# zhouyifan233/light-transport

Measured on AMD Instinct MI355X. Metric: photon_steps_per_sec, higher is better.
Workload: dtype f64

## Files before the change

light_transport_amd/csrc/lt_api.cpp:

```cpp
#include <hip/hip_runtime_api.h>

#include <dlfcn.h>

#include <algorithm>
#include <cmath>
#include <cctype>
#include <cstdarg>
#include <cstdio>
#include <cstdlib>
#include <cstring>
#include <limits>
#include <mutex>
#include <new>
#include <string>
#include <vector>

#include "lt_internal.hpp"

using namespace ltk;

static const size_t kMeshLdsBudget = 64 * 1024;

namespace {

// ... 593 lines not shown
        const uint64_t full = (body + rounds * (uint64_t)lanes - 1) / (rounds * (uint64_t)lanes);
        for (uint64_t k = 0, done_b = 0; k < rounds * (uint64_t)lanes && done_b < body; k++) {
            const uint64_t take = full < body - done_b ? full : body - done_b;
            plan->batches.emplace_back(l, take);
            done_b += take; left -= take; l = (l + 1) % lanes;
        }
        while (left > 0) {
            const uint64_t take = (double)left > fit ? (uint64_t)fit : left;
            plan->batches.emplace_back(l, take);
            left -= take; l = (l + 1) % lanes;
        }
    }
    return LT_OK;
}

int choose_lanes(lt_ctx* c, uint64_t n)
{
    c->auto_pending = -1;
    if (c->overlap_mode == 1) return 1;
    if (c->overlap_mode >= 2) return n >= 8192 ? c->overlap_mode : 1;
    if (c->blocks_per_cu > 0 || n < kOverlapMinPhotons) return 1;
    for (int k = kAutoLanes - 1; k >= 0; k--) {
        const bool stale = c->auto_photons[k] != 0 && (n > 2 * c->auto_photons[k] || c->auto_photons[k] > 2 * n);
        if (c->auto_ms_per_photon[k] <= 0.0 || stale) { c->auto_pending = k; return k + 1; }
    }
    int best = 0;
    for (int k = 1; k < kAutoLanes; k++) if (c->auto_ms_per_photon[k] < c->auto_ms_per_photon[best]) best = k;
    return best + 1;
}

struct LogRun {
    lt_ctx* c; WalkParams P; Variant v; LaunchCfg cfg; LogGeom G;
};

struct WalkGate {
    std::mutex mu;
    hipEvent_t ring[64] = {};
    unsigned next = 0;
    hipEvent_t last = nullptr;
};
WalkGate& walk_gate(int device)
{
    static WalkGate gates[16];
    return gates[device & 15];
}

hipError_t lane_event(LogLane& ln, hipStream_t s)
{
    if (ln.ev_used == ln.evs.size()) {
        hipEvent_t ev;
        hipError_t e = hipEventCreate(&ev);
        if (e != hipSuccess) return e;
        ln.evs.push_back(ev);
    }
    return hipEventRecord(ln.evs[ln.ev_used++], s);
}

int run_log_plan(LogRun& R, const LogPlan& plan, uint64_t offset, int* n_batches)
{
    lt_ctx* c = R.c;
    const LogGeom& G = R.G;
    const bool hot = G.bits2 != 0 && c->dmap_valid;
    const uint32_t n_hist = G.bits2 ? G.nb1 : G.n_tiles;
    LaunchCfg cfg = R.cfg;
    cfg.lds_bytes = walk_lds_bytes(R.v, R.P.n_media, R.P.n_layers, R.P.n_tris, R.P.n_nodes, n_hist);
    const int resident = walk_max_blocks_per_cu(R.v, cfg.threads, cfg.lds_bytes);
    if (resident <= 0) return c->fail(LT_E_HIP, "lt_launch: log-mode kernel not resident");
    int per_cu = c->blocks_per_cu > 0 ? c->blocks_per_cu : (plan.lanes >= 2 ? (resident + 1) / 2 : resident);
    if (plan.lanes >= 2 && c->knob.overlap_walk_bpc >= 1 && c->knob.overlap_walk_bpc <= 8) per_cu = (int)c->knob.overlap_walk_bpc;
    const unsigned long long cap = (unsigned long long)per_cu * (unsigned long long)c->prop.multiProcessorCount;
    if (plan.lanes >= 2) {
        const size_t gb = c->n_vox() * c->grid_elem();
        HIP_TRY(c, hipEventRecord(c->ev_fork, c->stream));
        for (int l = 1; l < plan.lanes; l++) {
            if (!c->lanes[l].stream) HIP_TRY(c, hipStreamCreateWithFlags(&c->lanes[l].stream, hipStreamNonBlocking));
            HIP_TRY(c, hipStreamWaitEvent(c->lanes[l].stream, c->ev_fork, 0));
            HIP_TRY(c, hipMemsetAsync(c->d_gridx[l - 1].p, 0, gb, c->lanes[l].stream));
        }
    }
    for (const auto& bt : plan.batches) {
        LogLane& ln = c->lanes[bt.first];
        hipStream_t s = ln.stream;
        uint32_t* meta = (uint32_t*)ln.meta.p;
        WalkParams P = R.P;
        P.n_photons = bt.second; P.photon_offset = offset;
        if (bt.first >= 1) P.grid = c->d_gridx[bt.first - 1].p;
        P.head = (unsigned long long*)ln.head.p;
        P.log_idx = (uint32_t*)ln.log_idx.p; P.log_val = ln.log_val.p; P.log_fill = (uint32_t*)ln.log_fill.p;
        P.log_next = meta + LM_NEXT; P.log_overflow = meta + LM_OVERFLOW; P.log_cap_chunks = plan.cap_chunks[bt.first];
        P.log_hist = (uint32_t*)(hot ? ln.hist_unused.p : (G.bits2 ? ln.hist1.p : ln.hist.p)); P.log_n_hist = n_hist; P.log_hist_shift = kTileShift + G.bits2;
        P.log_ntx = G.ntx; P.log_nty = G.nty;
        const unsigned long long want = (bt.second + (unsigned long long)cfg.threads - 1) / (unsigned long long)cfg.threads;
        cfg.blocks = (int)(want < cap ? want : cap);
        if (cfg.blocks < 1) cfg.blocks = 1;

        LogReduceParams L;
        std::memset(&L, 0, sizeof L);
        L.log_idx = P.log_idx; L.log_val = P.log_val; L.log_fill = P.log_fill;
        L.tmp_idx = (uint32_t*)ln.tmp_idx.p; L.tmp_val = ln.tmp_val.p;
        L.hist1 = (uint32_t*)ln.hist1.p; L.hist = (uint32_t*)ln.hist.p;
        L.bin_base = (uint32_t*)ln.bin_base.p; L.bin_cnt = (uint32_t*)ln.bin_cnt.p;
        L.tile_base = (uint32_t*)ln.tile_base.p; L.tile_cnt = (uint32_t*)ln.tile_cnt.p;
        L.cursor1 = (uint32_t*)ln.cursor1.p; L.cursor2 = (uint32_t*)ln.cursor2.p;
        L.items2 = (uint32_t*)ln.items2.p; L.items_c = (uint32_t*)ln.items_c.p; L.items_r = (uint32_t*)ln.items_r.p;
        L.itab = (uint32_t*)ln.itab.p;
        L.meta = meta; L.job = (unsigned long long*)c->d_job.p; L.cap_chunks = P.log_cap_chunks;
        L.n_tiles = G.n_tiles; L.bits2 = G.bits2;
        L.grid = bt.first >= 1 ? c->d_gridx[bt.first - 1].p : c->d_grid.p; L.n_vox = c->n_vox(); L.tally = c->tally;
        L.nx = (uint32_t)c->nx; L.ny = (uint32_t)c->ny; L.nz = (uint32_t)c->nz; L.ntx = G.ntx; L.nty = G.nty;
        L.flush_atomic = 0;
        if (hot) { L.dmap = (const uint16_t*)c->d_dmap.p; L.dmeta = (const uint32_t*)c->d_dmeta.p; }

        HIP_TRY(c, hipMemsetAsync(ln.head.p, 0, sizeof(unsigned long long), s));
        HIP_TRY(c, hipMemsetAsync(meta, 0, LM_WORDS * 4, s));
        HIP_TRY(c, hipMemsetAsync(ln.hist.p, 0, (size_t)G.n_tiles * (G.bits2 ? kLogGroups2 : kLogGroups) * 4, s));
        HIP_TRY(c, hipMemsetAsync(ln.log_fill.p, 0, (size_t)P.log_cap_chunks * 4, s));
        if (G.bits2) HIP_TRY(c, hipMemsetAsync(ln.hist1.p, 0, (size_t)(hot ? log_max_digits() : G.nb1) * kLogGroups * 4, s));
        const bool last_batch = &bt == &plan.batches.back();
        const uint64_t waves_launched = (uint64_t)cfg.blocks * (uint64_t)(cfg.threads / 64);
        const bool big_enough = c->knob.tail_split >= 2 || bt.second >= kTailSplitMinPerWave * waves_launched;
        const bool split = R.v.mesh <= 1 && !R.v.table && !R.v.capture && c->knob.tail_split != 0 && big_enough &&
                           ((plan.lanes == 1 && (c->blocks_per_cu == 0 || c->knob.serial_walks > 0) && (!R.v.f32 || c->knob.tail_split >= 2)) ||
                            (plan.lanes > 1 && last_batch));
        L.alone = (plan.lanes == 1 && c->blocks_per_cu == 0 && !split) ? 1 : 0;
        if (c->knob.part_alone == 0 || c->knob.part_alone == 1) L.alone = (int)c->knob.part_alone;
        L.lds_part = c->knob.part_lds > 0 ? (int)(c->knob.part_lds & 7) : 0;
        Variant vw = R.v;
        if (split) {
            const size_t cap = (size_t)cfg.blocks * (size_t)(cfg.threads / 64) * kDumpPoolLanes;
            P.dump_max = c->knob.tail_split > 1 ? (uint32_t)std::min<long>(c->knob.tail_split, (long)kDumpPoolLanes) : kDumpMaxLanes;
            HIP_TRY(c, ln.pool.ensure(cap * (R.v.f32 ? sizeof(SurvD<float>) : sizeof(SurvD<double>))));
            HIP_TRY(c, ln.pool_n.ensure(4));
            if (!ln.tail_stream) HIP_TRY(c, hipStreamCreateWithFlags(&ln.tail_stream, hipStreamNonBlocking));
            if (!ln.ev_bulk) HIP_TRY(c, hipEventCreateWithFlags(&ln.ev_bulk, hipEventDisableTiming));
            if (!ln.ev_tail) HIP_TRY(c, hipEventCreateWithFlags(&ln.ev_tail, hipEventDisableTiming));
            HIP_TRY(c, hipMemsetAsync(ln.pool_n.p, 0, 4, s));
            P.pool = ln.pool.p; P.pool_n = (uint32_t*)ln.pool_n.p; P.pool_cap = (uint32_t)cap;
            vw.phase = 1;
        }
        const bool train = c->knob.serial_walks > 0;
        if (train) {
            WalkGate& g = walk_gate(c->device);
            std::lock_guard<std::mutex> lk(g.mu);
            if (g.last) HIP_TRY(c, hipStreamWaitEvent(s, g.last, 0));
        }
        HIP_TRY(c, lane_event(ln, s));
        HIP_TRY(c, launch_walk(P, vw, cfg, s));
        HIP_TRY(c, lane_event(ln, s));
        if (split) {
            HIP_TRY(c, hipEventRecord(ln.ev_bulk, s));
            HIP_TRY(c, hipStreamWaitEvent(ln.tail_stream, ln.ev_bulk, 0));
            WalkParams Pt = P;
            Pt.log_idx = nullptr; Pt.log_val = nullptr; Pt.log_n_hist = 0;
            Variant vt = R.v; vt.phase = 2;
            LaunchCfg ct = cfg;
            ct.lds_bytes = walk_lds_bytes(vt, P.n_media, P.n_layers, P.n_tris, P.n_nodes, 0);
            ct.blocks = (int)((P.pool_cap / 64u + (unsigned)(cfg.threads / 64) - 1) / (unsigned)(cfg.threads / 64));
            if (ct.blocks < 1) ct.blocks = 1;
            HIP_TRY(c, launch_walk(Pt, vt, ct, ln.tail_stream));
            HIP_TRY(c, hipEventRecord(ln.ev_tail, ln.tail_stream));
        }
        if (hot) HIP_TRY(c, launch_log_count1(L, s));
        HIP_TRY(c, G.bits2 ? launch_log_scan_bins(L, s) : launch_log_scan_tiles(L, s));
        if (train) {
            WalkGate& g = walk_gate(c->device);
            std::lock_guard<std::mutex> lk(g.mu);
            hipEvent_t& ev = g.ring[g.next++ & 63u];
            if (!ev) HIP_TRY(c, hipEventCreateWithFlags(&ev, hipEventDisableTiming));
            HIP_TRY(c, hipEventRecord(ev, s));
            g.last = ev;
        }
        HIP_TRY(c, lane_event(ln, s));
        HIP_TRY(c, launch_log_part1(L, s));
        LogReduceParams Lr = L;
        if (G.bits2 == 0) { Lr.log_idx = L.tmp_idx; Lr.log_val = L.tmp_val; }
        else HIP_TRY(c, launch_log_part2(L, s));
        HIP_TRY(c, lane_event(ln, s));
        if (split) Lr.flush_atomic = 1;
        HIP_TRY(c, launch_log_reduce(Lr, s));
        HIP_TRY(c, lane_event(ln, s));
        if (split) HIP_TRY(c, hipStreamWaitEvent(s, ln.ev_tail, 0));
        if (bt.first == 0 && G.bits2) c->tile_cnt_ready = true;
        offset += bt.second;
        (*n_batches)++;
    }
    for (int l = 1; l < plan.lanes; l++) {
        HIP_TRY(c, hipEventRecord(c->lanes[l].ev_done, c->lanes[l].stream));
        HIP_TRY(c, hipStreamWaitEvent(c->stream, c->lanes[l].ev_done, 0));
        HIP_TRY(c, launch_grid_add(c->d_grid.p, c->d_gridx[l - 1].p, c->tally, c->n_vox(), c->stream));
    }
    return LT_OK;
}

bool bvh_is_valid(const std::vector<lt_bvh_node>& n, int n_tris, int* max_depth)
{
    std::vector<std::pair<int, int>> todo{{0, 0}};
    std::vector<char> seen(n.size(), 0);
    size_t visited = 0;
    *max_depth = 0;
    while (!todo.empty()) {
        const auto [idx, depth] = todo.back(); todo.pop_back();
        if (idx < 0 || idx >= (int)n.size() || seen[idx]) return false;
        seen[idx] = 1; visited++;
        if (depth > *max_depth) *max_depth = depth;
        const lt_bvh_node& nd = n[idx];
        if (nd.n_prims > 0) { if (nd.offset < 0 || nd.offset + nd.n_prims > n_tris) return false; continue; }
        if (nd.axis < 0 || nd.axis > 2 || nd.offset <= idx + 1) return false;
        todo.emplace_back(nd.offset, depth + 1); todo.emplace_back(idx + 1, depth + 1);
    }
    return visited == n.size();
}

}

extern "C" {

int lt_abi_version(void) { return LT_ABI_VERSION; }

const char* lt_last_error(const lt_ctx* ctx) { return ctx ? ctx->err.c_str() : g_create_error.c_str(); }

int lt_create(lt_ctx** out, int device_id)
{
    if (!out) return LT_E_INVALID;
    *out = nullptr;
    int n_dev = 0;
    hipError_t e = hipGetDeviceCount(&n_dev);
    if (e != hipSuccess || n_dev <= 0) {
        g_create_error = std::string("no HIP device available (") + (e != hipSuccess ? hipGetErrorString(e) : "0 devices") +
                         "); this library has no CPU fallback";
        return LT_E_HIP;
    }
    if (device_id < 0 || device_id >= n_dev) { g_create_error = "device_id out of range"; return LT_E_INVALID; }
    lt_ctx* c = new (std::nothrow) lt_ctx();
    if (!c) { g_create_error = "out of host memory"; return LT_E_NOMEM; }
    c->device = device_id;
    {
        static const char* const names[] = {"query_min", "log_bits2", "log_hot", "overlap_walk_bpc", "diag_no_tally", "log_timing", "march_cells",
                                            "march_scale_milli", "no_march", "no_clearance", "no_near_lists", "clearance_cells", "march_info", "force_march", "tail_split", "part_alone", "serial_walks", "part_lds",
                                            "render_lds_tables"};
        for (const char* k : names) {
            std::string name = "LT_";
            for (const char* q = k; *q; q++) name += (char)std::toupper((unsigned char)*q);
            if (const char* v = std::getenv(name.c_str())) *c->knob_by_name(k) = std::atol(v);
        }
        if (const char* v = std::getenv("LT_OVERLAP_PATTERN")) c->knob.overlap_pattern = v;
    }
    e = hipSetDevice(device_id);
    if (e == hipSuccess) e = hipGetDeviceProperties(&c->prop, device_id);
    if (e == hipSuccess && std::strncmp(c->prop.gcnArchName, "gfx950", 6) != 0) {
        g_create_error = std::string("device arch ") + c->prop.gcnArchName + " is not gfx950: kernels are built for MI355X only";
        delete c;
        return LT_E_UNSUPPORTED;
    }
    if (e == hipSuccess) {
        size_t quarter = c->prop.totalGlobalMem / 4;
        c->log_budget = c->default_log_budget = quarter < ((size_t)64 << 30) ? quarter : ((size_t)64 << 30);
    }
    if (e == hipSuccess) e = hipStreamCreateWithFlags(&c->stream, hipStreamNonBlocking);
    c->lanes[0].stream = c->stream;
    if (e == hipSuccess) e = hipEventCreate(&c->ev0);
    if (e == hipSuccess) e = hipEventCreate(&c->ev1);
    if (e == hipSuccess) e = hipEventCreateWithFlags(&c->ev_fork, hipEventDisableTiming);
    for (int k = 0; k < kMaxLanes && e == hipSuccess; k++) e = hipEventCreateWithFlags(&c->lanes[k].ev_done, hipEventDisableTiming);
    if (e == hipSuccess) e = c->d_job.ensure(2 * sizeof(unsigned long long));
    if (e == hipSuccess) e = c->d_counters.ensure(sizeof(DevCounters));
    if (e == hipSuccess) e = c->d_head.ensure(sizeof(unsigned long long));
    if (e == hipSuccess) e = hipMemsetAsync(c->d_counters.p, 0, sizeof(DevCounters), c->stream);
    if (e != hipSuccess) {
        g_create_error = std::string("lt_create: ") + hipGetErrorString(e);
        delete c;
        return LT_E_HIP;
    }
    *out = c;
    return LT_OK;
}

int lt_destroy(lt_ctx* c)
{
    if (!c) return LT_OK;
    (void)hipSetDevice(c->device);
    if (c->stream) (void)hipStreamSynchronize(c->stream);
    for (int i = 0; i < 2; i++) { c->d_media[i].release(); c->d_zb[i].release(); c->d_if[i].release(); c->d_tris[i].release(); c->d_nodes[i].release(); }
    c->d_lm.release(); c->d_grid.release(); c->d_counters.release(); c->d_head.release(); c->d_table.release();
    c->d_scratch_in.release(); c->d_scratch_out.release(); c->d_scratch_aux.release();
    c->d_mats.release(); c->d_lights.release(); c->d_r0.release(); c->d_r1.release(); c->d_lc.release();
    c->d_img.release(); c->d_xy.release(); c->d_vtx.release(); c->d_vcnt.release(); c->d_clear.release();
    c->d_job.release(); c->d_dmap.release(); c->d_dmeta.release();
    c->d_mcell.release(); c->d_mlist.release(); c->d_mcoarse.release(); c->d_links.release();
    for (int k = 1; k < kMaxLanes; k++) { c->d_gridx[k - 1].release(); if (c->lanes[k].stream) (void)hipStreamSynchronize(c->lanes[k].stream); }
    for (int k = 0; k < kMaxLanes; k++) {
        c->lanes[k].release_all();
        for (hipEvent_t ev : c->lanes[k].evs) (void)hipEventDestroy(ev);
        if (c->lanes[k].ev_done) (void)hipEventDestroy(c->lanes[k].ev_done);
    }
    if (c->ev0) (void)hipEventDestroy(c->ev0);
    if (c->ev1) (void)hipEventDestroy(c->ev1);
    if (c->ev_fork) (void)hipEventDestroy(c->ev_fork);
    for (int k = 0; k < kMaxLanes; k++) {
        if (c->lanes[k].tail_stream) { (void)hipStreamSynchronize(c->lanes[k].tail_stream); (void)hipStreamDestroy(c->lanes[k].tail_stream); }
        if (c->lanes[k].ev_bulk) (void)hipEventDestroy(c->lanes[k].ev_bulk);
        if (c->lanes[k].ev_tail) (void)hipEventDestroy(c->lanes[k].ev_tail);
    }
    for (int k = 1; k < kMaxLanes; k++) if (c->lanes[k].stream) (void)hipStreamDestroy(c->lanes[k].stream);
    if (c->stream) (void)hipStreamDestroy(c->stream);
    delete c;
    return LT_OK;
}
// ... 10 lines not shown
    c->media.assign(media, media + n);
    c->scene_changed();
    c->tables_dirty = true;
    return LT_OK;
}

int lt_set_layers(lt_ctx* c, const double* z_bounds, const int32_t* medium_idx, int n, double n_above, double n_below)
{
    CHECK_CTX(c);
    if (!z_bounds || !medium_idx || n <= 0 || n > kMaxLayers)
        return c->fail(LT_E_INVALID, "lt_set_layers: need 1..%d layers", kMaxLayers);
    if (!std::isfinite(z_bounds[0])) return c->fail(LT_E_INVALID, "lt_set_layers: z_bounds[0] must be finite");
    for (int i = 0; i < n; i++) {
        if (!(z_bounds[i + 1] > z_bounds[i])) return c->fail(LT_E_INVALID, "lt_set_layers: z_bounds must ascend");
        if (medium_idx[i] < 0) return c->fail(LT_E_INVALID, "lt_set_layers: negative medium index");
    }
    if (!(n_above > 0) || !(n_below > 0)) return c->fail(LT_E_INVALID, "lt_set_layers: ambient indices must be > 0");
    c->z_bounds.assign(z_bounds, z_bounds + n + 1);
    c->layer_medium.assign(medium_idx, medium_idx + n);
    c->n_above = n_above; c->n_below = n_below;
    c->have_layers = true; c->have_mesh = false;
    c->scene_changed();
    c->tables_dirty = true;
    return LT_OK;
}

int lt_set_mesh(lt_ctx* c, const double* verts, const int32_t* med_front, const int32_t* med_back, int n_tris,
                const lt_bvh_node* nodes, int n_nodes)
{
    CHECK_CTX(c);
    if (!verts || !med_front || !med_back || n_tris <= 0 || !nodes || n_nodes <= 0)
        return c->fail(LT_E_INVALID, "lt_set_mesh: empty mesh or BVH");
    for (size_t i = 0; i < (size_t)n_tris * 9; i++)
        if (!std::isfinite(verts[i])) return c->fail(LT_E_INVALID, "lt_set_mesh: non-finite vertex");
    std::vector<lt_bvh_node> nn(nodes, nodes + n_nodes);
    int depth = 0;
    if (!bvh_is_valid(nn, n_tris, &depth))
        return c->fail(LT_E_INVALID, "lt_set_mesh: BVH is not a valid pre-order tree over %d triangles", n_tris);
    size_t covered = 0;
    for (const auto& nd : nn) if (nd.n_prims > 0) covered += (size_t)nd.n_prims;
    if (covered != (size_t)n_tris) return c->fail(LT_E_INVALID, "lt_set_mesh: leaves cover %zu of %d triangles", covered, n_tris);
    c->verts.assign(verts, verts + (size_t)n_tris * 9);
    c->med_front.assign(med_front, med_front + n_tris);
    c->med_back.assign(med_back, med_back + n_tris);
    c->nodes.swap(nn);
    c->have_mesh = true; c->have_layers = false;
    c->surf_mats.clear();
    c->scene_changed();
    c->tables_dirty = true;
    return LT_OK;
}

int lt_set_grid(lt_ctx* c, int nx, int ny, int nz, const double origin[3], const double voxel[3], int tally_dtype)
{
    CHECK_CTX(c);
    if (nx <= 0 || ny <= 0 || nz <= 0 || !origin || !voxel) return c->fail(LT_E_INVALID, "lt_set_grid: bad shape");
    if (tally_dtype < LT_TALLY_F32 || tally_dtype > LT_TALLY_U64FX) return c->fail(LT_E_INVALID, "lt_set_grid: bad tally dtype");
    for (int k = 0; k < 3; k++)
        if (!(voxel[k] > 0) || !std::isfinite(origin[k])) return c->fail(LT_E_INVALID, "lt_set_grid: bad origin/voxel");
    if ((double)nx * ny * nz > 2147483647.0) return c->fail(LT_E_UNSUPPORTED, "lt_set_grid: more than 2^31-1 voxels");
    BIND(c);
    c->nx = nx; c->ny = ny; c->nz = nz; c->tally = tally_dtype;
    for (int k = 0; k < 3; k++) { c->origin[k] = origin[k]; c->voxel[k] = voxel[k]; }
    HIP_TRY(c, c->d_grid.ensure(c->n_vox() * c->grid_elem()));
    c->have_grid = true;
    c->scene_changed();
    return lt_zero_tally(c);
}

int lt_set_source(lt_ctx* c, int type, const double pos[3], const double dir[3], const double* extra, int start_medium)
{
    CHECK_CTX(c);
    if (!pos || !dir || (type != LT_SRC_PENCIL && type != LT_SRC_COSINE_QUAD)) return c->fail(LT_E_INVALID, "lt_set_source: bad arguments");
    const double l = std::sqrt(dir[0] * dir[0] + dir[1] * dir[1] + dir[2] * dir[2]);
    if (!(l > 0) || !std::isfinite(l)) return c->fail(LT_E_INVALID, "lt_set_source: zero direction");
    if (type == LT_SRC_COSINE_QUAD && !extra) return c->fail(LT_E_INVALID, "lt_set_source: quad source needs extra[6]");
    c->src_type = type; c->start_medium = start_medium;
    for (int k = 0; k < 3; k++) { c->src_pos[k] = pos[k]; c->src_dir[k] = dir[k] / l; }
    for (int k = 0; k < 6; k++) c->src_extra[k] = extra ? extra[k] : 0.0;
    c->have_source = true;
    c->scene_changed();
    return LT_OK;
}

int lt_set_max_steps(lt_ctx* c, uint32_t max_steps)
{
    CHECK_CTX(c);
    if (max_steps == 0) return c->fail(LT_E_INVALID, "lt_set_max_steps: must be > 0");
    c->max_steps = max_steps;
    return LT_OK;
}

int lt_set_tuning(lt_ctx* c, const char* key, int64_t value)
{
    CHECK_CTX(c);
    long* k = key ? c->knob_by_name(key) : nullptr;
    if (!k) return c->fail(LT_E_INVALID, "lt_set_tuning: unknown key '%s'", key ? key : "(null)");
    *k = value < 0 ? -1 : (long)value;
    if (!std::strcmp(key, "log_hot") || !std::strcmp(key, "log_bits2")) { c->dmap_valid = false; }
    return LT_OK;
}

int lt_set_tally_quantity(lt_ctx* c, int quantity)
{
    CHECK_CTX(c);
    if (quantity != LT_QUANTITY_ABSORBED && quantity != LT_QUANTITY_FLUENCE)
        return c->fail(LT_E_INVALID, "lt_set_tally_quantity: LT_QUANTITY_ABSORBED or LT_QUANTITY_FLUENCE");
    if (quantity != c->quantity) { c->quantity = quantity; c->media_dirty = true; }
    return LT_OK;
}

int lt_set_launch_config(lt_ctx* c, int blocks_per_cu, int threads_per_block)
{
    CHECK_CTX(c);
    if (blocks_per_cu < 0 || threads_per_block < 0 || threads_per_block > 256 || (threads_per_block % 64) != 0)
        return c->fail(LT_E_INVALID, "lt_set_launch_config: threads must be a multiple of 64, <= 256");
    c->blocks_per_cu = blocks_per_cu; c->threads_per_block = threads_per_block;
    return LT_OK;
}

int lt_zero_tally(lt_ctx* c)
{
    CHECK_CTX(c);
    BIND(c);
    if (c->have_grid) HIP_TRY(c, hipMemsetAsync(c->d_grid.p, 0, c->n_vox() * c->grid_elem(), c->stream));
    HIP_TRY(c, hipMemsetAsync(c->d_counters.p, 0, sizeof(DevCounters), c->stream));
    return LT_OK;
}

int lt_launch(lt_ctx* c, uint64_t n_photons, uint64_t photon_offset, uint64_t seed, const double* rng_table,
              uint64_t table_steps, uint32_t flags)
{
    CHECK_CTX(c);
    if (c->media.empty()) return c->fail(LT_E_STATE, "lt_launch: lt_set_media first");
    if (!c->have_layers && !c->have_mesh) return c->fail(LT_E_STATE, "lt_launch: lt_set_layers or lt_set_mesh first");
    if (!c->have_grid) return c->fail(LT_E_STATE, "lt_launch: lt_set_grid first");
    if (!c->have_source) return c->fail(LT_E_STATE, "lt_launch: lt_set_source first");
    const int n_media = (int)c->media.size();
    if (c->have_layers) {
        for (int32_t m : c->layer_medium) if (m >= n_media) return c->fail(LT_E_INVALID, "lt_launch: layer medium index %d >= %d media", m, n_media);
    } else {
        for (size_t i = 0; i < c->med_front.size(); i++)
            if (c->med_front[i] >= n_media || c->med_back[i] >= n_media || c->med_front[i] < -1 || c->med_back[i] < -1)
                return c->fail(LT_E_INVALID, "lt_launch: triangle %zu medium index out of range", i);
        if (c->start_medium < 0 || c->start_medium >= n_media) return c->fail(LT_E_INVALID, "lt_launch: start_medium out of range");
    }
    Variant v;
    v.f32 = (flags & LT_FLAG_F32_WALK) ? 1 : 0;
    v.mesh = c->have_mesh ? 1 : 0;
    v.table = rng_table ? 1 : 0;
    v.tally = c->tally;
    v.capture = c->max_vertices > 0 ? 1 : 0;
    v.phase = 0;
    if (v.capture && (v.f32 || v.table)) return c->fail(LT_E_UNSUPPORTED, "lt_launch: vertex capture runs the f64 walk with the XORWOW generator");
    if (c->on(c->knob.diag_no_tally)) v.tally = 3;
    if (v.table && v.f32) return c->fail(LT_E_UNSUPPORTED, "lt_launch: table RNG runs the f64 walk only");
    if (v.table && v.tally == LT_TALLY_F32) return c->fail(LT_E_UNSUPPORTED, "lt_launch: table RNG needs an f64 or u64fx tally");
    if (v.table && table_steps == 0) return c->fail(LT_E_INVALID, "lt_launch: table_steps == 0");
    BIND(c);
    int rc = upload_tables(c);
    if (rc) return rc;
    if (n_photons == 0) { c->timed = false; return LT_OK; }

    if (v.table) {
        const size_t bytes = (size_t)n_photons * (size_t)table_steps * 4 * sizeof(double);
        HIP_TRY(c, c->d_table.ensure(bytes));
        HIP_TRY(c, hipMemcpyAsync(c->d_table.p, rng_table, bytes, hipMemcpyHostToDevice, c->stream));
        HIP_TRY(c, hipStreamSynchronize(c->stream));
    }

    WalkParams P;
    std::memset(&P, 0, sizeof P);
    P.head = (unsigned long long*)c->d_head.p;
    P.n_photons = n_photons; P.photon_offset = photon_offset; P.seed = seed;
    const int pi = v.f32 ? 1 : 0;
    P.media = c->d_media[pi].p; P.zb = c->d_zb[pi].p; P.ifaces = c->d_if[pi].p; P.layer_medium = (const int32_t*)c->d_lm.p;
    P.tris = c->d_tris[pi].p; P.nodes = c->d_nodes[pi].p; P.links = c->have_mesh && c->have_links ? (const int16_t*)c->d_links.p : nullptr;
    P.n_media = n_media;
    P.n_layers = c->have_layers ? (int)c->layer_medium.size() : 0;
    P.n_tris = c->have_mesh ? (int)c->med_front.size() : 0;
    P.n_nodes = c->have_mesh ? (int)c->nodes.size() : 0;
    P.n_above = c->n_above; P.n_below = c->n_below;
    P.grid = c->d_grid.p; P.nx = c->nx; P.ny = c->ny; P.nz = c->nz; P.tally = c->tally;
    for (int k = 0; k < 3; k++) {
        P.origin[k] = c->origin[k]; P.inv_voxel[k] = 1.0 / c->voxel[k];
        P.src_pos[k] = c->src_pos[k]; P.src_dir[k] = c->src_dir[k];
        P.src_e1[k] = c->src_extra[k]; P.src_e2[k] = c->src_extra[3 + k];
    }
    P.fdim[0] = (double)c->nx; P.fdim[1] = (double)c->ny; P.fdim[2] = (double)c->nz;
    for (int k = 0; k < 3; k++) { P.f32.origin[k] = (float)P.origin[k]; P.f32.inv_voxel[k] = (float)P.inv_voxel[k]; P.f32.fdim[k] = (float)P.fdim[k]; }
    P.src_type = c->src_type; P.start_medium = c->start_medium;
    P.table = (const double*)c->d_table.p; P.table_steps = table_steps;
    P.max_steps = c->max_steps;
    P.counters = (DevCounters*)c->d_counters.p;
    if (c->knob.query_min >= 1 && c->knob.query_min <= 64) P.query_min = (unsigned)c->knob.query_min;
    if (c->have_mesh && c->have_clear) {
        P.clear = (const uint4*)c->d_clear.p; P.cnx = c->cn[0]; P.cny = c->cn[1]; P.cnz = c->cn[2];
        for (int k = 0; k < 3; k++) {
            P.corg[k] = c->corg[k]; P.cinv[k] = 1.0 / c->ccell[k]; P.cdim[k] = (double)c->cn[k];
            P.f32.corg[k] = (float)P.corg[k]; P.f32.cinv[k] = (float)P.cinv[k]; P.f32.cdim[k] = (float)P.cdim[k];
        }
    }
    if (c->have_mesh && c->have_march) P.mg = c->mgrid;
    c->captured_photons = 0;
    if (c->max_vertices > 0) {
        const size_t vb = (size_t)n_photons * c->max_vertices * sizeof(lt_vertex);
        if (vb > ((size_t)64 << 30)) return c->fail(LT_E_NOMEM, "lt_launch: vertex capture needs %zu bytes (> 64 GiB)", vb);
        HIP_TRY(c, c->d_vtx.ensure(vb));
        HIP_TRY(c, c->d_vcnt.ensure((size_t)n_photons * sizeof(uint32_t)));
        HIP_TRY(c, hipMemsetAsync(c->d_vcnt.p, 0, (size_t)n_photons * sizeof(uint32_t), c->stream));
        P.vertices = (lt_vertex*)c->d_vtx.p; P.vertex_counts = (uint32_t*)c->d_vcnt.p; P.max_vertices = c->max_vertices;
        c->captured_photons = n_photons; c->captured_max_vertices = c->max_vertices;
    }

    LaunchCfg cfg;
    cfg.threads = c->threads_per_block > 0 ? c->threads_per_block : 256;
    cfg.lds_bytes = walk_lds_bytes(v, P.n_media, P.n_layers, P.n_tris, P.n_nodes);
    if (v.mesh && (cfg.lds_bytes > kMeshLdsBudget || (c->on(c->knob.force_march) && c->have_march && !v.table))) {
        if (v.table) return c->fail(LT_E_UNSUPPORTED, "lt_launch: table RNG with a mesh beyond the LDS budget");
        v.mesh = c->have_march ? 3 : 2;
        cfg.lds_bytes = walk_lds_bytes(v, P.n_media, P.n_layers, P.n_tris, P.n_nodes);
    }
    int resident = walk_max_blocks_per_cu(v, cfg.threads, cfg.lds_bytes);
    if (resident <= 0) return c->fail(LT_E_HIP, "lt_launch: kernel variant not resident (occupancy query returned %d)", resident);
    int per_cu = c->blocks_per_cu > 0 ? c->blocks_per_cu : resident;
    unsigned long long want = (n_photons + (unsigned long long)cfg.threads - 1) / (unsigned long long)cfg.threads;
    unsigned long long cap = (unsigned long long)per_cu * (unsigned long long)c->prop.multiProcessorCount;
    cfg.blocks = (int)(want < cap ? want : cap);
    if (cfg.blocks < 1) cfg.blocks = 1;

    const int mode = c->tally_mode == 2 ? 1 : c->tally_mode;
    { int rc3 = collect_log_stats(c); if (rc3) return rc3; }
    LogGeom G = log_geom(c);
    bool use_log = mode == 1 && !v.table && c->max_vertices == 0 && G.n_tiles <= kMaxLogTiles && !c->on(c->knob.diag_no_tally);
    if (use_log) {
        LogRun R;
        R.c = c; R.P = P; R.v = v; R.cfg = cfg; R.G = G;
        if (c->dmap_valid && (c->dmap_tiles != G.n_tiles || c->dmap_bits2 != G.bits2)) c->dmap_valid = c->tile_cnt_ready = false;
        c->stages_valid = false;
        for (LogLane& ln : c->lanes) ln.ev_used = 0;
        HIP_TRY(c, hipMemsetAsync(c->d_job.p, 0, 2 * sizeof(unsigned long long), c->stream));
        uint64_t done = 0;
        int n_batches = 0;
        if (c->rec_per_photon <= 0.0 && n_photons > kPilotPhotons) {
            LogPlan pilot;
            rc = plan_log(c, kPilotPhotons, 1, &pilot);
            if (rc == LT_OK) rc = run_log_plan(R, pilot, photon_offset, &n_batches);
            if (rc == LT_E_NOMEM) { use_log = false; rc = LT_OK; }
            else if (rc) return rc;
            else {
                c->log_stats_pending = true; c->pending_photons = kPilotPhotons; c->auto_pending = -1;
                if ((rc = collect_log_stats(c))) return rc;
                done = kPilotPhotons;
            }
        }
        if (use_log && G.bits2 && !c->dmap_valid && c->tile_cnt_ready && G.n_tiles <= kMaxHotTiles && G.nb1 < log_max_digits()) {
            uint32_t max_hot = log_max_digits() - G.nb1;
            if (c->knob.log_hot >= 0 && (uint32_t)c->knob.log_hot < max_hot) max_hot = (uint32_t)c->knob.log_hot;
            if (max_hot > 0) {
                HIP_TRY(c, c->d_dmap.ensure(((size_t)G.n_tiles + 2) * sizeof(uint16_t)));
                HIP_TRY(c, c->d_dmeta.ensure(4 * sizeof(uint32_t)));
                HIP_TRY(c, launch_log_plan((const uint32_t*)c->lanes[0].tile_cnt.p, G.n_tiles, G.bits2, max_hot, (uint16_t*)c->d_dmap.p,
                                           (uint32_t*)c->d_dmeta.p, c->stream));
                c->dmap_valid = true; c->dmap_tiles = G.n_tiles; c->dmap_bits2 = G.bits2;
            }
        }
        if (use_log) {
            int lanes = choose_lanes(c, n_photons - done);
            LogPlan plan;
            rc = plan_log(c, n_photons - done, lanes, &plan);
            while (rc == LT_E_NOMEM && lanes > 1) {
                lanes--; rc = plan_log(c, n_photons - done, lanes, &plan);
                if (c->auto_pending >= 0) c->auto_pending = lanes - 1;
            }
            if (rc == LT_E_NOMEM) { use_log = false; rc = LT_OK; }
            else if (rc) return rc;
            else {
                HIP_TRY(c, hipEventRecord(c->ev0, c->stream));
                if ((rc = run_log_plan(R, plan, photon_offset + done, &n_batches))) return rc;
                HIP_TRY(c, hipEventRecord(c->ev1, c->stream));
                c->stages_valid = true; c->last_batches = (uint64_t)n_batches; c->last_lanes = plan.lanes;
                c->last_hot = G.bits2 != 0 && c->dmap_valid;
                c->log_stats_pending = true; c->pending_photons = n_photons;
                if (c->auto_pending >= 0 && done > 0) c->auto_pending = -1;
                c->timed = true;
                if (c->on(c->knob.log_timing)) {
                    double ms[4]; uint64_t rec = 0, bat = 0;
                    if (lt_last_log_stages(c, ms, &rec, &bat) == LT_OK)
                        std::fprintf(stderr, "[lt log] %llu photons, %d lane(s), %llu batches, %llu records (%.1f / photon), %llu to atomics; "
                                     "stage sums ms: walk %.2f scan %.2f partition %.2f reduce %.2f\n", (unsigned long long)n_photons,
                                     plan.lanes, (unsigned long long)bat, (unsigned long long)rec, (double)rec / (double)n_photons,
                                     (unsigned long long)c->last_overflow, ms[0], ms[1], ms[2], ms[3]);
                }
                return LT_OK;
            }
        }
        P.n_photons = n_photons - done; P.photon_offset = photon_offset + done;
        want = (P.n_photons + (unsigned long long)cfg.threads - 1) / (unsigned long long)cfg.threads;
        cfg.blocks = (int)(want < cap ? want : cap);
        if (cfg.blocks < 1) cfg.blocks = 1;
    }

    c->stages_valid = false;
    HIP_TRY(c, hipMemsetAsync(c->d_head.p, 0, sizeof(unsigned long long), c->stream));
    HIP_TRY(c, hipEventRecord(c->ev0, c->stream));
    HIP_TRY(c, launch_walk(P, v, cfg, c->stream));
    HIP_TRY(c, hipEventRecord(c->ev1, c->stream));
    c->timed = true;
    return LT_OK;
}

int lt_reserve_log(lt_ctx* c, uint64_t n_photons)
{
    CHECK_CTX(c);
    if (!c->have_grid) return c->fail(LT_E_STATE, "lt_reserve_log: lt_set_grid first");
    BIND(c);
    LogPlan plan;
    int lanes = c->overlap_mode == 1 ? 1 : (c->overlap_mode >= 2 ? c->overlap_mode : ((c->blocks_per_cu == 0 && n_photons >= kOverlapMinPhotons) ? kAutoLanes : 1));
    int rc = plan_log(c, n_photons, lanes, &plan);
    if (rc == LT_E_NOMEM) return c->fail(LT_E_NOMEM, "lt_reserve_log: not enough device memory for the deposit log");
    return rc;
}

int lt_set_tally_mode(lt_ctx* c, int mode, uint64_t log_bytes)
{
    CHECK_CTX(c);
    if (mode < 0 || mode > 2) return c->fail(LT_E_INVALID, "lt_set_tally_mode: mode must be LT_MODE_ATOMIC, LT_MODE_LOG or LT_MODE_AUTO");
    c->tally_mode = mode;
    c->log_budget = log_bytes ? (size_t)log_bytes : c->default_log_budget;
    return LT_OK;
}

int lt_last_log_hot_tiles(lt_ctx* c, uint32_t* hot_tiles, uint32_t* threshold)
{
    CHECK_CTX(c);
    if (!c->stages_valid) return c->fail(LT_E_STATE, "lt_last_log_hot_tiles: the last launch did not use the deposit log");
    BIND(c);
    uint32_t m[2] = {0, 0};
    if (c->last_hot) {
        HIP_TRY(c, hipStreamSynchronize(c->stream));
        HIP_TRY(c, hipMemcpy(m, c->d_dmeta.p, sizeof m, hipMemcpyDeviceToHost));
    }
    if (hot_tiles) *hot_tiles = m[0];
    if (threshold) *threshold = m[1];
    return LT_OK;
}

int lt_set_overlap(lt_ctx* c, int lanes)
{
    CHECK_CTX(c);
    if (lanes < 0 || lanes > kMaxLanes) return c->fail(LT_E_INVALID, "lt_set_overlap: 0 (auto), 1, 2 or 3");
    c->overlap_mode = lanes;
    for (double& a : c->auto_ms_per_photon) a = 0.0;
    for (uint64_t& a : c->auto_photons) a = 0;
    c->auto_pending = -1;
    return LT_OK;
}

int lt_sync(lt_ctx* c)
{
    CHECK_CTX(c);
    BIND(c);
    HIP_TRY(c, hipStreamSynchronize(c->stream));
    return collect_log_stats(c);
}

int lt_last_kernel_ms(lt_ctx* c, double* ms)
{
    CHECK_CTX(c);
    if (!ms) return c->fail(LT_E_INVALID, "lt_last_kernel_ms: null output");
    if (!c->timed) return c->fail(LT_E_STATE, "lt_last_kernel_ms: no launch recorded");
    BIND(c);
    HIP_TRY(c, hipEventSynchronize(c->ev1));
    float f = 0;
    HIP_TRY(c, hipEventElapsedTime(&f, c->ev0, c->ev1));
    *ms = (double)f;
    return LT_OK;
}

int lt_last_log_stages(lt_ctx* c, double ms_out[4], uint64_t* records, uint64_t* batches)
{
    CHECK_CTX(c);
    if (!ms_out) return c->fail(LT_E_INVALID, "lt_last_log_stages: null output");
    if (!c->stages_valid) return c->fail(LT_E_STATE, "lt_last_log_stages: the last launch did not use the log tally");
    BIND(c);
    HIP_TRY(c, hipEventSynchronize(c->ev1));
    { int rc3 = collect_log_stats(c); if (rc3) return rc3; }
    for (int k = 0; k < 4; k++) ms_out[k] = 0.0;
    for (int l = 0; l < kMaxLanes; l++) {
        const LogLane& ln = c->lanes[l];
// ... 398 lines not shown
```

light_transport_amd/csrc/lt_internal.hpp:

```cpp
#pragma once
#include <hip/hip_runtime_api.h>
#include <stdint.h>

#include "../../include/lt.h"

namespace ltk {

template <typename R>
struct MedD {
    R mu_t, inv_mu_t, absorb, g;
    R n, one_m_g2, one_p_g2, inv_2g;
    R dep;
    R one_m_g, two_g;
    R pad_;
};

template <typename R>
struct IfD {
    R n_up, n_dn;
    R nr_down, nr_up;
};

template <typename R>
struct TriD {
    R a[3], ab[3], ac[3], n[3];
    int32_t med_front, med_back;
};

template <typename R>
struct NodeD {
    R lo[3], hi[3];
    int32_t offset, n_prims, axis;
    int32_t skip;
};

struct DevCounters {
    unsigned long long photons, steps;
    double w[8];
};
enum { CW_ABSORBED = 0, CW_LOST, CW_ESC_TOP, CW_ESC_BOT, CW_ESC_MESH, CW_SPECULAR, CW_ROULETTE, CW_CAPPED };

constexpr int kMaxMedia = 32;
constexpr uint32_t kLogChunk = 8192;
constexpr uint32_t kTileShift = 14;
constexpr uint32_t kTileSize = 1u << kTileShift;
constexpr uint32_t kTileBX = 5, kTileBY = 5, kTileBZ = 4;
constexpr uint32_t kLogGroups = 16;
constexpr uint32_t kLogGroups2 = 8;
constexpr int kMaxLayers = 64;

constexpr uint32_t kMarchCountMask = 63u;
struct MarchGrid {
    const uint2* cell;
    const uint32_t* list;
    int nx, ny, nz;
    double org[3], inv[3], h[3];
    double fn[3];
    float org32[3], inv32[3], h32[3], fn32[3];
    double nudge64, nudge32;
};

template <typename R>
struct SurvD {
    R p[3], u[3], w, sleft;
    unsigned long long pid;
    int32_t cur;
    uint32_t step;
    uint32_t rng[6];
    uint32_t held[3];
    uint32_t q_pend;
};
constexpr uint32_t kDumpMaxLanes = 32;
constexpr uint32_t kDumpPoolLanes = 48;

struct WalkParams {
    unsigned long long* head;
    unsigned long long n_photons, photon_offset, seed;
    const void* media;
    const void* zb;
    const void* ifaces;
    const int32_t* layer_medium;
    const void* tris;
    const void* nodes;
    const int16_t* links;
    int n_media, n_layers, n_tris, n_nodes;
    double n_above, n_below;
    void* grid;
    int nx, ny, nz, tally;
    double origin[3], inv_voxel[3];
    double fdim[3];
    double cdim[3];
    struct { float origin[3], inv_voxel[3], fdim[3], corg[3], cinv[3], cdim[3]; } f32;
    int src_type, start_medium;
    double src_pos[3], src_dir[3], src_e1[3], src_e2[3];
    const double* table;
    unsigned long long table_steps;
    unsigned max_steps;
    unsigned query_min;
    DevCounters* counters;
    uint32_t* log_idx;
    void* log_val;
    uint32_t* log_fill;
    uint32_t* log_next;
    uint32_t log_cap_chunks;
    uint32_t* log_hist;
    uint32_t log_n_hist, log_hist_shift, log_ntx, log_nty;
    uint32_t* log_overflow;
    const uint4* clear;
    int cnx, cny, cnz;
    double corg[3], cinv[3];
    MarchGrid mg;
    void* pool;
    uint32_t* pool_n;
    uint32_t pool_cap;
    uint32_t dump_max;
    lt_vertex* vertices;
    uint32_t* vertex_counts;
    unsigned max_vertices;
};

struct LaunchCfg {
    int blocks, threads;
    size_t lds_bytes;
};

struct Variant {
    int f32;
    int mesh;
    int table;
    int tally;
    int capture;
    int phase;
};

hipError_t launch_walk(const WalkParams& P, const Variant& v, const LaunchCfg& cfg, hipStream_t s);
size_t walk_lds_bytes(const Variant& v, int n_media, int n_layers, int n_tris, int n_nodes, unsigned n_hist = 0);
int walk_max_blocks_per_cu(const Variant& v, int threads, size_t lds_bytes);

struct RenderParams {
    const void* tris;
    const void* nodes;
    const lt_surface_material* mats;
    const lt_point_light* lights;
    const int16_t* links;
    int n_tris, n_nodes, n_lights;
    int W, H, S, D;
    double cam[3], f_distance;
    const double* xs;
    const double* ys;
    double* rand_0;
    const double* rand_1;
    const int32_t* light_choice;
    double* image;
    int variant;
    int choices;
    int lds_tables;
};
constexpr int kRenderOldMaxDepth = 24;
hipError_t launch_march_clearance(const void* tris_f64, const void* nodes_f64, int n_nodes, const MarchGrid& G, uint2* cells,
                                  double* coarse, hipStream_t s);
hipError_t launch_build_clearance(const void* tris_f64, int n_tris, int near_lists, void* clear_records, int nx, int ny, int nz,
                                  const double org[3], const double cell[3], hipStream_t s);
hipError_t launch_render_surface(const RenderParams& P, hipStream_t s);

enum { LM_NEXT = 0,
       LM_OVERFLOW = 16,
       LM_RECORDS,
       LM_ITEMS2,
       LM_ITEMS_R,
       LM_SLICE,
       LM_ITEMS_C,
       LM_WORK,
       LM_WORDS = 24 };
static_assert(kLogGroups == 16, "LM_NEXT holds one counter per group");
constexpr uint32_t kTileAlign = 8, kBinAlign = 8;

struct LogReduceParams {
    const uint32_t* log_idx; const void* log_val; const uint32_t* log_fill;
    uint32_t* tmp_idx; void* tmp_val;
    uint32_t* hist1;
    uint32_t* hist;
    uint32_t* bin_base; uint32_t* bin_cnt;
    uint32_t* tile_base; uint32_t* tile_cnt;
    uint32_t* cursor1;
    uint32_t* cursor2;
    uint32_t* items2;
    uint32_t* items_c;
    uint32_t* itab;
    uint32_t* items_r;
    uint32_t* meta;
    unsigned long long* job;
    uint32_t cap_chunks;
    uint32_t n_tiles, bits2;
    void* grid; size_t n_vox; int tally;
    uint32_t nx, ny, nz, ntx, nty;
    const uint16_t* dmap; const uint32_t* dmeta;
    int alone;
    int flush_atomic;
    int lds_part;
};
hipError_t launch_log_scan_bins(const LogReduceParams& L, hipStream_t s);
hipError_t launch_log_count1(const LogReduceParams& L, hipStream_t s);
hipError_t launch_log_plan(const uint32_t* tile_cnt, uint32_t n_tiles, uint32_t bits2, uint32_t max_hot, uint16_t* dmap,
                           uint32_t* dmeta, hipStream_t s);
uint32_t log_max_digits();
constexpr uint32_t kMaxHotTiles = 8192;
hipError_t launch_log_scan_tiles(const LogReduceParams& L, hipStream_t s);
hipError_t launch_log_part1(const LogReduceParams& L, hipStream_t s);
hipError_t launch_log_part2(const LogReduceParams& L, hipStream_t s);
hipError_t launch_log_reduce(const LogReduceParams& L, hipStream_t s);
uint32_t log_part_item();

hipError_t launch_intersect_rays(const void* tris, const void* nodes, int n_tris, int n_nodes,
                                 const double* o, const double* d, const double* tmax, size_t n,
                                 int use_bvh, const MarchGrid* G, const int16_t* links, int32_t* prim, double* t, hipStream_t s);
hipError_t launch_triangle_intersect(const double* o, const double* d, const double* tris, size_t n,
                                     double* t, hipStream_t s);
hipError_t launch_intersect_bounds(const double* o, const double* d, const double* tmax,
                                   const double* boxes, size_t n, int32_t* hit, hipStream_t s);
hipError_t launch_eval(int fn, const double* in, size_t n, double* out, hipStream_t s);
hipError_t launch_rng_raw(unsigned long long seed, unsigned long long photon_id, unsigned count,
                          uint32_t* out, hipStream_t s);
hipError_t launch_grid_to_f64(const void* grid, int tally, size_t n, double* out, hipStream_t s);
hipError_t launch_grid_add(void* dst, const void* src, int tally, size_t n, hipStream_t s);

}
```

light_transport_amd/csrc/lt_kernels.hip:

```cpp
#include <hip/hip_runtime.h>

#define ROCRAND_DETAIL_BM_NOT_IN_STATE
#include <rocrand/rocrand_xorwow.h>
#include <rocrand/rocrand_uniform.h>

#include "lt_internal.hpp"

static_assert(sizeof(rocrand_state_xorwow) == 6 * sizeof(uint32_t), "rocrand_state_xorwow is not {d, x[5]}: SurvD::rng and the tail-split hand-over assume it");

namespace ltk {

#define LT_DEV __device__ __forceinline__
#define LT_PV(name, k) (sizeof(R) == 8 ? (R)P.name[k] : (R)P.f32.name[k])
#define LT_GV(name, k) (sizeof(R) == 8 ? (R)G.name[k] : (R)G.name##32[k])

#ifdef LT_K_IN_SGPR
LT_DEV double fma_k(double a, double b, double k) { double r; asm("v_fma_f64 %0, %1, %2, %3" : "=v"(r) : "v"(a), "v"(b), "s"(k)); return r; }
LT_DEV double fma_mk(double a, double k, double c) { return __builtin_fma(a, k, c); }
LT_DEV double mul_k(double a, double k) { return a * k; }
LT_DEV double fma_kk(double x, double k) { double r; asm("v_fma_f64 %0, %1, %2, %2" : "=v"(r) : "v"(x), "s"(k)); return r; }
#else
template <unsigned long long BITS> LT_DEV double fma_kb(double a, double b)
{
    double r;
// ... 31 lines not shown
{
    double r = __builtin_amdgcn_rcp(b);
    r = __builtin_fma(__builtin_fma(-b, r, 1.0), r, r);
    const double q = a * r;
    return __builtin_fma(__builtin_fma(-b, q, a), r, q);
}
LT_DEV double sqrt_core(double x, double y)
{
    double g = x * y, h = 0.5 * y;
    const double r = __builtin_fma(-h, g, 0.5);
    g = __builtin_fma(g, r, g); h = __builtin_fma(h, r, h);
    const double d = __builtin_fma(-g, g, x);
    return __builtin_fma(d, h, g);
}
LT_DEV double sqrt01(double x)
{
    const double xc = __builtin_fmax(x, 0.0);
    return sqrt_core(xc, __builtin_amdgcn_rsq(__builtin_fmax(xc, 1e-300)));
}
LT_DEV double sqrt_pos(double x) { return sqrt_core(x, __builtin_amdgcn_rsq(x)); }
LT_DEV double rsqrt_pos(double x)
{
    double y = __builtin_amdgcn_rsq(x);
    double e = __builtin_fma(-(x * y), y, 1.0);
    y = __builtin_fma(0.5 * y, e, y);
    e = __builtin_fma(-(x * y), y, 1.0);
    return __builtin_fma(0.5 * y, e, y);
}
__device__ const double kWalkMathTab[(97 + 64) * 2] = {
    0x1.5555555555555p-7, -0x1.269621134db92p-2, 0x1.51d07eae2f815p-7, -0x1.1bf99635a6b95p-2, 0x1.4e5e0a72f0539p-7, -0x1.1178e8227e47cp-2,
    0x1.4afd6a052bf5bp-7, -0x1.07138604d5862p-2, 0x1.47ae147ae147bp-7, -0x1.f991c6cb3b379p-3, 0x1.446f86562d9fbp-7, -0x1.e530effe71012p-3,
    0x1.4141414141414p-7, -0x1.d1037f2655e7bp-3, 0x1.3e22cbce4a902p-7, -0x1.bd087383bd8adp-3, 0x1.3b13b13b13b14p-7, -0x1.a93ed3c8ad9e3p-3,
    0x1.3813813813814p-7, -0x1.95a5adcf7017fp-3, 0x1.3521cfb2b78c1p-7, -0x1.823c16551a3c2p-3, 0x1.323e34a2b10bfp-7, -0x1.6f0128b756abcp-3,
    0x1.2f684bda12f68p-7, -0x1.5bf406b543db2p-3, 0x1.2c9fb4d812ca0p-7, -0x1.4913d8333b561p-3, 0x1.29e4129e4129ep-7, -0x1.365fcb0159016p-3,
    0x1.27350b8812735p-7, -0x1.23d712a49c202p-3, 0x1.2492492492492p-7, -0x1.1178e8227e47cp-3, 0x1.21fb78121fb78p-7, -0x1.fe89139dbd566p-4,
    0x1.1f7047dc11f70p-7, -0x1.da727638446a2p-4, 0x1.1cf06ada2811dp-7, -0x1.b6ac88dad5b1cp-4, 0x1.1a7b9611a7b96p-7, -0x1.9335e5d594989p-4,
    0x1.1811811811812p-7, -0x1.700d30aeac0e1p-4, 0x1.15b1e5f75270dp-7, -0x1.4d3115d207eacp-4, 0x1.135c81135c811p-7, -0x1.2aa04a44717a5p-4,
    0x1.1111111111111p-7, -0x1.08598b59e3a07p-4, 0x1.0ecf56be69c90p-7, -0x1.ccb73cdddb2ccp-5, 0x1.0c9714fbcda3bp-7, -0x1.894aa149fb343p-5,
    0x1.0a6810a6810a7p-7, -0x1.466aed42de3eap-5, 0x1.0842108421084p-7, -0x1.0415d89e74444p-5, 0x1.0624dd2f1a9fcp-7, -0x1.8492528c8cabfp-6,
    0x1.0410410410410p-7, -0x1.0205658935847p-6, 0x1.0204081020408p-7, -0x1.010157588de71p-7, 0x1.0000000000000p-7, 0x0.0p+0,
    0x1.fc07f01fc07f0p-8, 0x1.fe02a6b106789p-8, 0x1.f81f81f81f820p-8, 0x1.fc0a8b0fc03e4p-7, 0x1.f44659e4a4271p-8, 0x1.7b91b07d5b11bp-6,
    0x1.f07c1f07c1f08p-8, 0x1.f829b0e783300p-6, 0x1.ecc07b301ecc0p-8, 0x1.39e87b9febd60p-5, 0x1.e9131abf0b767p-8, 0x1.77458f632dcfcp-5,
    0x1.e573ac901e574p-8, 0x1.b42dd711971bfp-5, 0x1.e1e1e1e1e1e1ep-8, 0x1.f0a30c01162a6p-5, 0x1.de5d6e3f8868ap-8, 0x1.16536eea37ae1p-4,
    0x1.dae6076b981dbp-8, 0x1.341d7961bd1d1p-4, 0x1.d77b654b82c34p-8, 0x1.51b073f06183fp-4, 0x1.d41d41d41d41dp-8, 0x1.6f0d28ae56b4cp-4,
    0x1.d0cb58f6ec074p-8, 0x1.8c345d6319b21p-4, 0x1.cd85689039b0bp-8, 0x1.a926d3a4ad563p-4, 0x1.ca4b3055ee191p-8, 0x1.c5e548f5bc743p-4,
    0x1.c71c71c71c71cp-8, 0x1.e27076e2af2e6p-4, 0x1.c3f8f01c3f8f0p-8, 0x1.fec9131dbeabbp-4, 0x1.c0e070381c0e0p-8, 0x1.0d77e7cd08e59p-3,
    0x1.bdd2b899406f7p-8, 0x1.1b72ad52f67a0p-3, 0x1.bacf914c1bad0p-8, 0x1.29552f81ff523p-3, 0x1.b7d6c3dda338bp-8, 0x1.371fc201e8f74p-3,
    0x1.b4e81b4e81b4fp-8, 0x1.44d2b6ccb7d1ep-3, 0x1.b2036406c80d9p-8, 0x1.526e5e3a1b438p-3, 0x1.af286bca1af28p-8, 0x1.5ff3070a793d4p-3,
    0x1.ac5701ac5701bp-8, 0x1.6d60fe719d21dp-3, 0x1.a98ef606a63bep-8, 0x1.7ab890210d909p-3, 0x1.a6d01a6d01a6dp-8, 0x1.87fa06520c911p-3,
    0x1.a41a41a41a41ap-8, 0x1.9525a9cf456b4p-3, 0x1.a16d3f97a4b02p-8, 0x1.a23bc1fe2b563p-3, 0x1.9ec8e951033d9p-8, 0x1.af3c94e80bff3p-3,
    0x1.9c2d14ee4a102p-8, 0x1.bc286742d8cd6p-3, 0x1.999999999999ap-8, 0x1.c8ff7c79a9a22p-3, 0x1.970e4f80cb872p-8, 0x1.d5c216b4fbb91p-3,
    0x1.948b0fcd6e9e0p-8, 0x1.e27076e2af2e6p-3, 0x1.920fb49d0e229p-8, 0x1.ef0adcbdc5936p-3, 0x1.8f9c18f9c18fap-8, 0x1.fb9186d5e3e2bp-3,
    0x1.8d3018d3018d3p-8, 0x1.0402594b4d041p-2, 0x1.8acb90f6bf3aap-8, 0x1.0a324e27390e3p-2, 0x1.886e5f0abb04ap-8, 0x1.1058bf9ae4ad5p-2,
    0x1.8618618618618p-8, 0x1.1675cababa60ep-2, 0x1.83c977ab2beddp-8, 0x1.1c898c16999fbp-2, 0x1.8181818181818p-8, 0x1.22941fbcf7966p-2,
    0x1.7f405fd017f40p-8, 0x1.2895a13de86a3p-2, 0x1.7d05f417d05f4p-8, 0x1.2e8e2bae11d31p-2, 0x1.7ad2208e0ecc3p-8, 0x1.347dd9a987d55p-2,
    0x1.78a4c8178a4c8p-8, 0x1.3a64c556945eap-2, 0x1.767dce434a9b1p-8, 0x1.404308686a7e4p-2, 0x1.745d1745d1746p-8, 0x1.4618bc21c5ec2p-2,
    0x1.724287f46debcp-8, 0x1.4be5f957778a1p-2, 0x1.702e05c0b8170p-8, 0x1.51aad872df82dp-2, 0x1.6e1f76b4337c7p-8, 0x1.5767717455a6cp-2,
    0x1.6c16c16c16c17p-8, 0x1.5d1bdbf5809cap-2, 0x1.6a13cd1537290p-8, 0x1.62c82f2b9c795p-2, 0x1.6816816816817p-8, 0x1.686c81e9b14afp-2,
    0x1.661ec6a5122f9p-8, 0x1.6e08eaa2ba1e4p-2, 0x1.642c8590b2164p-8, 0x1.739d7f6bbd007p-2, 0x1.623fa77016240p-8, 0x1.792a55fdd47a2p-2,
    0x1.6058160581606p-8, 0x1.7eaf83b82afc3p-2, 0x1.5e75bb8d015e7p-8, 0x1.842d1da1e8b17p-2, 0x1.5c9882b931057p-8, 0x1.89a3386c1425bp-2,
    0x1.5ac056b015ac0p-8, 0x1.8f11e873662c7p-2, 0x1.58ed2308158edp-8, 0x1.947941c2116fbp-2, 0x1.571ed3c506b3ap-8, 0x1.99d958117e08bp-2,
    0x1.5555555555555p-8, 0x1.9f323ecbf984cp-2,
    0x0.0p+0, 0x1.0000000000000p+0, 0x1.917a6bc29b42cp-4, 0x1.fd88da3d12526p-1, 0x1.8f8b83c69a60bp-3, 0x1.f6297cff75cb0p-1,
    0x1.294062ed59f06p-2, 0x1.e9f4156c62ddap-1, 0x1.87de2a6aea963p-2, 0x1.d906bcf328d46p-1, 0x1.e2b5d3806f63bp-2, 0x1.c38b2f180bdb1p-1,
    0x1.1c73b39ae68c8p-1, 0x1.a9b66290ea1a3p-1, 0x1.44cf325091dd6p-1, 0x1.8bc806b151741p-1, 0x1.6a09e667f3bcdp-1, 0x1.6a09e667f3bcdp-1,
    0x1.8bc806b151741p-1, 0x1.44cf325091dd6p-1, 0x1.a9b66290ea1a3p-1, 0x1.1c73b39ae68c8p-1, 0x1.c38b2f180bdb1p-1, 0x1.e2b5d3806f63bp-2,
    0x1.d906bcf328d46p-1, 0x1.87de2a6aea963p-2, 0x1.e9f4156c62ddap-1, 0x1.294062ed59f06p-2, 0x1.f6297cff75cb0p-1, 0x1.8f8b83c69a60bp-3,
    0x1.fd88da3d12526p-1, 0x1.917a6bc29b42cp-4, 0x1.0000000000000p+0, 0x0.0p+0, 0x1.fd88da3d12526p-1, -0x1.917a6bc29b42cp-4,
    0x1.f6297cff75cb0p-1, -0x1.8f8b83c69a60bp-3, 0x1.e9f4156c62ddap-1, -0x1.294062ed59f06p-2, 0x1.d906bcf328d46p-1, -0x1.87de2a6aea963p-2,
    0x1.c38b2f180bdb1p-1, -0x1.e2b5d3806f63bp-2, 0x1.a9b66290ea1a3p-1, -0x1.1c73b39ae68c8p-1, 0x1.8bc806b151741p-1, -0x1.44cf325091dd6p-1,
    0x1.6a09e667f3bcdp-1, -0x1.6a09e667f3bcdp-1, 0x1.44cf325091dd6p-1, -0x1.8bc806b151741p-1, 0x1.1c73b39ae68c8p-1, -0x1.a9b66290ea1a3p-1,
    0x1.e2b5d3806f63bp-2, -0x1.c38b2f180bdb1p-1, 0x1.87de2a6aea963p-2, -0x1.d906bcf328d46p-1, 0x1.294062ed59f06p-2, -0x1.e9f4156c62ddap-1,
    0x1.8f8b83c69a60bp-3, -0x1.f6297cff75cb0p-1, 0x1.917a6bc29b42cp-4, -0x1.fd88da3d12526p-1, 0x0.0p+0, -0x1.0000000000000p+0,
    -0x1.917a6bc29b42cp-4, -0x1.fd88da3d12526p-1, -0x1.8f8b83c69a60bp-3, -0x1.f6297cff75cb0p-1, -0x1.294062ed59f06p-2, -0x1.e9f4156c62ddap-1,
    -0x1.87de2a6aea963p-2, -0x1.d906bcf328d46p-1, -0x1.e2b5d3806f63bp-2, -0x1.c38b2f180bdb1p-1, -0x1.1c73b39ae68c8p-1, -0x1.a9b66290ea1a3p-1,
    -0x1.44cf325091dd6p-1, -0x1.8bc806b151741p-1, -0x1.6a09e667f3bcdp-1, -0x1.6a09e667f3bcdp-1, -0x1.8bc806b151741p-1, -0x1.44cf325091dd6p-1,
    -0x1.a9b66290ea1a3p-1, -0x1.1c73b39ae68c8p-1, -0x1.c38b2f180bdb1p-1, -0x1.e2b5d3806f63bp-2, -0x1.d906bcf328d46p-1, -0x1.87de2a6aea963p-2,
    -0x1.e9f4156c62ddap-1, -0x1.294062ed59f06p-2, -0x1.f6297cff75cb0p-1, -0x1.8f8b83c69a60bp-3, -0x1.fd88da3d12526p-1, -0x1.917a6bc29b42cp-4,
    -0x1.0000000000000p+0, 0x0.0p+0, -0x1.fd88da3d12526p-1, 0x1.917a6bc29b42cp-4, -0x1.f6297cff75cb0p-1, 0x1.8f8b83c69a60bp-3,
    -0x1.e9f4156c62ddap-1, 0x1.294062ed59f06p-2, -0x1.d906bcf328d46p-1, 0x1.87de2a6aea963p-2, -0x1.c38b2f180bdb1p-1, 0x1.e2b5d3806f63bp-2,
    -0x1.a9b66290ea1a3p-1, 0x1.1c73b39ae68c8p-1, -0x1.8bc806b151741p-1, 0x1.44cf325091dd6p-1, -0x1.6a09e667f3bcdp-1, 0x1.6a09e667f3bcdp-1,
    -0x1.44cf325091dd6p-1, 0x1.8bc806b151741p-1, -0x1.1c73b39ae68c8p-1, 0x1.a9b66290ea1a3p-1, -0x1.e2b5d3806f63bp-2, 0x1.c38b2f180bdb1p-1,
    -0x1.87de2a6aea963p-2, 0x1.d906bcf328d46p-1, -0x1.294062ed59f06p-2, 0x1.e9f4156c62ddap-1, -0x1.8f8b83c69a60bp-3, 0x1.f6297cff75cb0p-1,
    -0x1.917a6bc29b42cp-4, 0x1.fd88da3d12526p-1
};
constexpr int kLnTabEntries = 97, kScTabEntries = 64;
constexpr size_t kWalkMathTabBytes = sizeof(double) * 2 * (kLnTabEntries + kScTabEntries);
LT_DEV double neg_log_tab(double x, const double* T)
{
    int e = __builtin_amdgcn_frexp_exp(x);
    double m = __builtin_amdgcn_frexp_mant(x);
    if (m < 0.75) { m += m; e -= 1; }
    const double t = m * 128.0;
    const double qf = __builtin_rint(t);
    const double d = t - qf;
    const double2 Tj = *reinterpret_cast<const double2*>(T + 2 * ((int)qf - 96));
    const double r = d * Tj.x;
    double p = 1.0 / 7.0;
    p = fma_k(p, r, -1.0 / 6.0); p = fma_k(p, r, 1.0 / 5.0); p = fma_k(p, r, -0.25); p = fma_k(p, r, 1.0 / 3.0);
    p = __builtin_fma(p, r, -0.5);
    const double lnm = Tj.y + __builtin_fma(r * r, p, r);
    const double de = (double)e;
    return -fma_mk(de, 6.93147180369123816490e-01, fma_mk(de, 1.90821492927058770002e-10, lnm));
}
LT_DEV void sincos_turn_tab(double xi, const double* T, double* sn, double* cs)
{
    const double t = 64.0 * xi;
    const double qf = __builtin_rint(t);
    const double a = mul_k(t - qf, 9.8174770424681038702e-02);
    const double z = a * a;
    double ps = -1.9841269841269841270e-04;
    ps = fma_k(ps, z, 8.3333333333333333333e-03);
    ps = fma_k(ps, z, -1.6666666666666666667e-01);
    const double sd = __builtin_fma(a * z, ps, a);
    double pc = 2.4801587301587301587e-05;
    pc = fma_k(pc, z, -1.3888888888888888889e-03);
    pc = fma_k(pc, z, 4.1666666666666666667e-02);
    pc = __builtin_fma(pc, z, -0.5);
    const double cd = __builtin_fma(pc, z, 1.0);
    const double2 Ti = *reinterpret_cast<const double2*>(T + 2 * (kLnTabEntries + ((int)qf & (kScTabEntries - 1))));
    *sn = __builtin_fma(Ti.x, cd, Ti.y * sd);
    *cs = __builtin_fma(Ti.y, cd, -(Ti.x * sd));
}

LT_DEV void sincos_small_f64(double x, double* sn, double* cs)
{
    const double kf = __builtin_rint(x * 0.63661977236758134308);
    double a = __builtin_fma(-kf, 1.57079632679489655800e+00, x);
    a = __builtin_fma(-kf, 6.12323399573676603587e-17, a);
    const double z = a * a;
    double ps = -7.6471637318198164759e-13;
    ps = fma_k(ps, z, 1.6059043836821614599e-10);
    ps = fma_k(ps, z, -2.5052108385441718775e-08);
    ps = fma_k(ps, z, 2.7557319223985890653e-06);
    ps = fma_k(ps, z, -1.9841269841269841270e-04);
    ps = fma_k(ps, z, 8.3333333333333333333e-03);
    ps = fma_k(ps, z, -1.6666666666666666667e-01);
    const double s = __builtin_fma(a * z, ps, a);
    double pc = 4.7794773323873852974e-14;
    pc = fma_k(pc, z, -1.1470745597729724714e-11);
    pc = fma_k(pc, z, 2.0876756987868098979e-09);
    pc = fma_k(pc, z, -2.7557319223985890653e-07);
    pc = fma_k(pc, z, 2.4801587301587301587e-05);
    pc = fma_k(pc, z, -1.3888888888888888889e-03);
    pc = fma_k(pc, z, 4.1666666666666666667e-02);
    pc = __builtin_fma(pc, z, -0.5);
    const double c = __builtin_fma(pc, z, 1.0);
    const int q = (int)kf & 3;
    const double s1 = (q & 1) ? c : s, c1 = (q & 1) ? s : c;
    *sn = (q & 2) ? -s1 : s1;
    *cs = ((q + 1) & 2) ? -c1 : c1;
}

LT_DEV double neg_log_raw(unsigned k, const double* T)
{
    const unsigned n = k + 1u;
    const int lz = __clz((int)n);
    const unsigned nm = n << (lz & 31);
    const unsigned hi = nm >= 0xC0000000u ? 1u : 0u;
    const unsigned sh = 24u + hi;
    const unsigned j = ((nm >> (sh - 1u)) + 1u) >> 1;
    const int dint = (int)(nm - (j << sh));
    const double d = __builtin_ldexp((double)dint, -(int)sh);
    const double2 Tj = *reinterpret_cast<const double2*>(T + 2 * ((int)j - 96));
    const double r = d * Tj.x;
    double p = 1.0 / 7.0;
    p = fma_k(p, r, -1.0 / 6.0); p = fma_k(p, r, 1.0 / 5.0); p = fma_k(p, r, -0.25); p = fma_k(p, r, 1.0 / 3.0);
    p = __builtin_fma(p, r, -0.5);
    const double lnm = Tj.y + __builtin_fma(r * r, p, r);
    const double de = (double)((int)hi - 1 - lz);
    const double v = -fma_mk(de, 6.93147180369123816490e-01, fma_mk(de, 1.90821492927058770002e-10, lnm));
    return n == 0u ? 0.0 : v;
}
LT_DEV void sincos_turn_raw(unsigned k, const double* T, double* sn, double* cs)
{
    const unsigned n = k + 1u;
    const unsigned iq = ((n >> 25) + 1u) >> 1;
    const int drem = (int)(n - (iq << 26));
    const double a = mul_k((double)drem, 1.4629180792671596e-09);
    const double z = a * a;
    double ps = -1.9841269841269841270e-04;
    ps = fma_k(ps, z, 8.3333333333333333333e-03);
    ps = fma_k(ps, z, -1.6666666666666666667e-01);
    const double sd = __builtin_fma(a * z, ps, a);
    double pc = 2.4801587301587301587e-05;
    pc = fma_k(pc, z, -1.3888888888888888889e-03);
    pc = fma_k(pc, z, 4.1666666666666666667e-02);
    pc = __builtin_fma(pc, z, -0.5);
    const double cd = __builtin_fma(pc, z, 1.0);
    const double2 Ti = *reinterpret_cast<const double2*>(T + 2 * (kLnTabEntries + (int)(iq & (unsigned)(kScTabEntries - 1))));
    *sn = __builtin_fma(Ti.x, cd, Ti.y * sd);
    *cs = __builtin_fma(Ti.y, cd, -(Ti.x * sd));
}
template <typename R> struct Mx;
template <> struct Mx<double> {
    static LT_DEV double log(double x) { return ::log(x); }
    static LT_DEV double sqrt(double x) { return ::sqrt(x); }
    static LT_DEV double abs(double x) { return ::fabs(x); }
    static LT_DEV double clamp_unit(double c) { return __builtin_fmax(__builtin_fmin(c, 1.0), -1.0); }
    static LT_DEV double sin(double x) { return ::sin(x); }
    static LT_DEV double cos(double x) { return ::cos(x); }
    static LT_DEV double neg_log(double xi, const double* T) { return neg_log_tab(xi, T); }
    static LT_DEV double sqrt_unit(double x) { return sqrt01(x); }
    static LT_DEV double max0(double x) { return __builtin_fmax(x, 0.0); }
    static LT_DEV unsigned sign_word(double x) { return (unsigned)__double2hiint(x); }
    static LT_DEV double max_tiny(double x) { return __builtin_fmax(x, 1e-300); }
    static LT_DEV double sqrt_pos(double x) { return ltk::sqrt_pos(x); }
    static LT_DEV double rsqrt_pos(double x) { return ltk::rsqrt_pos(x); }
    static LT_DEV double quot(double a, double b) { return fast_div(a, b); }
    static LT_DEV double rcp48(double d) { double r = __builtin_amdgcn_rcp(d); return __builtin_fma(__builtin_fma(-d, r, 1.0), r, r); }
    static LT_DEV void sincos_turn(double xi, const double* T, double* s, double* c) { sincos_turn_tab(xi, T, s, c); }
    static LT_DEV double inf() { return __builtin_huge_val(); }
    static LT_DEV double uniform(rocrand_state_xorwow* st)
    {
        const unsigned v1 = rocrand(st), v2 = rocrand(st);
        return fma_kk((double)(((unsigned long long)(v2 >> 11) << 32) | v1), 1.1102230246251565404e-16);
    }
    static LT_DEV double uniform32(rocrand_state_xorwow* st) { return fma_kk((double)rocrand(st), 2.3283064365386962891e-10); }
};
template <> struct Mx<float> {
    static LT_DEV float log(float x) { return ::logf(x); }
    static LT_DEV float sqrt(float x) { return ::sqrtf(x); }
    static LT_DEV float abs(float x) { return ::fabsf(x); }
    static LT_DEV float clamp_unit(float c) { return __builtin_fmaxf(__builtin_fminf(c, 1.0f), -1.0f); }
    static LT_DEV float sin(float x) { return ::sinf(x); }
    static LT_DEV float cos(float x) { return ::cosf(x); }
    static LT_DEV float neg_log(float xi, const double*) { return -::logf(xi); }
    static LT_DEV float sqrt_unit(float x) { return ::sqrtf(__builtin_fmaxf(x, 0.0f)); }
    static LT_DEV float max0(float x) { return __builtin_fmaxf(x, 0.0f); }
    static LT_DEV unsigned sign_word(float x) { return __float_as_uint(x); }
    static LT_DEV float max_tiny(float x) { return __builtin_fmaxf(x, 1e-30f); }
    static LT_DEV float sqrt_pos(float x) { return ::sqrtf(x); }
    static LT_DEV float rsqrt_pos(float x) { return 1.0f / ::sqrtf(x); }
    static LT_DEV float quot(float a, float b) { return a / b; }
    static LT_DEV float rcp48(float d) { return 1.0f / d; }
    static LT_DEV void sincos_turn(float xi, const double*, float* s, float* c) { ::sincospif(2.0f * xi, s, c); }
    static LT_DEV float inf() { return __builtin_huge_valf(); }
    static LT_DEV float uniform(rocrand_state_xorwow* st) { return rocrand_uniform(st); }
    static LT_DEV float uniform32(rocrand_state_xorwow* st) { return rocrand_uniform(st); }
};

template <typename R> LT_DEV R dot3(const R* a, const R* b) { return a[0] * b[0] + a[1] * b[1] + a[2] * b[2]; }
template <typename R> LT_DEV void cross3(const R* a, const R* b, R* o)
{
    o[0] = a[1] * b[2] - a[2] * b[1];
    o[1] = a[2] * b[0] - a[0] * b[2];
    o[2] = a[0] * b[1] - a[1] * b[0];
}
template <typename R> LT_DEV void normalize3(R* v)
{
    R l = Mx<R>::sqrt(v[0] * v[0] + v[1] * v[1] + v[2] * v[2]);
    v[0] /= l; v[1] /= l; v[2] /= l;
}

template <typename R>
LT_DEV R tri_hit(const R* o, const R* d, const TriD<R>* T)
{
    const R eps = (R)1e-7;
    const R nan = (R)__builtin_nanf("");
    R n[3] = {T->n[0], T->n[1], T->n[2]};
    R ddn = dot3(d, n);
    if (Mx<R>::abs(ddn) <= eps) return nan;
    R ab[3] = {T->ab[0], T->ab[1], T->ab[2]};
    R ac[3] = {T->ac[0], T->ac[1], T->ac[2]};
    R pvec[3], qvec[3], tvec[3];
    cross3(d, ac, pvec);
    R det = dot3(ab, pvec);
    if (-eps < det && det < eps) return nan;
    R inv_det = (R)1 / det;
    tvec[0] = o[0] - T->a[0]; tvec[1] = o[1] - T->a[1]; tvec[2] = o[2] - T->a[2];
    R u = dot3(tvec, pvec) * inv_det;
    if (u < 0 || u > 1) return nan;
    cross3(tvec, ab, qvec);
    R v = dot3(d, qvec) * inv_det;
    if (v < 0 || u + v > 1) return nan;
    R t = dot3(ac, qvec) * inv_det;
    return (t > eps) ? t : nan;
}

template <typename R> LT_DEV R box_widen()
{
    const R eps = (R)5.9604644775390625e-08;
    return (R)1 + (R)2 * (((R)3 * eps) / ((R)1 - (R)3 * eps));
}

template <typename R>
LT_DEV bool box_hit(const R* lo, const R* hi, const R* o, const R* inv_d, R tmax)
{
    R t0 = 0, t1 = tmax;
    const R widen = box_widen<R>();
#pragma unroll
    for (int i = 0; i < 3; i++) {
        R tn = (lo[i] - o[i]) * inv_d[i];
        R tf = (hi[i] - o[i]) * inv_d[i];
        if (tn > tf) { R s = tn; tn = tf; tf = s; }
        tf *= widen;
        t0 = tn > t0 ? tn : t0;
        t1 = tf < t1 ? tf : t1;
        if (t0 > t1) return false;
    }
    return true;
}

template <typename R>
LT_DEV void consider(const TriD<R>* tris, int i, const R* o, const R* d, int& bi, R& bt)
{
    R t = tri_hit(o, d, &tris[i]);
    if (t == t && t > (R)1e-6) {
        if (t < bt || (t == bt && bi >= 0 && i < bi)) { bt = t; bi = i; }
    }
}

template <typename R>
LT_DEV void nearest_bvh(const TriD<R>* tris, const NodeD<R>* nodes, int n_nodes, const R* o,
                        const R* d, R tmax, int& prim, R& t_out)
{
    int bi = -1; R bt = tmax;
    const R inv_d[3] = {(R)1 / d[0], (R)1 / d[1], (R)1 / d[2]};
    const R slack = box_widen<R>();
    int cur = 0;
    while (cur < n_nodes) {
        const NodeD<R>* nd = &nodes[cur];
        const R lo[3] = {nd->lo[0], nd->lo[1], nd->lo[2]};
        const R hi[3] = {nd->hi[0], nd->hi[1], nd->hi[2]};
        const int np = nd->n_prims, off = nd->offset, skip = nd->skip;
        if (box_hit(lo, hi, o, inv_d, bt * slack)) {
            if (np > 0) {
                for (int k = 0; k < np; k++) consider(tris, off + k, o, d, bi, bt);
                cur = skip;
            } else {
                cur = cur + 1;
            }
        } else {
            cur = skip;
        }
    }
    prim = bi; t_out = bi >= 0 ? bt : Mx<R>::inf();
}

template <typename R>
LT_DEV void nearest_bvh_ordered(const TriD<R>* tris, const NodeD<R>* nodes, int n_nodes, const int16_t* links, const R* o,
                                const R* d, R tmax, int& prim, R& t_out, bool ANY = false)
{
    int bi = -1; R bt = tmax;
    const R inv_d[3] = {(R)1 / d[0], (R)1 / d[1], (R)1 / d[2]};
    const R slack = box_widen<R>();
// ... 224 lines not shown
}

template <typename R>
LT_DEV bool march_round(const MarchGrid& G, MarchWave<R>* W, bool& marching, bool& heavy, bool& dirty, R& tcur, unsigned& qn)
{
    const unsigned lane = threadIdx.x & 63u;
    const R inf = Mx<R>::inf(), tol = (R)1e-4;
    const R hx = LT_GV(h, 0), hy = LT_GV(h, 1), hz = LT_GV(h, 2);
    const R nudge = sizeof(R) == 8 ? (R)G.nudge64 : (R)G.nudge32;
    unsigned n = 0, lst = 0;
    R tex = inf, bt = inf; float clr = 0.0f;
    bool m = marching;
    if (m) {
        bt = march_unbits(W->slot_t[lane]);
        if (!(tcur < bt)) m = false;
    }
    if (m) {
        const R px = W->ray[0][lane], py = W->ray[1][lane], pz = W->ray[2][lane];
        const R ux = W->ray[3][lane], uy = W->ray[4][lane], uz = W->ray[5][lane];
        const R fx = (px + tcur * ux - LT_GV(org, 0)) * LT_GV(inv, 0), fy = (py + tcur * uy - LT_GV(org, 1)) * LT_GV(inv, 1),
                fz = (pz + tcur * uz - LT_GV(org, 2)) * LT_GV(inv, 2);
        if (!(fx >= -tol && fx <= LT_GV(fn, 0) + tol && fy >= -tol && fy <= LT_GV(fn, 1) + tol && fz >= -tol && fz <= LT_GV(fn, 2) + tol) ||
            (ux > 0 ? fx >= LT_GV(fn, 0) : (ux < 0 && fx <= 0)) || (uy > 0 ? fy >= LT_GV(fn, 1) : (uy < 0 && fy <= 0)) ||
            (uz > 0 ? fz >= LT_GV(fn, 2) : (uz < 0 && fz <= 0))) m = false;
        else {
            int cx = (int)__builtin_floor(fx), cy = (int)__builtin_floor(fy), cz = (int)__builtin_floor(fz);
            cx = cx < 0 ? 0 : (cx >= G.nx ? G.nx - 1 : cx);
            cy = cy < 0 ? 0 : (cy >= G.ny ? G.ny - 1 : cy);
            cz = cz < 0 ? 0 : (cz >= G.nz ? G.nz - 1 : cz);
            const uint2 rec = G.cell[((size_t)cz * G.ny + cy) * G.nx + cx];
            n = rec.x & kMarchCountMask; lst = rec.y; clr = __uint_as_float(rec.x & ~kMarchCountMask);
            if (n == kMarchCountMask) { heavy = true; m = false; n = 0; }
            const R ix = W->ray[6][lane], iy = W->ray[7][lane], iz = W->ray[8][lane];
            const R ex = ix < inf && ix > -inf ? (LT_GV(org, 0) + (R)(cx + (ux > 0 ? 1 : 0)) * hx - px) * ix : inf;
            const R ey = iy < inf && iy > -inf ? (LT_GV(org, 1) + (R)(cy + (uy > 0 ? 1 : 0)) * hy - py) * iy : inf;
            const R ez = iz < inf && iz > -inf ? (LT_GV(org, 2) + (R)(cz + (uz > 0 ? 1 : 0)) * hz - pz) * iz : inf;
            tex = ex < ey ? (ex < ez ? ex : ez) : (ey < ez ? ey : ez);
        }
    }
    if (!m) marching = false;
    unsigned excl = 0, total_ = 0;
#pragma unroll
    for (unsigned b = 0; b < 6; b++) {
        const unsigned long long mb = __ballot((n >> b) & 1u);
        excl += __builtin_amdgcn_mbcnt_hi((unsigned)(mb >> 32), __builtin_amdgcn_mbcnt_lo((unsigned)mb, 0u)) << b;
        total_ += (unsigned)__popcll(mb) << b;
    }
    const unsigned incl = excl + n, cap = kMarchQ - qn;
    const bool blocked = incl > cap;
    const unsigned long long bm = __ballot(blocked);
    const unsigned pushed = bm ? (unsigned)__builtin_amdgcn_readlane((int)excl, __ffsll((long long)bm) - 1) : total_;
    if (!blocked) for (unsigned k = 0; k < n; k++) W->q_item[qn + excl + k] = (lane << 26) | (lst + k);
    qn += pushed;
    if (m && !blocked) {
        if (n) dirty = true;
        const R jump_min = (R)1.5 * (hx < hy ? (hx < hz ? hx : hz) : (hy < hz ? hy : hz));
        if (!(tex < bt)) marching = false;
        else {
            R tn = (R)clr > jump_min ? tex + (R)clr : tex + nudge;
            const R floor_ = tcur + nudge;
            tcur = tn > floor_ ? tn : floor_;
            if (!(tcur < bt)) marching = false;
        }
    }
    return bm != 0ull;
}

template <typename R>
LT_DEV void march_drain(const TriD<R>* tris, const MarchGrid& G, MarchWave<R>* W, unsigned& qn)
{
    typedef typename MarchBits<R>::type UB;
    const unsigned lane = threadIdx.x & 63u;
    __builtin_amdgcn_fence(__ATOMIC_RELEASE, "wavefront");
    for (unsigned j0 = 0; j0 < qn; j0 += 64u) {
        const unsigned j = j0 + lane;
        UB tb = ~(UB)0;
        if (j < qn) {
            const unsigned item = W->q_item[j], src = item >> 26;
            const int id = (int)G.list[item & 0x3ffffffu];
            const R o[3] = {W->ray[0][src], W->ray[1][src], W->ray[2][src]};
            const R d[3] = {W->ray[3][src], W->ray[4][src], W->ray[5][src]};
            const R t = tri_hit(o, d, &tris[id]);
            if (t == t && t > (R)1e-6) {
                tb = march_bits(t);
                const UB old = __hip_atomic_fetch_min(&W->slot_t[src], tb, __ATOMIC_RELAXED, __HIP_MEMORY_SCOPE_WORKGROUP);
                if (tb < old) W->slot_i[src] = kMarchNone;
            }
        }
        W->q_t[j] = tb;
    }
    __builtin_amdgcn_fence(__ATOMIC_ACQ_REL, "wavefront");
    for (unsigned j0 = 0; j0 < qn; j0 += 64u) {
        const unsigned j = j0 + lane;
        if (j < qn) {
            const UB tb = W->q_t[j];
            const unsigned item = W->q_item[j], src = item >> 26;
            if (tb != ~(UB)0 && tb == W->slot_t[src])
                (void)__hip_atomic_fetch_min(&W->slot_i[src], G.list[item & 0x3ffffffu], __ATOMIC_RELAXED, __HIP_MEMORY_SCOPE_WORKGROUP);
        }
    }
    __builtin_amdgcn_fence(__ATOMIC_ACQ_REL, "wavefront");
    qn = 0;
}

template <typename R>
LT_DEV void march_result(const TriD<R>* tris, const NodeD<R>* nodes, int n_nodes, const int16_t* links, MarchWave<R>* W, bool use_bvh, R px, R py, R pz,
                         R ux, R uy, R uz, R tmax, int& prim, R& t_out)
{
    const unsigned lane = threadIdx.x & 63u;
    prim = -1; t_out = Mx<R>::inf();
    if (use_bvh) {
        const R o[3] = {px, py, pz}, d[3] = {ux, uy, uz};
        nearest_bvh_walk(tris, nodes, n_nodes, links, o, d, tmax, prim, t_out);
    } else {
        const typename MarchBits<R>::type b = W->slot_t[lane];
        if (b < march_bits(tmax)) { prim = (int)W->slot_i[lane]; t_out = march_unbits(b); }
    }
}

template <typename R>
LT_DEV void march_service(const TriD<R>* tris, const NodeD<R>* nodes, int n_nodes, const MarchGrid& G, MarchWave<R>* W,
                          bool want, R px, R py, R pz, R ux, R uy, R uz, R tmax, R t0, int& prim, R& t_out)
{
    bool marching = false, heavy = false, dirty = false, outside = false;
    R tcur = t0 > 0 ? t0 : (R)0;
    if (want) { outside = !march_enter(G, W, px, py, pz, ux, uy, uz, tmax); marching = !outside; }
    unsigned qn = 0;
    while (__any(marching) || qn > 0) {
        bool full = false;
        if (__any(marching)) full = march_round(G, W, marching, heavy, dirty, tcur, qn);
        if (qn > 0 && (full || qn >= 64u || !__any(marching))) march_drain(tris, G, W, qn);
    }
    if (want) march_result(tris, nodes, n_nodes, (const int16_t*)nullptr, W, outside || heavy, px, py, pz, ux, uy, uz, tmax, prim, t_out);
    else { prim = -1; t_out = Mx<R>::inf(); }
}

template <typename R> LT_DEV R hg_pdf(R cos_t, R g)
{
    R denom = (R)1 + g * g + (R)2 * g * cos_t;
    return (R)0.07957747154594767 * ((R)1 - g * g) / (denom * Mx<R>::sqrt(denom));
}

template <typename R> LT_DEV R hg_sample(R xi, R g, R one_m_g2, R one_p_g2, R inv_2g)
{
    R c;
    if (g == 0) c = (R)2 * xi - (R)1;
    else {
        R t = Mx<R>::quot(one_m_g2, (R)1 - g + (R)2 * g * xi);
        c = (one_p_g2 - t * t) * inv_2g;
    }
    return Mx<R>::clamp_unit(c);
}

template <typename R> LT_DEV R hg_sample_walk(R xi, const MedD<R>* M)
{
    if (M->g == 0) return (R)2 * xi - (R)1;
    const R t = Mx<R>::quot(M->one_m_g2, M->two_g * xi + M->one_m_g);
    return (M->one_p_g2 - t * t) * M->inv_2g;
}

template <typename R> LT_DEV void onb(const R* n, R* v2, R* v3)
{
    if (Mx<R>::abs(n[0]) > Mx<R>::abs(n[1])) {
        R l = Mx<R>::sqrt(n[0] * n[0] + n[2] * n[2]);
        v2[0] = -n[2] / l; v2[1] = 0; v2[2] = n[0] / l;
    } else {
        R l = Mx<R>::sqrt(n[1] * n[1] + n[2] * n[2]);
        v2[0] = 0; v2[1] = n[2] / l; v2[2] = -n[1] / l;
    }
    cross3(n, v2, v3);
}

template <typename R, bool LEAN = false> LT_DEV void disk(R u0, R u1, R* d)
{
    R ox = (R)2 * u0 - (R)1, oy = (R)2 * u1 - (R)1;
    if (ox == 0 && oy == 0) { d[0] = 0; d[1] = 0; return; }
    R r, theta;
    if (Mx<R>::abs(ox) > Mx<R>::abs(oy)) { r = ox; theta = (R)0.7853981633974483 * (oy / ox); }
    else { r = oy; theta = (R)1.5707963267948966 - (R)0.7853981633974483 * (ox / oy); }
    if constexpr (LEAN && sizeof(R) == 8) {
        double sn, cs;
        sincos_small_f64(theta, &sn, &cs);
        d[0] = r * cs; d[1] = r * sn;
    } else {
        d[0] = r * Mx<R>::cos(theta); d[1] = r * Mx<R>::sin(theta);
    }
}

template <typename R> LT_DEV void cosine_hemi_frame(const R* n, const R* v2, const R* v3, const R* wi_in, R u0, R u1, R* out)
{
    R wiz = -wi_in[2];
    R d[2]; disk(u0, u1, d);
    R zz = (R)1 - d[0] * d[0] - d[1] * d[1];
    R z = Mx<R>::sqrt(zz > 0 ? zz : (R)0);
    R oz = z;
    if (wiz < 0) oz = -oz;
    R pdf = (wiz * oz > 0) ? Mx<R>::abs(z) * (R)0.3183098861837907 : (R)0;
#pragma unroll
    for (int k = 0; k < 3; k++) out[k] = d[0] * v2[k] + d[1] * v3[k] + oz * n[k];
    out[3] = pdf;
}
template <typename R, bool LEAN = false> LT_DEV void cosine_hemi(const R* n, const R* wi_in, R u0, R u1, R* out)
{
    R wiz = -wi_in[2];
    R d[2]; disk<R, LEAN>(u0, u1, d);
    R zz = (R)1 - d[0] * d[0] - d[1] * d[1];
    R z = Mx<R>::sqrt(zz > 0 ? zz : (R)0);
    R oz = z;
    R v2[3], v3[3]; onb(n, v2, v3);
    if (wiz < 0) oz = -oz;
    R pdf = (wiz * oz > 0) ? Mx<R>::abs(z) * (R)0.3183098861837907 : (R)0;
#pragma unroll
    for (int k = 0; k < 3; k++) out[k] = d[0] * v2[k] + d[1] * v3[k] + oz * n[k];
    out[3] = pdf;
}

template <typename R> LT_DEV void reflect(const R* v, const R* n, R* o)
{
    R k = (R)2 * dot3(v, n);
    o[0] = v[0] - k * n[0]; o[1] = v[1] - k * n[1]; o[2] = v[2] - k * n[2];
    normalize3(o);
}

template <typename R> LT_DEV void reflect_walk(const R* v, const R* n, R* o)
{
    R k = (R)2 * dot3(v, n);
    o[0] = v[0] - k * n[0]; o[1] = v[1] - k * n[1]; o[2] = v[2] - k * n[2];
    const R inv = Mx<R>::rsqrt_pos(o[0] * o[0] + o[1] * o[1] + o[2] * o[2]);
    o[0] *= inv; o[1] *= inv; o[2] *= inv;
}

template <typename R> LT_DEV R boundary(const R* d, const R* nf, R n1, R n2, R* cos_t_out, R* refr)
{
    R cos_i = -dot3(d, nf);
    if (n1 == n2) {
        *cos_t_out = cos_i; refr[0] = d[0]; refr[1] = d[1]; refr[2] = d[2];
        return 0;
    }
    R Nr = Mx<R>::quot(n1, n2);
    R rad = (R)1 - Nr * Nr * ((R)1 - cos_i * cos_i);
    if (rad <= 0) { *cos_t_out = 0; refr[0] = refr[1] = refr[2] = 0; return 1; }
    R cos_t = Mx<R>::sqrt_pos(rad);
    R a = n1 * cos_i, b = n2 * cos_t, c = n1 * cos_t, e = n2 * cos_i;
    const R sab = a + b, sce = c + e;
    const R rr = Mx<R>::rcp48(sab * sce);
    R rs = (a - b) * sce * rr, rp = (c - e) * sab * rr;
    R k = Nr * cos_i - cos_t;
    refr[0] = d[0] * Nr + nf[0] * k;
    refr[1] = d[1] * Nr + nf[1] * k;
    refr[2] = d[2] * Nr + nf[2] * k;
    const R inv = Mx<R>::rsqrt_pos(refr[0] * refr[0] + refr[1] * refr[1] + refr[2] * refr[2]);
    refr[0] *= inv; refr[1] *= inv; refr[2] *= inv;
    *cos_t_out = cos_t;
    return (R)0.5 * (rs * rs + rp * rp);
}

template <typename R> LT_DEV R boundary_planar(R uz, R n1, R n2, R Nr, R* cos_t_out)
{
    const R cos_i = Mx<R>::abs(uz);
    if (n1 == n2) { *cos_t_out = cos_i; return 0; }
    const R rad = (R)1 - Nr * Nr * ((R)1 - cos_i * cos_i);
    if (rad <= 0) { *cos_t_out = 0; return 1; }
    const R cos_t = Mx<R>::sqrt_pos(rad);
    const R a = n1 * cos_i, b = n2 * cos_t, c = n1 * cos_t, e = n2 * cos_i;
    const R sab = a + b, sce = c + e;
    const R r = Mx<R>::rcp48(sab * sce);
    const R rs = (a - b) * sce * r, rp = (c - e) * sab * r;
    *cos_t_out = cos_t;
    return (R)0.5 * (rs * rs + rp * rp);
}

template <typename R, bool TABLE> LT_DEV void spin(R* u, R ct, typename HeldU<R, TABLE>::type xi_phi, const double* T)
{
    const R st2 = Mx<R>::max0((R)1 - ct * ct);
    R sp, cp; HeldU<R, TABLE>::sincos_turn(xi_phi, T, &sp, &cp);
    R ux = u[0], uy = u[1], uz = u[2];
    if (Mx<R>::abs(uz) > (R)0.99999) {
        const R st = Mx<R>::sqrt_unit(st2);
        u[0] = st * cp; u[1] = st * sp; u[2] = uz >= 0 ? ct : -ct;
    } else {
        const R t2 = (R)1 - uz * uz;
        const R a = st2 * Mx<R>::rsqrt_pos(Mx<R>::max_tiny(st2 * t2));
        const R sc = a * cp, ss = a * sp;
        const R k = uz * sc + ct;
        u[0] = ux * k - uy * ss;
        u[1] = uy * k + ux * ss;
        u[2] = uz * ct - sc * t2;
    }
}

LT_DEV unsigned long long mix64(unsigned long long z)
{
    z = (z ^ (z >> 30)) * 0xBF58476D1CE4E5B9ull;
    z = (z ^ (z >> 27)) * 0x94D049BB133111EBull;
    return z ^ (z >> 31);
}
LT_DEV unsigned long long mix_seed(unsigned long long seed, unsigned long long photon_id)
{
    return mix64(mix64(seed + 0x9E3779B97F4A7C15ull) ^ ((photon_id + 1ull) * 0x9E3779B97F4A7C15ull));
}

constexpr int kRngWarmup = 8;
LT_DEV void photon_stream(unsigned long long seed, unsigned long long photon_id, rocrand_state_xorwow* st)
{
    rocrand_init(mix_seed(seed, photon_id), 0ull, 0ull, st);
#pragma unroll
    for (int k = 0; k < kRngWarmup; k++) (void)rocrand(st);
}

template <int TALLY> struct TallyT { typedef double type; };
template <> struct TallyT<LT_TALLY_F32> { typedef float type; };
template <> struct TallyT<LT_TALLY_U64FX> { typedef unsigned long long type; };
#define LT_TALLY_NONE 3

template <int TALLY, typename R> LT_DEV typename TallyT<TALLY>::type tally_quantum(R dw)
{
    if constexpr (TALLY == LT_TALLY_U64FX) return (unsigned long long)((double)dw * LT_FX_SCALE + 0.5);
    else return (typename TallyT<TALLY>::type)dw;
}

template <int TALLY> LT_DEV void tally_add(void* grid, unsigned idx, typename TallyT<TALLY>::type v)
{
    if constexpr (TALLY == LT_TALLY_NONE) { asm volatile("" ::"v"(idx), "v"(v)); }
    else
        __hip_atomic_fetch_add(reinterpret_cast<typename TallyT<TALLY>::type*>(grid) + idx, v, __ATOMIC_RELAXED,
                               __HIP_MEMORY_SCOPE_AGENT);
}

LT_DEV size_t align16(size_t x) { return (x + 15) & ~(size_t)15; }

template <typename R> struct LdsLayout {
    size_t off_cnt, off_frame, off_media, off_zb, off_if, off_lm, off_tris, off_nodes, off_links, off_hist, off_march, off_math, total;
    __host__ __device__ LdsLayout(int n_media, int n_layers, int n_tris, int n_nodes, unsigned n_hist = 0, size_t march_bytes = 0)
    {
        auto al = [](size_t x) { return (x + 15) & ~(size_t)15; };
        size_t o = 0;
        off_cnt = o;   o = al(o + 8 * sizeof(double));
        off_frame = o; o = al(o + 15 * sizeof(R));
        off_media = o; o = al(o + (size_t)n_media * sizeof(MedD<R>));
        off_zb = o;    o = al(o + (size_t)(n_layers + 1) * sizeof(R));
        off_if = o;    o = al(o + (size_t)(n_layers > 0 ? n_layers + 1 : 0) * sizeof(IfD<R>));
        off_lm = o;    o = al(o + (size_t)(n_layers > 0 ? n_layers : 1) * sizeof(int32_t));
        off_tris = o;  o = al(o + (size_t)n_tris * sizeof(TriD<R>));
        off_nodes = o; o = al(o + (size_t)n_nodes * sizeof(NodeD<R>));
        off_links = o; o = al(o + (size_t)n_nodes * 16 * sizeof(int16_t));
        off_hist = o;  o = al(o + (size_t)n_hist * sizeof(uint32_t));
        off_march = o; o = al(o + march_bytes);
        off_math = o;  o = al(o + (sizeof(R) == 8 ? kWalkMathTabBytes : 0));
        total = o;
    }
};

LT_DEV void lds_copy(void* dst, const void* src, size_t bytes)
{
    uint32_t* d = reinterpret_cast<uint32_t*>(dst);
    const uint32_t* s = reinterpret_cast<const uint32_t*>(src);
    for (size_t i = threadIdx.x; i < bytes / 4; i += blockDim.x) d[i] = s[i];
}

LT_DEV unsigned long long readlane64(unsigned long long v, int lane)
{
    unsigned lo = __builtin_amdgcn_readlane((unsigned)v, lane);
    unsigned hi = __builtin_amdgcn_readlane((unsigned)(v >> 32), lane);
    return ((unsigned long long)hi << 32) | lo;
}

template <typename T> LT_DEV T wave_sum(T v)
{
#pragma unroll
    for (int off = 32; off > 0; off >>= 1) v += __shfl_down(v, off, 64);
    return v;
}

template <typename R>
LT_DEV void record_vertex(const WalkParams& P, unsigned long long rel, unsigned& nv, R px, R py, R pz, R ux, R uy,
                          R uz, R w, int kind, int medium, unsigned step, R gx, R gy, R gz, R pdf_pos, R pdf_dir)
{
    if (nv < P.max_vertices) {
        lt_vertex* v = P.vertices + rel * (unsigned long long)P.max_vertices + nv;
        v->point[0] = (double)px; v->point[1] = (double)py; v->point[2] = (double)pz;
        v->direction[0] = (double)ux; v->direction[1] = (double)uy; v->direction[2] = (double)uz;
        v->g_norm[0] = (double)gx; v->g_norm[1] = (double)gy; v->g_norm[2] = (double)gz;
        v->throughput = (double)w; v->pdf_pos = (double)pdf_pos; v->pdf_dir = (double)pdf_dir;
        v->kind = kind; v->medium = medium; v->step = step; v->pad_ = 0;
        nv++;
        P.vertex_counts[rel] = nv;
    }
}

constexpr unsigned kLogExhausted = 0xfffffffeu;
template <int TALLY>
LT_DEV void emit_deposit(const WalkParams& P, bool has, unsigned idx, typename TallyT<TALLY>::type val,
                         unsigned& lg_cur, unsigned& lg_end, unsigned& lg_chunk, uint32_t* s_hist)
{
    typedef typename TallyT<TALLY>::type TV;
    if (P.log_idx == nullptr) {
        if (has) tally_add<TALLY>(P.grid, idx, val);
        return;
    }
    const unsigned long long m = __ballot(has);
    if (m == 0ull) return;
    const unsigned cnt = (unsigned)__popcll(m);
    if (lg_chunk != kLogExhausted && lg_end - lg_cur < cnt) {
        const int lane = threadIdx.x & 63;
        const unsigned grp = blockIdx.x & (kLogGroups - 1);
        if (lg_chunk < kLogExhausted && lane == 0) P.log_fill[lg_chunk] = lg_cur - lg_chunk * kLogChunk;
        unsigned c = 0;
        if (lane == 0) c = __hip_atomic_fetch_add(P.log_next + grp, 1u, __ATOMIC_RELAXED, __HIP_MEMORY_SCOPE_AGENT);
        c = grp + kLogGroups * __builtin_amdgcn_readfirstlane(c);
        if (c < P.log_cap_chunks) { lg_chunk = c; lg_cur = c * kLogChunk; lg_end = lg_cur + kLogChunk; }
        else { lg_chunk = kLogExhausted; lg_cur = lg_end = 0; }
    }
    if (lg_chunk == kLogExhausted) {
        if ((threadIdx.x & 63) == 0) __hip_atomic_fetch_add(P.log_overflow, cnt, __ATOMIC_RELAXED, __HIP_MEMORY_SCOPE_AGENT);
        if (has) {
            unsigned ntx = P.log_ntx, nty = P.log_nty;
            asm volatile("" : "+s"(ntx), "+s"(nty));
            const unsigned tile = idx >> kTileShift, tx = tile % ntx, ty = (tile / ntx) % nty,
                           tz = tile / (ntx * nty);
            const unsigned vx = (tx << kTileBX) | (idx & 31u), vy = (ty << kTileBY) | ((idx >> 5) & 31u),
                           vz = (tz << kTileBZ) | ((idx >> 10) & 15u);
            tally_add<TALLY>(P.grid, (vz * (unsigned)P.ny + vy) * (unsigned)P.nx + vx, val);
        }
        return;
    }
    if (has) {
        const unsigned rank = __builtin_amdgcn_mbcnt_hi((unsigned)(m >> 32), __builtin_amdgcn_mbcnt_lo((unsigned)m, 0u));
        P.log_idx[lg_cur + rank] = idx;
        reinterpret_cast<TV*>(P.log_val)[lg_cur + rank] = val;
        atomicAdd(&s_hist[idx >> P.log_hist_shift], 1u);
    }
    lg_cur += cnt;
}

constexpr unsigned kPacket = 64;
#ifndef LT_REFILL_MIN
#define LT_REFILL_MIN 4
#endif
constexpr unsigned kRefillMin = LT_REFILL_MIN;
#ifndef LT_QUERY_MIN
#define LT_QUERY_MIN 8
#endif
constexpr unsigned kQueryMin = LT_QUERY_MIN;
constexpr unsigned kQueryMinGlobal = 48;
#ifndef LT_QUERY_MAX_AGE
#define LT_QUERY_MAX_AGE 8
#endif
constexpr unsigned kQueryMaxAge = LT_QUERY_MAX_AGE;
#ifndef LT_MARCH_DRAIN_MIN
#define LT_MARCH_DRAIN_MIN 8
#endif
constexpr unsigned kMarchDrainMin = LT_MARCH_DRAIN_MIN;

#ifndef LT_F64_WAVES
#define LT_F64_WAVES 4
#endif
#ifndef LT_F64_GLOBAL_WAVES
#define LT_F64_GLOBAL_WAVES 3
#endif
#ifndef LT_F64_SLAB_WAVES
#define LT_F64_SLAB_WAVES 4
#endif
#ifndef LT_F32_WAVES
#define LT_F32_WAVES 5
#endif
#ifndef LT_INV_MODE_SLAB
#define LT_INV_MODE_SLAB 1
#endif
#ifndef LT_INV_MODE_MESH
#define LT_INV_MODE_MESH 2
#endif
#ifndef LT_INV_MODE_MARCH
#define LT_INV_MODE_MARCH 2
#endif
#define LT_INV_MODE LT_INV_MODE_SLAB
#define LT_WALK_NAME walk_kernel
#define LT_WALK_BATCH 0
#include "lt_walk_kernel.inc"
#undef LT_WALK_NAME
#undef LT_WALK_BATCH
#undef LT_INV_MODE
#define LT_INV_MODE LT_INV_MODE_MESH
#define LT_WALK_NAME walk_kernel_q
#define LT_WALK_BATCH 1
#include "lt_walk_kernel.inc"
#undef LT_WALK_NAME
#undef LT_WALK_BATCH
#undef LT_INV_MODE
#define LT_INV_MODE LT_INV_MODE_MARCH
#define LT_WALK_NAME walk_kernel_m
#define LT_WALK_BATCH 2
#include "lt_walk_kernel.inc"
#undef LT_WALK_NAME
#undef LT_WALK_BATCH
#undef LT_INV_MODE

typedef void (*WalkFn)(const WalkParams);

template <typename R, int GEOM, bool TABLE, bool CAPTURE>
static WalkFn pick_tally(int tally)
{
    switch (tally) {
    case LT_TALLY_F32:
        if constexpr (TABLE) return nullptr;
        else if constexpr (GEOM == 0) return walk_kernel<R, GEOM, TABLE, LT_TALLY_F32, CAPTURE>;
        else return walk_kernel_q<R, GEOM, TABLE, LT_TALLY_F32, CAPTURE>;
    case LT_TALLY_F64:
        if constexpr (GEOM == 0) return walk_kernel<R, GEOM, TABLE, LT_TALLY_F64, CAPTURE>;
        else return walk_kernel_q<R, GEOM, TABLE, LT_TALLY_F64, CAPTURE>;
    case LT_TALLY_U64FX:
        if constexpr (GEOM == 0) return walk_kernel<R, GEOM, TABLE, LT_TALLY_U64FX, CAPTURE>;
        else return walk_kernel_q<R, GEOM, TABLE, LT_TALLY_U64FX, CAPTURE>;
    case LT_TALLY_NONE:
        if constexpr (!TABLE && GEOM == 0 && !CAPTURE) return walk_kernel<R, GEOM, TABLE, LT_TALLY_NONE, false>; else return nullptr;
    }
    return nullptr;
}

template <typename R, bool CAPTURE>
static WalkFn pick_march(int tally)
{
    switch (tally) {
    case LT_TALLY_F32: return walk_kernel_m<R, 2, false, LT_TALLY_F32, CAPTURE>;
    case LT_TALLY_F64: return walk_kernel_m<R, 2, false, LT_TALLY_F64, CAPTURE>;
    case LT_TALLY_U64FX: return walk_kernel_m<R, 2, false, LT_TALLY_U64FX, CAPTURE>;
    }
    return nullptr;
}

template <typename R, bool TABLE, bool CAPTURE>
static WalkFn pick_geom(const Variant& v)
{
    if (v.mesh == 3) { if constexpr (!TABLE) return pick_march<R, CAPTURE>(v.tally); else return nullptr; }
    if (v.mesh == 0) return pick_tally<R, 0, TABLE, CAPTURE>(v.tally);
    if (v.mesh == 1) return pick_tally<R, 1, TABLE, CAPTURE>(v.tally);
    if constexpr (!TABLE) return pick_tally<R, 2, TABLE, CAPTURE>(v.tally); else return nullptr;
}

template <typename R, int PHASE>
static WalkFn pick_phase(int tally)
{
    switch (tally) {
    case LT_TALLY_F32: return walk_kernel<R, 0, false, LT_TALLY_F32, false, PHASE>;
    case LT_TALLY_F64: return walk_kernel<R, 0, false, LT_TALLY_F64, false, PHASE>;
    case LT_TALLY_U64FX: return walk_kernel<R, 0, false, LT_TALLY_U64FX, false, PHASE>;
    }
    return nullptr;
}

template <typename R, int PHASE>
static WalkFn pick_phase_q(int tally)
{
    switch (tally) {
    case LT_TALLY_F32: return walk_kernel_q<R, 1, false, LT_TALLY_F32, false, PHASE>;
    case LT_TALLY_F64: return walk_kernel_q<R, 1, false, LT_TALLY_F64, false, PHASE>;
    case LT_TALLY_U64FX: return walk_kernel_q<R, 1, false, LT_TALLY_U64FX, false, PHASE>;
    }
    return nullptr;
}

static WalkFn pick(const Variant& v)
{
    if (v.phase) {
        if (v.mesh > 1 || v.table || v.capture) return nullptr;
        if (v.mesh == 1) {
            if (v.phase == 1) return v.f32 ? pick_phase_q<float, 1>(v.tally) : pick_phase_q<double, 1>(v.tally);
            return v.f32 ? pick_phase_q<float, 2>(v.tally) : pick_phase_q<double, 2>(v.tally);
        }
        if (v.phase == 1) return v.f32 ? pick_phase<float, 1>(v.tally) : pick_phase<double, 1>(v.tally);
        return v.f32 ? pick_phase<float, 2>(v.tally) : pick_phase<double, 2>(v.tally);
    }
    if (v.capture) return (v.f32 || v.table) ? nullptr : pick_geom<double, false, true>(v);
    if (v.f32) return v.table ? nullptr : pick_geom<float, false, false>(v);
    return v.table ? pick_geom<double, true, false>(v) : pick_geom<double, false, false>(v);
}

size_t walk_lds_bytes(const Variant& v, int n_media, int n_layers, int n_tris, int n_nodes, unsigned n_hist)
{
    if (v.mesh) n_layers = 0;
    if (v.mesh != 1) { n_tris = 0; n_nodes = 0; }
    return v.f32 ? LdsLayout<float>(n_media, n_layers, n_tris, n_nodes, n_hist, v.mesh == 3 ? 4 * sizeof(MarchWave<float>) : 0).total
                 : LdsLayout<double>(n_media, n_layers, n_tris, n_nodes, n_hist, v.mesh == 3 ? 4 * sizeof(MarchWave<double>) : 0).total;
}

int walk_max_blocks_per_cu(const Variant& v, int threads, size_t lds_bytes)
{
    WalkFn fn = pick(v);
    if (!fn) return 0;
    int nb = 0;
    if (hipOccupancyMaxActiveBlocksPerMultiprocessor(&nb, reinterpret_cast<const void*>(fn), threads, lds_bytes) != hipSuccess)
        return 0;
    return nb;
}

hipError_t launch_walk(const WalkParams& Pin, const Variant& v, const LaunchCfg& cfg, hipStream_t s)
{
    WalkFn fn = pick(v);
    if (!fn) return hipErrorInvalidValue;
    WalkParams P = Pin;
    if (v.mesh) P.n_layers = 0; else { P.n_tris = 0; P.n_nodes = 0; }
    if (cfg.lds_bytes > 64 * 1024) {
        hipError_t e = hipFuncSetAttribute(reinterpret_cast<const void*>(fn),
                                           hipFuncAttributeMaxDynamicSharedMemorySize, (int)cfg.lds_bytes);
        if (e != hipSuccess) return e;
    }
    hipLaunchKernelGGL(fn, dim3(cfg.blocks), dim3(cfg.threads), cfg.lds_bytes, s, P);
    return hipGetLastError();
}

__global__ void k_intersect_rays(const TriD<double>* tris, const NodeD<double>* nodes, int n_tris, int n_nodes,
                                 const double* o, const double* d, const double* tmax, size_t n, int use_bvh,
                                 const MarchGrid G, const int16_t* links, int32_t* prim, double* t)
{
    size_t i = (size_t)blockIdx.x * blockDim.x + threadIdx.x;
    if (use_bvh == 2) {
        __shared__ MarchWave<double> mw[4];
        const bool want = i < n;
        const size_t k = want ? i : 0;
        int pi; double tt;
        march_service<double>(tris, nodes, n_nodes, G, &mw[threadIdx.x >> 6], want, o[3 * k], o[3 * k + 1], o[3 * k + 2], d[3 * k], d[3 * k + 1],
                              d[3 * k + 2], tmax ? tmax[k] : __builtin_huge_val(), 0.0, pi, tt);
        if (want) { prim[i] = pi; t[i] = tt; }
        return;
    }
    if (i >= n) return;
    double oo[3] = {o[3 * i], o[3 * i + 1], o[3 * i + 2]}, dd[3] = {d[3 * i], d[3 * i + 1], d[3 * i + 2]};
    double tm = tmax ? tmax[i] : __builtin_huge_val();
    int pi; double tt;
    if (use_bvh == 4) nearest_bvh_ordered(tris, nodes, n_nodes, links + ray_octant(dd) * 2 * n_nodes, oo, dd, tm, pi, tt);
    else if (use_bvh == 3) nearest_march(tris, nodes, n_nodes, G, oo, dd, tm, 0.0, pi, tt);
    else if (use_bvh) nearest_bvh(tris, nodes, n_nodes, oo, dd, tm, pi, tt);
    else nearest_brute(tris, n_tris, oo, dd, tm, pi, tt);
    prim[i] = pi; t[i] = tt;
}

__global__ void k_triangle_intersect(const double* o, const double* d, const double* tris, size_t n, double* t)
{
    size_t i = (size_t)blockIdx.x * blockDim.x + threadIdx.x;
    if (i >= n) return;
    const double* a = tris + 9 * i; const double* b = a + 3; const double* c = a + 6;
    TriD<double> T;
    {
#pragma clang fp contract(off)
        for (int k = 0; k < 3; k++) { T.a[k] = a[k]; T.ab[k] = b[k] - a[k]; T.ac[k] = c[k] - a[k]; }
        double nn[3];
        nn[0] = T.ab[1] * T.ac[2] - T.ab[2] * T.ac[1];
        nn[1] = T.ab[2] * T.ac[0] - T.ab[0] * T.ac[2];
        nn[2] = T.ab[0] * T.ac[1] - T.ab[1] * T.ac[0];
        double l = ::sqrt(nn[0] * nn[0] + nn[1] * nn[1] + nn[2] * nn[2]);
        for (int k = 0; k < 3; k++) T.n[k] = nn[k] / l;
    }
    T.med_front = T.med_back = -1;
    double oo[3] = {o[3 * i], o[3 * i + 1], o[3 * i + 2]}, dd[3] = {d[3 * i], d[3 * i + 1], d[3 * i + 2]};
    t[i] = tri_hit(oo, dd, &T);
}

__global__ void k_intersect_bounds(const double* o, const double* d, const double* tmax, const double* boxes,
                                   size_t n, int32_t* hit)
{
    size_t i = (size_t)blockIdx.x * blockDim.x + threadIdx.x;
    if (i >= n) return;
    double oo[3] = {o[3 * i], o[3 * i + 1], o[3 * i + 2]};
    double inv[3] = {1.0 / d[3 * i], 1.0 / d[3 * i + 1], 1.0 / d[3 * i + 2]};
    double lo[3] = {boxes[6 * i], boxes[6 * i + 1], boxes[6 * i + 2]};
    double hi[3] = {boxes[6 * i + 3], boxes[6 * i + 4], boxes[6 * i + 5]};
    hit[i] = box_hit(lo, hi, oo, inv, tmax ? tmax[i] : __builtin_huge_val()) ? 1 : 0;
}

__global__ void k_eval(int fn, const double* in, size_t n, double* out)
{
    size_t i = (size_t)blockIdx.x * blockDim.x + threadIdx.x;
    if (i >= n) return;
    switch (fn) {
    case LT_FN_HG_PDF: out[i] = hg_pdf(in[2 * i], in[2 * i + 1]); break;
    case LT_FN_HG_SAMPLE: {
        double g = in[2 * i + 1];
        out[i] = hg_sample(in[2 * i], g, 1.0 - g * g, 1.0 + g * g, 1.0 / (2.0 * g));
    } break;
    case LT_FN_ONB: {
        double nn[3] = {in[3 * i], in[3 * i + 1], in[3 * i + 2]}, v2[3], v3[3];
        onb(nn, v2, v3);
        for (int k = 0; k < 3; k++) { out[6 * i + k] = v2[k]; out[6 * i + 3 + k] = v3[k]; }
    } break;
    case LT_FN_DISK: { double dd[2]; disk(in[2 * i], in[2 * i + 1], dd); out[2 * i] = dd[0]; out[2 * i + 1] = dd[1]; } break;
    case LT_FN_COSINE_HEMI: {
        double nn[3] = {in[8 * i], in[8 * i + 1], in[8 * i + 2]}, wi[3] = {in[8 * i + 3], in[8 * i + 4], in[8 * i + 5]}, o4[4];
        cosine_hemi(nn, wi, in[8 * i + 6], in[8 * i + 7], o4);
        for (int k = 0; k < 4; k++) out[4 * i + k] = o4[k];
    } break;
    case LT_FN_REFLECT: {
        double v[3] = {in[6 * i], in[6 * i + 1], in[6 * i + 2]}, nn[3] = {in[6 * i + 3], in[6 * i + 4], in[6 * i + 5]}, r[3];
        reflect(v, nn, r);
        for (int k = 0; k < 3; k++) out[3 * i + k] = r[k];
    } break;
    case LT_FN_BOUNDARY: {
        double dd[3] = {in[8 * i], in[8 * i + 1], in[8 * i + 2]}, nf[3] = {in[8 * i + 3], in[8 * i + 4], in[8 * i + 5]}, ct, refr[3];
        out[5 * i] = boundary(dd, nf, in[8 * i + 6], in[8 * i + 7], &ct, refr);
        out[5 * i + 1] = ct; out[5 * i + 2] = refr[0]; out[5 * i + 3] = refr[1]; out[5 * i + 4] = refr[2];
    } break;
    case LT_FN_SPIN: {
        double u[3] = {in[5 * i], in[5 * i + 1], in[5 * i + 2]};
        spin<double, true>(u, in[5 * i + 3], in[5 * i + 4], kWalkMathTab);
        for (int k = 0; k < 3; k++) out[3 * i + k] = u[k];
    } break;
    case LT_FN_WALK_MATH: {
        const double x = in[i];
        out[5 * i] = neg_log_tab(x, kWalkMathTab);
        sincos_turn_tab(x, kWalkMathTab, &out[5 * i + 1], &out[5 * i + 2]);
        out[5 * i + 3] = sqrt01(x);
        out[5 * i + 4] = fast_div(1.0, 1.0 + x);
    } break;
    case LT_FN_WALK_MATH_RAW: {
        const unsigned k = (unsigned)in[i];
        out[3 * i] = neg_log_raw(k, kWalkMathTab);
        sincos_turn_raw(k, kWalkMathTab, &out[3 * i + 1], &out[3 * i + 2]);
    } break;
    }
}

__global__ void k_rng_raw(unsigned long long seed, unsigned long long photon_id, unsigned count, uint32_t* out)
{
    if (blockIdx.x != 0 || threadIdx.x != 0) return;
    rocrand_state_xorwow st;
    photon_stream(seed, photon_id, &st);
    for (unsigned i = 0; i < count; i++) out[i] = rocrand(&st);
}

__global__ void k_grid_to_f64(const void* grid, int tally, size_t n, double* out)
{
    for (size_t i = (size_t)blockIdx.x * blockDim.x + threadIdx.x; i < n; i += (size_t)gridDim.x * blockDim.x) {
        if (tally == LT_TALLY_F32) out[i] = (double)reinterpret_cast<const float*>(grid)[i];
        else if (tally == LT_TALLY_F64) out[i] = reinterpret_cast<const double*>(grid)[i];
        else out[i] = (double)reinterpret_cast<const unsigned long long*>(grid)[i] * (1.0 / LT_FX_SCALE);
    }
}

template <typename T>
__global__ void __launch_bounds__(256) k_grid_add(T* __restrict__ dst, const T* __restrict__ src, size_t n)
{
    constexpr size_t kV = 16 / sizeof(T);
    struct alignas(16) V { T v[kV]; };
    const size_t nv = n / kV;
    for (size_t i = (size_t)blockIdx.x * blockDim.x + threadIdx.x; i < nv; i += (size_t)gridDim.x * blockDim.x) {
        V a = reinterpret_cast<V*>(dst)[i];
        const V b = reinterpret_cast<const V*>(src)[i];
#pragma unroll
        for (size_t k = 0; k < kV; k++) a.v[k] += b.v[k];
        reinterpret_cast<V*>(dst)[i] = a;
    }
    for (size_t i = nv * kV + (size_t)blockIdx.x * blockDim.x + threadIdx.x; i < n; i += (size_t)gridDim.x * blockDim.x) dst[i] += src[i];
}
// ... 568 lines not shown
```

light_transport_amd/csrc/lt_walk_kernel.inc:

```
#ifndef LT_MED
#define LT_MED(i) reinterpret_cast<const MedD<R>*>(reinterpret_cast<const unsigned char*>(s_med) + __umul24((unsigned)(i), (unsigned)sizeof(MedD<R>)))
#endif
#if LT_WALK_BATCH != 2
template <typename R, int GEOM, bool TABLE, int TALLY, bool CAPTURE, int PHASE = 0>
#else
template <typename R, int GEOM, bool TABLE, int TALLY, bool CAPTURE>
#endif
#if LT_WALK_BATCH == 0 && defined(LT_SLAB_VGPR_CAP)
__attribute__((amdgpu_num_vgpr(LT_SLAB_VGPR_CAP)))
#endif
__global__ void __launch_bounds__(256, (sizeof(R) == 8 ? (GEOM == 0 ? LT_F64_SLAB_WAVES : (GEOM == 2 ? LT_F64_GLOBAL_WAVES : LT_F64_WAVES)) : (GEOM == 0 ? LT_F32_WAVES : 4))) LT_WALK_NAME(const WalkParams P)
{
    constexpr bool MESH = GEOM != 0;
#if LT_WALK_BATCH == 2
    constexpr int PHASE = 0;
#endif
#if LT_WALK_PRIO
    __builtin_amdgcn_s_setprio(LT_WALK_PRIO);
#endif
    extern __shared__ __attribute__((aligned(16))) unsigned char lds_raw[];
    const LdsLayout<R> L(P.n_media, P.n_layers, GEOM == 1 ? P.n_tris : 0, GEOM == 1 ? P.n_nodes : 0,
                         P.log_idx ? P.log_n_hist : 0u, LT_WALK_BATCH == 2 ? 4 * sizeof(MarchWave<R>) : 0);
    uint32_t* s_hist = reinterpret_cast<uint32_t*>(lds_raw + L.off_hist);
    if (P.log_idx) for (unsigned t = threadIdx.x; t < P.log_n_hist; t += blockDim.x) s_hist[t] = 0;
    double* s_cnt = reinterpret_cast<double*>(lds_raw + L.off_cnt);
    const MedD<R>* s_med = reinterpret_cast<const MedD<R>*>(lds_raw + L.off_media);
    const R* s_zb = reinterpret_cast<const R*>(lds_raw + L.off_zb);
    const int32_t* s_lm = reinterpret_cast<const int32_t*>(lds_raw + L.off_lm);
    const IfD<R>* s_if = reinterpret_cast<const IfD<R>*>(lds_raw + L.off_if);
    const TriD<R>* s_tris = GEOM == 2 ? reinterpret_cast<const TriD<R>*>(P.tris)
                                      : reinterpret_cast<const TriD<R>*>(lds_raw + L.off_tris);
    const NodeD<R>* s_nodes = GEOM == 2 ? reinterpret_cast<const NodeD<R>*>(P.nodes)
                                        : reinterpret_cast<const NodeD<R>*>(lds_raw + L.off_nodes);

    const int16_t* s_links = !MESH || !P.links ? nullptr
                             : (GEOM == 1 ? reinterpret_cast<const int16_t*>(lds_raw + L.off_links) : P.links);
    if (threadIdx.x < 8) s_cnt[threadIdx.x] = 0.0;
    R* s_frame = reinterpret_cast<R*>(lds_raw + L.off_frame);
    if (threadIdx.x == 64 % blockDim.x && P.src_type == LT_SRC_COSINE_QUAD) {
        const R nrm[3] = {(R)P.src_dir[0], (R)P.src_dir[1], (R)P.src_dir[2]};
        R v2[3], v3[3];
        onb(nrm, v2, v3);
#pragma unroll
        for (int k = 0; k < 3; k++) { s_frame[k] = v2[k]; s_frame[3 + k] = v3[k]; }
    }
#if LT_INV_MODE == 2
    const R* s_inv = s_frame + 6;
    if (threadIdx.x == 128 % blockDim.x) {
#pragma unroll
        for (int k = 0; k < 3; k++) { s_frame[6 + k] = LT_PV(origin, k); s_frame[9 + k] = LT_PV(inv_voxel, k); s_frame[12 + k] = LT_PV(fdim, k); }
    }
#endif
    const double* s_math = reinterpret_cast<const double*>(lds_raw + L.off_math);
    if constexpr (sizeof(R) == 8) lds_copy(lds_raw + L.off_math, kWalkMathTab, kWalkMathTabBytes);
    lds_copy(lds_raw + L.off_media, P.media, (size_t)P.n_media * sizeof(MedD<R>));
    if constexpr (!MESH) {
        lds_copy(lds_raw + L.off_zb, P.zb, (size_t)(P.n_layers + 1) * sizeof(R));
        lds_copy(lds_raw + L.off_lm, P.layer_medium, (size_t)P.n_layers * sizeof(int32_t));
        lds_copy(lds_raw + L.off_if, P.ifaces, (size_t)(P.n_layers + 1) * sizeof(IfD<R>));
    } else if constexpr (GEOM == 1) {
        lds_copy(lds_raw + L.off_tris, P.tris, (size_t)P.n_tris * sizeof(TriD<R>));
        lds_copy(lds_raw + L.off_nodes, P.nodes, (size_t)P.n_nodes * sizeof(NodeD<R>));
        if (P.links) lds_copy(lds_raw + L.off_links, P.links, (size_t)P.n_nodes * 16 * sizeof(int16_t));
    }
    __syncthreads();

    const R eps = (R)1e-6;
    const R inf = Mx<R>::inf();
    const int lane = threadIdx.x & 63;

    bool alive = false;
    R px = 0, py = 0, pz = 0, ux = 0, uy = 0, uz = 1, w = 0, sleft = 0;
    int cur = 0;
    unsigned step = 0, max_steps = P.max_steps, nv = 0;
    unsigned long long pid = 0, grp = 0;
    rocrand_state_xorwow rng;
    double acc_abs = 0.0, acc_lost = 0.0;
    unsigned long long acc_steps = 0;
    typedef typename TallyT<TALLY>::type TV;
    constexpr unsigned kNoVoxel = 0xffffffffu;
    unsigned pend_idx = kNoVoxel;
    TV pend_val = 0;
    unsigned lg_cur = 0, lg_end = 0, lg_chunk = kNoVoxel;
    unsigned long long pk_next = 0, pk_end = 0;
    bool q_done = false;
    bool dumped = false;
#if LT_WALK_BATCH
    bool q_pend = false;
#if LT_WALK_BATCH == 1
    typename HeldU<R, TABLE>::type q_u1 = 0, q_u2 = 0, q_u3 = 0;
#endif
#if LT_WALK_BATCH == 2
    R q_tc = 0;
    bool q_march = false, q_dirty = false, q_bvh = false;
    unsigned mq_n = 0;
    MarchWave<R>* const mw = reinterpret_cast<MarchWave<R>*>(lds_raw + L.off_march) + (threadIdx.x >> 6);
#endif
#if defined(LT_DIAG_MESH)
    unsigned long long dg_iter = 0, dg_alive = 0, dg_prep = 0, dg_wait = 0, dg_trav_it = 0, dg_trav = 0, dg_go = 0, dg_bnd_it = 0, dg_bnd = 0,
                       dg_int_it = 0, dg_int = 0, dg_refill_it = 0, dg_refill = 0, dg_bvh_it = 0, dg_bvh = 0, dg_l4_it = 0, dg_l4 = 0;
    unsigned long long dg_clk_srv = 0, dg_clk_bnd = 0, dg_clk_all = clock64();
    unsigned long long dgm_clk[4] = {0, 0, 0, 0};
#endif
#endif

#if LT_WALK_BATCH == 1
    const unsigned query_min = P.query_min ? P.query_min : (GEOM == 2 ? kQueryMinGlobal : kQueryMin);
    unsigned q_age = 0;
#elif LT_WALK_BATCH == 2
    const unsigned drain_min = P.query_min ? P.query_min : kMarchDrainMin;
#endif
#if LT_INV_MODE == 2
#define gx0 s_inv[0]
#define gy0 s_inv[1]
#define gz0 s_inv[2]
#define ivx s_inv[3]
#define ivy s_inv[4]
#define ivz s_inv[5]
#define fnx s_inv[6]
#define fny s_inv[7]
#define fnz s_inv[8]
#else
    R gx0 = LT_PV(origin, 0), gy0 = LT_PV(origin, 1), gz0 = LT_PV(origin, 2);
    R ivx = LT_PV(inv_voxel, 0), ivy = LT_PV(inv_voxel, 1), ivz = LT_PV(inv_voxel, 2);
    [[maybe_unused]] const R fnx = LT_PV(fdim, 0), fny = LT_PV(fdim, 1), fnz = LT_PV(fdim, 2);
#if LT_INV_MODE == 1
    asm volatile("" : "+v"(gx0), "+v"(gy0), "+v"(gz0), "+v"(ivx), "+v"(ivy), "+v"(ivz));
#endif
#endif

    if constexpr (PHASE == 2) {
        q_done = true;
        const unsigned have = *P.pool_n < P.pool_cap ? *P.pool_n : P.pool_cap;
        const unsigned e = (blockIdx.x * (blockDim.x >> 6) + (threadIdx.x >> 6)) * 64u + (unsigned)lane;
        if (e < have) {
            const SurvD<R>& S = reinterpret_cast<const SurvD<R>*>(P.pool)[e];
            px = S.p[0]; py = S.p[1]; pz = S.p[2]; ux = S.u[0]; uy = S.u[1]; uz = S.u[2]; w = S.w; sleft = S.sleft;
            cur = S.cur; step = S.step;
            __builtin_memcpy(&rng, S.rng, sizeof S.rng);
            alive = true;
#if LT_WALK_BATCH == 1
            if constexpr (!TABLE) {
                q_pend = S.q_pend != 0u;
                q_u1 = __builtin_bit_cast(typename HeldU<R, TABLE>::type, S.held[0]);
                q_u2 = __builtin_bit_cast(typename HeldU<R, TABLE>::type, S.held[1]);
                q_u3 = __builtin_bit_cast(typename HeldU<R, TABLE>::type, S.held[2]);
            }
#endif
        }
    }
    for (;;) {
        unsigned long long need = __ballot(!alive);
        if (need != 0ull && !(q_done && pk_next >= pk_end) &&
            ((unsigned)__popcll(need) >= kRefillMin || need == __ballot(true))) {
            const unsigned cnt = (unsigned)__popcll(need);
#if LT_WALK_BATCH && defined(LT_DIAG_MESH)
            dg_refill_it++; dg_refill += cnt;
#endif
            const unsigned rank = __builtin_amdgcn_mbcnt_hi((unsigned)(need >> 32),
                                      __builtin_amdgcn_mbcnt_lo((unsigned)need, 0u));
            const unsigned long long avail = pk_end - pk_next;
            unsigned long long nlo = 0, nhi = 0;
            if (cnt > avail && !q_done) {
                const int leader = __ffsll((long long)need) - 1;
                unsigned long long base = 0;
                if (lane == leader)
                    base = __hip_atomic_fetch_add(P.head, (unsigned long long)kPacket, __ATOMIC_RELAXED,
                                                  __HIP_MEMORY_SCOPE_AGENT);
                base = readlane64(base, leader);
                nlo = base < P.n_photons ? base : P.n_photons;
                nhi = base + kPacket < P.n_photons ? base + kPacket : P.n_photons;
                if (nhi >= P.n_photons) q_done = true;
            }
            bool got = false;
            unsigned long long id = 0;
            if (!alive) {
                if (rank < avail) { id = pk_next + rank; got = true; }
                else if (rank - avail < nhi - nlo) { id = nlo + (rank - avail); got = true; }
            }
            if (cnt <= avail) pk_next += cnt;
            else {
                unsigned long long used = cnt - avail;
                if (used > nhi - nlo) used = nhi - nlo;
                pk_next = nlo + used; pk_end = nhi;
            }

            if (got) {
                pid = P.photon_offset + id;
                alive = true; w = 1; sleft = 0; step = 0; grp = 0;
                R e_pdf_dir = 1;
                max_steps = P.max_steps;
                if constexpr (!TABLE) photon_stream(P.seed, pid, &rng);
                if (P.src_type == LT_SRC_COSINE_QUAD) {
                    R u4[4];
                    if constexpr (TABLE) {
                        const double* t = P.table + (id * P.table_steps + grp) * 4;
#pragma unroll
                        for (int k = 0; k < 4; k++) u4[k] = (R)(1.0 - t[k]);
                    } else {
#pragma unroll
                        for (int k = 0; k < 4; k++) u4[k] = Mx<R>::uniform32(&rng);
                    }
                    grp++;
                    R nrm[3] = {(R)P.src_dir[0], (R)P.src_dir[1], (R)P.src_dir[2]};
                    R wi[3] = {-nrm[0], -nrm[1], -nrm[2]};
                    R o4[4];
                    {
                        const R v2[3] = {s_frame[0], s_frame[1], s_frame[2]}, v3[3] = {s_frame[3], s_frame[4], s_frame[5]};
                        cosine_hemi_frame(nrm, v2, v3, wi, u4[2], u4[3], o4);
                    }
                    e_pdf_dir = Mx<R>::abs(o4[0] * nrm[0] + o4[1] * nrm[1] + o4[2] * nrm[2]) * (R)0.3183098861837907;
                    ux = o4[0]; uy = o4[1]; uz = o4[2];
                    px = (R)P.src_pos[0] + u4[0] * (R)P.src_e1[0] + u4[1] * (R)P.src_e2[0] + eps * o4[0];
                    py = (R)P.src_pos[1] + u4[0] * (R)P.src_e1[1] + u4[1] * (R)P.src_e2[1] + eps * o4[1];
                    pz = (R)P.src_pos[2] + u4[0] * (R)P.src_e1[2] + u4[1] * (R)P.src_e2[2] + eps * o4[2];
                } else {
                    px = (R)P.src_pos[0]; py = (R)P.src_pos[1]; pz = (R)P.src_pos[2];
                    ux = (R)P.src_dir[0]; uy = (R)P.src_dir[1]; uz = (R)P.src_dir[2];
                }
                if constexpr (!MESH) {
                    cur = -1;
                    for (int l = 0; l < P.n_layers; l++)
                        if (pz >= s_zb[l] && pz < s_zb[l + 1]) { cur = l; break; }
                    if (cur < 0) {
                        atomicAdd(&s_cnt[CW_ESC_TOP], (double)w); alive = false;
                    } else if (P.src_type == LT_SRC_PENCIL && pz == s_zb[0] && uz > 0) {
                        R n2 = s_med[s_lm[0]].n, n1 = (R)P.n_above;
                        if (n1 != n2) {
                            R d[3] = {ux, uy, uz}, nf[3] = {0, 0, -1}, ct, refr[3];
                            R Rs = boundary(d, nf, n1, n2, &ct, refr);
                            atomicAdd(&s_cnt[CW_SPECULAR], (double)(w * Rs));
                            w -= w * Rs;
                            if (!(w > 0)) alive = false;
                            ux = refr[0]; uy = refr[1]; uz = refr[2];
                        }
                    }
                } else {
                    cur = P.start_medium;
                }
                nv = 0;
                if constexpr (CAPTURE) if (P.vertices) {
                    P.vertex_counts[id] = 0;
                    if (alive) {
                        R pdf_pos = 1;
                        if (P.src_type == LT_SRC_COSINE_QUAD) {
                            const R e1[3] = {(R)P.src_e1[0], (R)P.src_e1[1], (R)P.src_e1[2]}, e2[3] = {(R)P.src_e2[0], (R)P.src_e2[1], (R)P.src_e2[2]};
                            R cr[3]; cross3(e1, e2, cr);
                            pdf_pos = (R)1 / Mx<R>::sqrt(dot3(cr, cr));
                        }
                        record_vertex<R>(P, id, nv, px, py, pz, ux, uy, uz, w, LT_VERTEX_LIGHT, cur, 0u, (R)P.src_dir[0], (R)P.src_dir[1],
                                         (R)P.src_dir[2], pdf_pos, e_pdf_dir);
                    }
                }
                if constexpr (TABLE) {
                    unsigned long long cap = P.table_steps > grp ? P.table_steps - grp : 0ull;
                    if (cap < (unsigned long long)max_steps) max_steps = (unsigned)cap;
                }
            }
        }
        if constexpr (PHASE == 1) {
            if (q_done && pk_next >= pk_end && !dumped) {
                const unsigned long long am = __ballot(alive);
                const unsigned na = (unsigned)__popcll(am);
                if (na != 0u && na <= P.dump_max) {
                    emit_deposit<TALLY>(P, pend_idx != kNoVoxel, pend_idx, pend_val, lg_cur, lg_end, lg_chunk, s_hist);
                    pend_idx = kNoVoxel;
                    const int leader = __ffsll((long long)am) - 1;
                    unsigned base = 0;
                    if (lane == leader) base = __hip_atomic_fetch_add(P.pool_n, na, __ATOMIC_RELAXED, __HIP_MEMORY_SCOPE_AGENT);
                    base = (unsigned)__builtin_amdgcn_readlane((int)base, leader);
                    if (alive) {
                        const unsigned slot = base + __builtin_amdgcn_mbcnt_hi((unsigned)(am >> 32), __builtin_amdgcn_mbcnt_lo((unsigned)am, 0u));
                        if (slot < P.pool_cap) {
                            SurvD<R>& S = reinterpret_cast<SurvD<R>*>(P.pool)[slot];
                            S.p[0] = px; S.p[1] = py; S.p[2] = pz; S.u[0] = ux; S.u[1] = uy; S.u[2] = uz; S.w = w; S.sleft = sleft;
                            S.pid = 0ull; S.cur = cur; S.step = step;
                            __builtin_memcpy(S.rng, &rng, sizeof S.rng);
#if LT_WALK_BATCH == 1
                            if constexpr (!TABLE) {
                                S.q_pend = q_pend ? 1u : 0u;
                                S.held[0] = __builtin_bit_cast(uint32_t, q_u1); S.held[1] = __builtin_bit_cast(uint32_t, q_u2);
                                S.held[2] = __builtin_bit_cast(uint32_t, q_u3);
                                q_pend = false;
                            }
#else
                            S.q_pend = 0u;
#endif
                            alive = false;
                        }
                    }
                    dumped = true;
                }
            }
        }
        if (!__any(alive)) break;

#if LT_WALK_BATCH == 2
        unsigned f_idx = kNoVoxel;
        TV f_val = 0;
        bool go = false;
        R u1 = 0, s = 0, tb = inf;
        typename HeldU<R, TABLE>::type x2 = 0, x3 = 0;
        int hit_tri = -1;
#if defined(LT_DIAG_MESH)
        const long long dgm_t0 = clock64();
        dg_iter++; dg_alive += __popcll(__ballot(alive)); dg_prep += __popcll(__ballot(alive && !q_pend));
#endif
        if (alive && !q_pend) {
            if (step >= max_steps) {
                atomicAdd(&s_cnt[CW_CAPPED], (double)w); alive = false;
            } else {
                step++;
                acc_steps++;
                const float clr = march_clearance<R>(P.mg, px, py, pz);
                const typename HeldU<R, TABLE>::type x0 = HeldU<R, TABLE>::draw(&rng);
                u1 = Mx<R>::uniform32(&rng);
                x2 = HeldU<R, TABLE>::draw(&rng);
                x3 = HeldU<R, TABLE>::draw(&rng);
                grp++;
                const MedD<R>* Mq = LT_MED(cur);
                if (sleft == 0) sleft = HeldU<R, TABLE>::neg_log(x0, s_math);
                s = (Mq->mu_t > 0) ? sleft * Mq->inv_mu_t : inf;
                if (!(s < (R)clr)) {
                    q_pend = true;
                    mw->held[0][lane] = s; mw->held[1][lane] = u1; mw->held[2][lane] = HeldU<R, TABLE>::as_real(x2); mw->held[3][lane] = HeldU<R, TABLE>::as_real(x3);
                    q_tc = clr > 0.0f ? (R)clr : (R)0;
                    q_march = march_enter<R>(P.mg, mw, px, py, pz, ux, uy, uz, s);
                    q_bvh = !q_march; q_dirty = false;
                } else go = true;
            }
        }
        {
            bool full = false;
#if defined(LT_DIAG_MESH)
            const long long dgm_t1 = clock64();
            dgm_clk[0] += dgm_t1 - dgm_t0;
            { const unsigned long long m_ = __ballot(q_march); if (m_) { dg_trav_it++; dg_trav += __popcll(m_); } }
#endif
            if (__any(q_march)) {
                bool heavy = false;
                full = march_round<R>(P.mg, mw, q_march, heavy, q_dirty, q_tc, mq_n);
                q_bvh = q_bvh || heavy;
            }
#if defined(LT_DIAG_MESH)
            const long long dgm_t2 = clock64();
            dgm_clk[1] += dgm_t2 - dgm_t1;
#endif
            const unsigned long long wm = __ballot(q_pend && !q_march && q_dirty);
            if (mq_n > 0 && (full || mq_n >= 64u || (unsigned)__popcll(wm) >= drain_min || !__any(go || q_march))) {
#if defined(LT_DIAG_MESH)
                dg_bvh_it++; dg_bvh += mq_n;
#endif
                march_drain<R>(s_tris, P.mg, mw, mq_n);
                q_dirty = false;
            }
#if defined(LT_DIAG_MESH)
            const long long dgm_t3 = clock64();
            dgm_clk[2] += dgm_t3 - dgm_t2;
#endif
            if (q_pend && !q_march && !q_dirty) {
                s = mw->held[0][lane]; u1 = mw->held[1][lane]; x2 = HeldU<R, TABLE>::from_real(mw->held[2][lane]); x3 = HeldU<R, TABLE>::from_real(mw->held[3][lane]);
                R th;
                march_result<R>(s_tris, s_nodes, P.n_nodes, s_links, mw, q_bvh, px, py, pz, ux, uy, uz, s, hit_tri, th);
                if (hit_tri >= 0) tb = th;
                q_pend = false; q_bvh = false; go = true;
            }
#if defined(LT_DIAG_MESH)
            dgm_clk[3] += clock64() - dgm_t3;
#endif
        }
#if defined(LT_DIAG_MESH)
        const long long dg_t1 = clock64();
        {
            const unsigned long long gm = __ballot(go), bm = __ballot(go && hit_tri >= 0);
            dg_go += __popcll(gm);
            if (bm) { dg_bnd_it++; dg_bnd += __popcll(bm); }
            if (gm & ~bm) { dg_int_it++; dg_int += __popcll(gm & ~bm); }
        }
#endif
        if (go) {
            {
                const MedD<R>* Mp = LT_MED(cur);
                const R mu_t = Mp->mu_t;
#elif LT_WALK_BATCH
        unsigned f_idx = kNoVoxel;
        TV f_val = 0;
        bool go = false;
        R u1 = 0, s = 0, tb = inf;
        typename HeldU<R, TABLE>::type x2 = 0, x3 = 0;
        int hit_tri = -1;
#if defined(LT_DIAG_MESH)
        dg_iter++; dg_alive += __popcll(__ballot(alive)); dg_prep += __popcll(__ballot(alive && !(MESH && q_pend)));
#endif
        if (alive && !(MESH && q_pend)) {
            if (step >= max_steps) {
                atomicAdd(&s_cnt[CW_CAPPED], (double)w); alive = false;
            } else {
                step++;
                acc_steps++;
                float clr = -1.0f;
                unsigned rec_y = 0u, rec_z = 0xffffffffu;
                if constexpr (GEOM == 2) {
                    if (P.mg.cell) clr = march_clearance<R>(P.mg, px, py, pz);
                } else if constexpr (MESH) {
                    if (P.clear) {
                        const R cx = (px - LT_PV(corg, 0)) * LT_PV(cinv, 0), cy = (py - LT_PV(corg, 1)) * LT_PV(cinv, 1),
                                cz = (pz - LT_PV(corg, 2)) * LT_PV(cinv, 2);
                        if (cx >= 0 && cx < LT_PV(cdim, 0) && cy >= 0 && cy < LT_PV(cdim, 1) && cz >= 0 && cz < LT_PV(cdim, 2)) {
                            const uint4 rec = P.clear[((size_t)(int)cz * P.cny + (int)cy) * P.cnx + (int)cx];
                            clr = __uint_as_float(rec.x); rec_y = rec.y; rec_z = rec.z;
                        }
                    }
                }
                typename HeldU<R, TABLE>::type x0, h1, h2, h3;
                if constexpr (TABLE) {
                    const double* t = P.table + ((pid - P.photon_offset) * P.table_steps + grp) * 4;
                    x0 = (R)(1.0 - t[0]); h1 = (R)(1.0 - t[1]); h2 = (R)(1.0 - t[2]); h3 = (R)(1.0 - t[3]);
                } else if constexpr (sizeof(R) == 8) {
                    x0 = rocrand(&rng); h1 = rocrand(&rng); h2 = rocrand(&rng); h3 = rocrand(&rng);
                } else {
                    x0 = Mx<R>::uniform32(&rng); h1 = Mx<R>::uniform32(&rng); h2 = Mx<R>::uniform32(&rng); h3 = HeldU<R, TABLE>::draw(&rng);
                }
                u1 = HeldU<R, TABLE>::get(h1); x2 = h2; x3 = h3;
                grp++;
                const MedD<R>* Mq = LT_MED(MESH ? cur : s_lm[cur]);
                if (sleft == 0) sleft = HeldU<R, TABLE>::neg_log(x0, s_math);
                s = (Mq->mu_t > 0) ? sleft * Mq->inv_mu_t : inf;

                if constexpr (!MESH) {
                    if (uz != 0) {
                        const R dz = (uz > 0 ? s_zb[cur + 1] : s_zb[cur]) - pz;
                        const R guard = sizeof(R) == 8 ? (R)(1.0 + 1e-12) : (R)(1.0 + 1e-5);
                        const bool near = !(Mx<R>::abs(dz) > s * Mx<R>::abs(uz) * guard);
                        if (__any(near)) {
                            R den = uz;
                            asm volatile("" : "+v"(den));
                            if (near) tb = dz / den;
                        }
                    }
                    go = true;
                } else {
                    if (!(s < (R)clr)) {
                        bool need = true;
                        if constexpr (GEOM == 1) {
                            const float c2 = (float)__builtin_bit_cast(_Float16, (unsigned short)(rec_y & 0xffffu));
                            if (s < (R)c2) {
                                const unsigned i0 = rec_z & 0xffffu, i1 = rec_z >> 16;
                                need = (i0 != 0xffffu && plane_within_reach(&s_tris[i0], px, py, pz, ux, uy, uz, s)) ||
                                       (i1 != 0xffffu && plane_within_reach(&s_tris[i1], px, py, pz, ux, uy, uz, s));
                            }
                        }
                        if (need) { q_pend = true; q_u1 = h1; q_u2 = h2; q_u3 = h3; }
                        else go = true;
                    } else go = true;
                }
            }
        }
        if constexpr (MESH) {
            const unsigned long long wq = __ballot(q_pend);
#if defined(LT_DIAG_MESH)
            if (wq != 0ull && ((unsigned)__popcll(wq) >= query_min || q_age + 1 > kQueryMaxAge || !__any(go))) { dg_trav_it++; dg_trav += __popcll(wq); }
            else dg_wait += __popcll(wq);
#endif
            if (wq != 0ull) q_age++;
            if (wq != 0ull && ((unsigned)__popcll(wq) >= query_min || q_age > kQueryMaxAge || !__any(go))) {
                q_age = 0;
#if defined(LT_DIAG_MESH)
                const long long dg_t0 = clock64();
#endif
                if (q_pend) {
                    {
                        const MedD<R>* Mq = LT_MED(MESH ? cur : s_lm[cur]);
                        s = (Mq->mu_t > 0) ? sleft * Mq->inv_mu_t : inf;
                    }
                    u1 = HeldU<R, TABLE>::get(q_u1); x2 = q_u2; x3 = q_u3;
                    R o[3] = {px, py, pz}, d[3] = {ux, uy, uz}, th;
                    if constexpr (GEOM == 2) {
                        nearest_bvh_walk(s_tris, s_nodes, P.n_nodes, s_links, o, d, s, hit_tri, th);
                    } else {
                    uint4 rec = make_uint4(0u, 0u, 0xffffffffu, 0xffffffffu);
                    if (P.clear) {
                        const R cx = (px - LT_PV(corg, 0)) * LT_PV(cinv, 0), cy = (py - LT_PV(corg, 1)) * LT_PV(cinv, 1),
                                cz = (pz - LT_PV(corg, 2)) * LT_PV(cinv, 2);
                        if (cx >= 0 && cx < LT_PV(cdim, 0) && cy >= 0 && cy < LT_PV(cdim, 1) && cz >= 0 && cz < LT_PV(cdim, 2))
                            rec = P.clear[((size_t)(int)cz * P.cny + (int)cy) * P.cnx + (int)cx];
                    }
#if defined(LT_DIAG_MESH)
                    {
                        const float c2_ = (float)__builtin_bit_cast(_Float16, (unsigned short)(rec.y & 0xffffu));
                        const float c4_ = (float)__builtin_bit_cast(_Float16, (unsigned short)(rec.y >> 16));
                        const unsigned long long fb = __ballot(!(s < (R)c4_)), f4 = __ballot(!(s < (R)c2_) && s < (R)c4_);
                        if (fb) { dg_bvh_it++; dg_bvh += __popcll(fb); }
                        if (f4) { dg_l4_it++; dg_l4 += __popcll(f4); }
                    }
#endif
                    nearest_listed(s_tris, s_nodes, P.n_nodes, s_links, rec, o, d, s, hit_tri, th);
                    }
                    if (hit_tri >= 0) tb = th;
                    q_pend = false; go = true;
                }
#if defined(LT_DIAG_MESH)
                dg_clk_srv += clock64() - dg_t0;
#endif
            }
        }
#if defined(LT_DIAG_MESH)
        {
            const unsigned long long gm = __ballot(go), bm = __ballot(go && hit_tri >= 0);
            dg_go += __popcll(gm);
            if (bm) { dg_bnd_it++; dg_bnd += __popcll(bm); }
            if (gm & ~bm) { dg_int_it++; dg_int += __popcll(gm & ~bm); }
        }
#endif
#if defined(LT_DIAG_MESH)
        const long long dg_t1 = clock64();
#endif
        if (go) {
            {
                const MedD<R>* Mp = LT_MED(MESH ? cur : s_lm[cur]);
                const R mu_t = Mp->mu_t;
#else
        unsigned f_idx = kNoVoxel;
        TV f_val = 0;
        if (alive) {
            if (step >= max_steps) {
                atomicAdd(&s_cnt[CW_CAPPED], (double)w); alive = false;
            } else {
                step++;
                acc_steps++;
                float clr = -1.0f;
                if constexpr (GEOM == 2) {
                    if (P.mg.cell) clr = march_clearance<R>(P.mg, px, py, pz);
                } else if constexpr (MESH) {
                    if (P.clear) {
                        const R cx = (px - LT_PV(corg, 0)) * LT_PV(cinv, 0), cy = (py - LT_PV(corg, 1)) * LT_PV(cinv, 1),
                                cz = (pz - LT_PV(corg, 2)) * LT_PV(cinv, 2);
                        if (cx >= 0 && cx < LT_PV(cdim, 0) && cy >= 0 && cy < LT_PV(cdim, 1) && cz >= 0 && cz < LT_PV(cdim, 2))
                            clr = __uint_as_float(P.clear[((size_t)(int)cz * P.cny + (int)cy) * P.cnx + (int)cx].x);
                    }
                }
                R u1;
                typename HeldU<R, TABLE>::type x0, x2, x3;
                if constexpr (TABLE) {
                    const double* t = P.table + ((pid - P.photon_offset) * P.table_steps + grp) * 4;
                    x0 = (R)(1.0 - t[0]); u1 = (R)(1.0 - t[1]); x2 = (R)(1.0 - t[2]); x3 = (R)(1.0 - t[3]);
                } else {
                    x0 = HeldU<R, TABLE>::draw(&rng);
                    u1 = Mx<R>::uniform32(&rng);
                    x2 = HeldU<R, TABLE>::draw(&rng);
                    x3 = HeldU<R, TABLE>::draw(&rng);
                }
                grp++;
                const MedD<R>* Mp = LT_MED(MESH ? cur : s_lm[cur]);
                const R mu_t = Mp->mu_t;
                if (sleft == 0) sleft = HeldU<R, TABLE>::neg_log(x0, s_math);
                const R s = (mu_t > 0) ? sleft * Mp->inv_mu_t : inf;

                R tb = inf; int hit_tri = -1;
                if constexpr (!MESH) {
                    if (uz != 0) {
                        const R dz = (uz > 0 ? s_zb[cur + 1] : s_zb[cur]) - pz;
                        const R guard = sizeof(R) == 8 ? (R)(1.0 + 1e-12) : (R)(1.0 + 1e-5);
                        const bool near = !(Mx<R>::abs(dz) > s * Mx<R>::abs(uz) * guard);
                        if (__any(near)) {
                            R den = uz;
                            asm volatile("" : "+v"(den));
                            if (near) tb = dz / den;
                        }
                    }
                } else {
                    const bool query = !(s < (R)clr);
                    if (query) {
                        R o[3] = {px, py, pz}, d[3] = {ux, uy, uz}, th;
                        nearest_bvh_walk(s_tris, s_nodes, P.n_nodes, s_links, o, d, s, hit_tri, th);
                        if (hit_tri >= 0) tb = th;
                    }
                }
#endif
                const bool at_boundary = MESH ? (hit_tri >= 0) : (tb <= s);
                if (!at_boundary && !(s < inf)) {
                    atomicAdd(&s_cnt[MESH ? CW_ESC_MESH : CW_CAPPED], (double)w); alive = false;
                } else if (at_boundary) {
                    px += ux * tb; py += uy * tb; pz += uz * tb;
                    sleft -= tb * mu_t;
                    if (!(sleft > 0)) sleft = 0;
                    if constexpr (!MESH) {
                        const bool down = uz > 0;
                        const int k = down ? cur + 1 : cur, next = down ? cur + 1 : cur - 1;
                        pz = s_zb[k];
                        const IfD<R> F = s_if[k];
                        const R Nr = down ? F.nr_down : F.nr_up;
                        R ct;
                        const R Rf = boundary_planar(uz, down ? F.n_up : F.n_dn, down ? F.n_dn : F.n_up, Nr, &ct);
                        const bool refl = HeldU<R, TABLE>::get(x3) <= Rf;
                        const bool gone = !refl && (next < 0 || next >= P.n_layers);
                        if constexpr (CAPTURE) if (P.vertices)
                            record_vertex<R>(P, pid - P.photon_offset, nv, px, py, pz, ux, uy, uz, w,
                                             refl ? LT_VERTEX_REFLECTIVE : LT_VERTEX_TRANSMISSIVE, cur, step, (R)0, (R)0, down ? (R)-1 : (R)1, (R)0,
                                             gone ? (R)0 : (refl ? Rf : (R)1 - Rf));
                        if (refl) uz = -uz;
                        else if (gone) { atomicAdd(&s_cnt[next < 0 ? CW_ESC_TOP : CW_ESC_BOT], (double)w); alive = false; }
                        else { ux *= Nr; uy *= Nr; uz = down ? ct : -ct; cur = next; }
                    } else {
                    R nf[3], n1 = Mp->n, n2; int next;
                    {
                        const TriD<R>* T = &s_tris[hit_tri];
                        R tn[3] = {T->n[0], T->n[1], T->n[2]};
                        R d[3] = {ux, uy, uz};
                        R dn = dot3(d, tn);
                        R sg = dn > 0 ? (R)-1 : (R)1;
                        nf[0] = sg * tn[0]; nf[1] = sg * tn[1]; nf[2] = sg * tn[2];
                        next = dn > 0 ? T->med_front : T->med_back;
                        n2 = next >= 0 ? s_med[next].n : n1;
                    }
                    R d[3] = {ux, uy, uz}, ct, refr[3];
                    R Rf = boundary(d, nf, n1, n2, &ct, refr);
                    if constexpr (CAPTURE) if (P.vertices) {
                        const bool refl = HeldU<R, TABLE>::get(x3) <= Rf;
                        const bool leaves = !refl && next < 0;
                        record_vertex<R>(P, pid - P.photon_offset, nv, px, py, pz, ux, uy, uz, w,
                                         refl ? LT_VERTEX_REFLECTIVE : LT_VERTEX_TRANSMISSIVE, cur, step, nf[0], nf[1], nf[2], (R)0,
                                         leaves ? (R)0 : (refl ? Rf : (R)1 - Rf));
                    }
                    if (HeldU<R, TABLE>::get(x3) <= Rf) {
                        R ro[3]; reflect_walk(d, nf, ro);
                        ux = ro[0]; uy = ro[1]; uz = ro[2];
                        px += eps * nf[0]; py += eps * nf[1]; pz += eps * nf[2];
                    } else if (next < 0) {
                        atomicAdd(&s_cnt[CW_ESC_MESH], (double)w); alive = false;
                    } else {
                        ux = refr[0]; uy = refr[1]; uz = refr[2];
                        px -= eps * nf[0]; py -= eps * nf[1]; pz -= eps * nf[2];
                        cur = next;
                    }
                    }
                } else {
                    px += ux * s; py += uy * s; pz += uz * s;
                    sleft = 0;
                    const R dw = w * Mp->absorb;
                    if constexpr (CAPTURE) if (P.vertices) {
                        const R ct_c = hg_sample_walk(u1, Mp);
                        record_vertex<R>(P, pid - P.photon_offset, nv, px, py, pz, ux, uy, uz, w, LT_VERTEX_VOLUME, cur, step, (R)0, (R)0, (R)0,
                                         (R)0, (w - dw > 0) ? hg_pdf(-ct_c, Mp->g) : (R)0);
                    }
                    const R fx = (px - gx0) * ivx, fy = (py - gy0) * ivy, fz = (pz - gz0) * ivz;
                    const unsigned vx = (unsigned)(int)fx, vy = (unsigned)(int)fy, vz = (unsigned)(int)fz;
                    bool inside;
                    if constexpr (!MESH) inside = (int)(Mx<R>::sign_word(fx) | Mx<R>::sign_word(fy) | Mx<R>::sign_word(fz)) >= 0 &&
                                                  vx < (unsigned)P.nx && vy < (unsigned)P.ny && vz < (unsigned)P.nz;
                    else inside = fx >= 0 && fx < fnx && fy >= 0 && fy < fny && fz >= 0 && fz < fnz;
                    const unsigned idx = P.log_idx
                        ? (((__umul24(__umul24(vz >> kTileBZ, P.log_nty) + (vy >> kTileBY), P.log_ntx) + (vx >> kTileBX)) << kTileShift)
                           | ((vz & 15u) << 10) | ((vy & 31u) << 5) | (vx & 31u))
                        : (vz * (unsigned)P.ny + vy) * (unsigned)P.nx + vx;
                    const TV q = tally_quantum<TALLY, R>(w * Mp->dep);
                    const bool same = inside && idx == pend_idx;
                    const bool flush = inside && !same;
                    f_idx = flush ? pend_idx : kNoVoxel; f_val = pend_val;
                    pend_val = same ? pend_val + q : (flush ? q : pend_val);
                    pend_idx = flush ? idx : pend_idx;
                    acc_abs += inside ? (double)dw : 0.0;
                    acc_lost += inside ? 0.0 : (double)dw;
                    w -= dw;
                    if (!(w > 0)) alive = false;
                    else {
                        R u[3] = {ux, uy, uz};
                        spin<R, TABLE>(u, hg_sample_walk(u1, Mp), x2, s_math);
                        ux = u[0]; uy = u[1]; uz = u[2];
                        if (w < (R)1e-4) {
                            if (HeldU<R, TABLE>::get(x3) <= (R)0.1) { atomicAdd(&s_cnt[CW_ROULETTE], -9.0 * (double)w); w *= (R)10; }
                            else { atomicAdd(&s_cnt[CW_ROULETTE], (double)w); alive = false; }
                        }
                    }
                }
            }
        }
#if LT_WALK_BATCH && defined(LT_DIAG_MESH)
        dg_clk_bnd += clock64() - dg_t1;
#endif
        emit_deposit<TALLY>(P, f_idx != kNoVoxel, f_idx, f_val, lg_cur, lg_end, lg_chunk, s_hist);
    }
    emit_deposit<TALLY>(P, pend_idx != kNoVoxel, pend_idx, pend_val, lg_cur, lg_end, lg_chunk, s_hist);
    if (P.log_idx && lg_chunk < kLogExhausted && (threadIdx.x & 63) == 0) P.log_fill[lg_chunk] = lg_cur - lg_chunk * kLogChunk;

#if LT_WALK_BATCH && defined(LT_DIAG_MESH)
#if LT_WALK_BATCH == 2
    if (blockIdx.x == 7 && threadIdx.x == 0) {
        const double tot = (double)(clock64() - dg_clk_all);
        printf("[march diag] iterations %llu, cycles per iteration %.0f | alive %.1f, preparing %.1f | share of the wave's time: prepare %.3f, march round %.3f "
               "(in %.3f of iterations, %.1f lanes), drain %.3f (in %.3f of iterations, %.1f items), resolve %.3f, complete %.3f | complete %.1f lanes: "
               "boundary in %.3f of iterations (%.1f lanes), interaction in %.3f (%.1f lanes) | refills %.3f of iterations (%.1f lanes)\n",
               dg_iter, tot / dg_iter, (double)dg_alive / dg_iter, (double)dg_prep / dg_iter, dgm_clk[0] / tot, dgm_clk[1] / tot, (double)dg_trav_it / dg_iter,
               dg_trav_it ? (double)dg_trav / dg_trav_it : 0.0, dgm_clk[2] / tot, (double)dg_bvh_it / dg_iter, dg_bvh_it ? (double)dg_bvh / dg_bvh_it : 0.0,
               dgm_clk[3] / tot, dg_clk_bnd / tot, (double)dg_go / dg_iter, (double)dg_bnd_it / dg_iter, dg_bnd_it ? (double)dg_bnd / dg_bnd_it : 0.0,
               (double)dg_int_it / dg_iter, dg_int_it ? (double)dg_int / dg_int_it : 0.0, (double)dg_refill_it / dg_iter, dg_refill_it ? (double)dg_refill / dg_refill_it : 0.0);
    }
#else
    if (blockIdx.x == 7 && threadIdx.x == 0) {
        const double tot = (double)(clock64() - dg_clk_all);
        printf("[mesh diag] cycles per service %.0f; share of the wave's time: services %.3f, complete-stage %.3f; cycles per iteration %.0f\n",
               dg_trav_it ? (double)dg_clk_srv / dg_trav_it : 0.0, dg_clk_srv / tot, dg_clk_bnd / tot, tot / dg_iter);
    }
#endif
    if (blockIdx.x == 7 && threadIdx.x == 0)
        printf("[mesh diag] iterations %llu | alive %.1f/64 | prepare %.1f | waiting for a query %.1f | traversals: %.3f of iterations, %.1f lanes each | "
               "complete %.1f lanes: boundary in %.3f of iterations (%.1f lanes), interaction in %.3f (%.1f lanes) | refills: %.3f of iterations, %.1f lanes | "
               "services with BVH lanes %.3f of iterations (%.1f lanes), with 4-triangle lanes %.3f (%.1f lanes)\n",
               dg_iter, (double)dg_alive / dg_iter, (double)dg_prep / dg_iter, (double)dg_wait / dg_iter, (double)dg_trav_it / dg_iter,
               dg_trav_it ? (double)dg_trav / dg_trav_it : 0.0, (double)dg_go / dg_iter, (double)dg_bnd_it / dg_iter,
               dg_bnd_it ? (double)dg_bnd / dg_bnd_it : 0.0, (double)dg_int_it / dg_iter, dg_int_it ? (double)dg_int / dg_int_it : 0.0,
               (double)dg_refill_it / dg_iter, dg_refill_it ? (double)dg_refill / dg_refill_it : 0.0,
               (double)dg_bvh_it / dg_iter, dg_bvh_it ? (double)dg_bvh / dg_bvh_it : 0.0, (double)dg_l4_it / dg_iter, dg_l4_it ? (double)dg_l4 / dg_l4_it : 0.0);
#endif
    const double wa = wave_sum(acc_abs), wl = wave_sum(acc_lost);
    const unsigned long long ws = wave_sum(acc_steps);
    if (lane == 0) {
        atomicAdd(&s_cnt[CW_ABSORBED], wa);
        atomicAdd(&s_cnt[CW_LOST], wl);
        __hip_atomic_fetch_add(&P.counters->steps, ws, __ATOMIC_RELAXED, __HIP_MEMORY_SCOPE_AGENT);
    }
    __syncthreads();
    if (P.log_idx)
        for (unsigned t = threadIdx.x; t < P.log_n_hist; t += blockDim.x)
            if (s_hist[t]) __hip_atomic_fetch_add(&P.log_hist[t * kLogGroups + (blockIdx.x & (kLogGroups - 1))], s_hist[t],
                                                  __ATOMIC_RELAXED, __HIP_MEMORY_SCOPE_AGENT);
    if (PHASE != 2 && blockIdx.x == 0 && threadIdx.x == 8)
        __hip_atomic_fetch_add(&P.counters->photons, P.n_photons, __ATOMIC_RELAXED, __HIP_MEMORY_SCOPE_AGENT);
    if (threadIdx.x < 8)
        __hip_atomic_fetch_add(&P.counters->w[threadIdx.x], s_cnt[threadIdx.x], __ATOMIC_RELAXED,
                               __HIP_MEMORY_SCOPE_AGENT);
}
#if LT_INV_MODE == 2
#undef gx0
#undef gy0
#undef gz0
#undef ivx
#undef ivy
#undef ivz
#undef fnx
#undef fny
#undef fnz
#endif
```

Before: 88.33 billion.

## Specialize slab walk kernel on log mode and pair-align medium reads

Adds a compile-time LOG template parameter to the slab walk kernel so deposit routing and histogram handling are resolved statically instead of testing P.log_idx at runtime. It also moves the math table and histogram to fixed LDS offsets at the front, reorders MedD into 16-byte-aligned pairs so they can be fetched with paired loads, and caches the current medium offset and next boundary z. Table cells for log and sincos lookups can be fetched early, separately from the arithmetic. Step accounting moves to photon termination. The cost is more kernel instantiations, stricter launch validation, and a changed MedD layout that the host packing must match.

After: 91.70 billion, median of 6. 1.04x the previous value.

```diff
diff --git a/light_transport_amd/csrc/lt_api.cpp b/light_transport_amd/csrc/lt_api.cpp
--- a/light_transport_amd/csrc/lt_api.cpp
+++ b/light_transport_amd/csrc/lt_api.cpp
@@ -769,7 +769,7 @@
             HIP_TRY(c, hipStreamWaitEvent(ln.tail_stream, ln.ev_bulk, 0));
             WalkParams Pt = P;
             Pt.log_idx = nullptr; Pt.log_val = nullptr; Pt.log_n_hist = 0;
-            Variant vt = R.v; vt.phase = 2;
+            Variant vt = R.v; vt.phase = 2; vt.log = 0;
             LaunchCfg ct = cfg;
             ct.lds_bytes = walk_lds_bytes(vt, P.n_media, P.n_layers, P.n_tris, P.n_nodes, 0);
             ct.blocks = (int)((P.pool_cap / 64u + (unsigned)(cfg.threads / 64) - 1) / (unsigned)(cfg.threads / 64));
@@ -1086,6 +1086,7 @@
     v.tally = c->tally;
     v.capture = c->max_vertices > 0 ? 1 : 0;
     v.phase = 0;
+    v.log = 0;
     if (v.capture && (v.f32 || v.table)) return c->fail(LT_E_UNSUPPORTED, "lt_launch: vertex capture runs the f64 walk with the XORWOW generator");
     if (c->on(c->knob.diag_no_tally)) v.tally = 3;
     if (v.table && v.f32) return c->fail(LT_E_UNSUPPORTED, "lt_launch: table RNG runs the f64 walk only");
@@ -1170,6 +1171,7 @@
     if (use_log) {
         LogRun R;
         R.c = c; R.P = P; R.v = v; R.cfg = cfg; R.G = G;
+        R.v.log = 1;
         if (c->dmap_valid && (c->dmap_tiles != G.n_tiles || c->dmap_bits2 != G.bits2)) c->dmap_valid = c->tile_cnt_ready = false;
         c->stages_valid = false;
         for (LogLane& ln : c->lanes) ln.ev_used = 0;
diff --git a/light_transport_amd/csrc/lt_internal.hpp b/light_transport_amd/csrc/lt_internal.hpp
--- a/light_transport_amd/csrc/lt_internal.hpp
+++ b/light_transport_amd/csrc/lt_internal.hpp
@@ -7,13 +7,16 @@
 namespace ltk {
 
 template <typename R>
-struct MedD {
-    R mu_t, inv_mu_t, absorb, g;
-    R n, one_m_g2, one_p_g2, inv_2g;
-    R dep;
+struct alignas(2 * sizeof(R)) MedD {
+    R mu_t, inv_mu_t;
+    R absorb, dep;
+    R g, inv_2g;
     R one_m_g, two_g;
+    R one_m_g2, one_p_g2;
+    R n;
     R pad_;
 };
+static_assert(sizeof(MedD<double>) == 96 && sizeof(MedD<float>) == 48, "MedD: six aligned pairs");
 
 template <typename R>
 struct IfD {
@@ -131,6 +134,7 @@
     int tally;
     int capture;
     int phase;
+    int log;
 };
 
 hipError_t launch_walk(const WalkParams& P, const Variant& v, const LaunchCfg& cfg, hipStream_t s);
diff --git a/light_transport_amd/csrc/lt_kernels.hip b/light_transport_amd/csrc/lt_kernels.hip
--- a/light_transport_amd/csrc/lt_kernels.hip
+++ b/light_transport_amd/csrc/lt_kernels.hip
@@ -207,7 +207,14 @@
     *cs = ((q + 1) & 2) ? -c1 : c1;
 }
 
-LT_DEV double neg_log_raw(unsigned k, const double* T)
+LT_DEV const double2* neg_log_raw_cell(unsigned k, const double* T)
+{
+    const unsigned nm = (k + 1u) << (__clz((int)(k + 1u)) & 31);
+    const unsigned sh = 24u + (nm >= 0xC0000000u ? 1u : 0u);
+    const unsigned j = ((nm >> (sh - 1u)) + 1u) >> 1;
+    return reinterpret_cast<const double2*>(T + 2 * ((int)(j < 96u ? 96u : j) - 96));
+}
+LT_DEV double neg_log_raw_at(unsigned k, const double2 Tj)
 {
     const unsigned n = k + 1u;
     const int lz = __clz((int)n);
@@ -217,7 +224,6 @@
     const unsigned j = ((nm >> (sh - 1u)) + 1u) >> 1;
     const int dint = (int)(nm - (j << sh));
     const double d = __builtin_ldexp((double)dint, -(int)sh);
-    const double2 Tj = *reinterpret_cast<const double2*>(T + 2 * ((int)j - 96));
     const double r = d * Tj.x;
     double p = 1.0 / 7.0;
     p = fma_k(p, r, -1.0 / 6.0); p = fma_k(p, r, 1.0 / 5.0); p = fma_k(p, r, -0.25); p = fma_k(p, r, 1.0 / 3.0);
@@ -227,7 +233,13 @@
     const double v = -fma_mk(de, 6.93147180369123816490e-01, fma_mk(de, 1.90821492927058770002e-10, lnm));
     return n == 0u ? 0.0 : v;
 }
-LT_DEV void sincos_turn_raw(unsigned k, const double* T, double* sn, double* cs)
+LT_DEV double neg_log_raw(unsigned k, const double* T) { return neg_log_raw_at(k, *neg_log_raw_cell(k, T)); }
+LT_DEV const double2* sincos_turn_raw_cell(unsigned k, const double* T)
+{
+    const unsigned iq = (((k + 1u) >> 25) + 1u) >> 1;
+    return reinterpret_cast<const double2*>(T + 2 * (kLnTabEntries + (int)(iq & (unsigned)(kScTabEntries - 1))));
+}
+LT_DEV void sincos_turn_raw_at(unsigned k, const double2 Ti, double* sn, double* cs)
 {
     const unsigned n = k + 1u;
     const unsigned iq = ((n >> 25) + 1u) >> 1;
@@ -243,10 +255,10 @@
     pc = fma_k(pc, z, 4.1666666666666666667e-02);
     pc = __builtin_fma(pc, z, -0.5);
     const double cd = __builtin_fma(pc, z, 1.0);
-    const double2 Ti = *reinterpret_cast<const double2*>(T + 2 * (kLnTabEntries + (int)(iq & (unsigned)(kScTabEntries - 1))));
     *sn = __builtin_fma(Ti.x, cd, Ti.y * sd);
     *cs = __builtin_fma(Ti.y, cd, -(Ti.x * sd));
 }
+LT_DEV void sincos_turn_raw(unsigned k, const double* T, double* sn, double* cs) { sincos_turn_raw_at(k, *sincos_turn_raw_cell(k, T), sn, cs); }
 template <typename R> struct Mx;
 template <> struct Mx<double> {
     static LT_DEV double log(double x) { return ::log(x); }
@@ -777,11 +789,14 @@
     return Mx<R>::clamp_unit(c);
 }
 
+template <typename R> struct alignas(2 * sizeof(R)) Pair { R a, b; };
+template <typename R> LT_DEV Pair<R> ld_pair(const R* p) { return *reinterpret_cast<const Pair<R>*>(p); }
 template <typename R> LT_DEV R hg_sample_walk(R xi, const MedD<R>* M)
 {
-    if (M->g == 0) return (R)2 * xi - (R)1;
-    const R t = Mx<R>::quot(M->one_m_g2, M->two_g * xi + M->one_m_g);
-    return (M->one_p_g2 - t * t) * M->inv_2g;
+    const Pair<R> gi = ld_pair(&M->g), den = ld_pair(&M->one_m_g), num = ld_pair(&M->one_m_g2);
+    if (gi.a == 0) return (R)2 * xi - (R)1;
+    const R t = Mx<R>::quot(num.a, den.b * xi + den.a);
+    return (num.b - t * t) * gi.b;
 }
 
 template <typename R> LT_DEV void onb(const R* n, R* v2, R* v3)
@@ -895,10 +910,15 @@
     return (R)0.5 * (rs * rs + rp * rp);
 }
 
+template <typename R> LT_DEV void spin_with(R* u, R ct, R sp, R cp);
 template <typename R, bool TABLE> LT_DEV void spin(R* u, R ct, typename HeldU<R, TABLE>::type xi_phi, const double* T)
 {
+    R sp, cp; HeldU<R, TABLE>::sincos_turn(xi_phi, T, &sp, &cp);
+    spin_with(u, ct, sp, cp);
+}
+template <typename R> LT_DEV void spin_with(R* u, R ct, R sp, R cp)
+{
     const R st2 = Mx<R>::max0((R)1 - ct * ct);
-    R sp, cp; HeldU<R, TABLE>::sincos_turn(xi_phi, T, &sp, &cp);
     R ux = u[0], uy = u[1], uz = u[2];
     if (Mx<R>::abs(uz) > (R)0.99999) {
         const R st = Mx<R>::sqrt_unit(st2);
@@ -954,14 +974,22 @@
 
 LT_DEV size_t align16(size_t x) { return (x + 15) & ~(size_t)15; }
 
-template <typename R> struct LdsLayout {
+template <typename R, bool FRONT = false> struct LdsLayout {
+    static constexpr size_t al(size_t x) { return (x + 15) & ~(size_t)15; }
+    static constexpr size_t kCntBytes = al(8 * sizeof(double));
+    static constexpr size_t kFrameBytes = al(15 * sizeof(R));
+    static constexpr size_t kMathBytes = al(sizeof(R) == 8 ? kWalkMathTabBytes : 0);
+    static constexpr size_t kOffCnt = 0, kOffFrame = kCntBytes, kOffMath = kOffFrame + kFrameBytes, kOffHist = kOffMath + kMathBytes;
     size_t off_cnt, off_frame, off_media, off_zb, off_if, off_lm, off_tris, off_nodes, off_links, off_hist, off_march, off_math, total;
     __host__ __device__ LdsLayout(int n_media, int n_layers, int n_tris, int n_nodes, unsigned n_hist = 0, size_t march_bytes = 0)
     {
-        auto al = [](size_t x) { return (x + 15) & ~(size_t)15; };
         size_t o = 0;
-        off_cnt = o;   o = al(o + 8 * sizeof(double));
-        off_frame = o; o = al(o + 15 * sizeof(R));
+        off_cnt = o;   o += kCntBytes;
+        off_frame = o; o += kFrameBytes;
+        if constexpr (FRONT) {
+            off_math = o; o += kMathBytes;
+            off_hist = o; o = al(o + (size_t)n_hist * sizeof(uint32_t));
+        }
         off_media = o; o = al(o + (size_t)n_media * sizeof(MedD<R>));
         off_zb = o;    o = al(o + (size_t)(n_layers + 1) * sizeof(R));
         off_if = o;    o = al(o + (size_t)(n_layers > 0 ? n_layers + 1 : 0) * sizeof(IfD<R>));
@@ -969,9 +997,9 @@
         off_tris = o;  o = al(o + (size_t)n_tris * sizeof(TriD<R>));
         off_nodes = o; o = al(o + (size_t)n_nodes * sizeof(NodeD<R>));
         off_links = o; o = al(o + (size_t)n_nodes * 16 * sizeof(int16_t));
-        off_hist = o;  o = al(o + (size_t)n_hist * sizeof(uint32_t));
+        if constexpr (!FRONT) { off_hist = o; o = al(o + (size_t)n_hist * sizeof(uint32_t)); }
         off_march = o; o = al(o + march_bytes);
-        off_math = o;  o = al(o + (sizeof(R) == 8 ? kWalkMathTabBytes : 0));
+        if constexpr (!FRONT) { off_math = o; o += kMathBytes; }
         total = o;
     }
 };
@@ -1014,12 +1042,12 @@
 }
 
 constexpr unsigned kLogExhausted = 0xfffffffeu;
-template <int TALLY>
+template <int TALLY, int ROUTE = -1>
 LT_DEV void emit_deposit(const WalkParams& P, bool has, unsigned idx, typename TallyT<TALLY>::type val,
                          unsigned& lg_cur, unsigned& lg_end, unsigned& lg_chunk, uint32_t* s_hist)
 {
     typedef typename TallyT<TALLY>::type TV;
-    if (P.log_idx == nullptr) {
+    if (ROUTE < 0 ? P.log_idx == nullptr : ROUTE == 0) {
         if (has) tally_add<TALLY>(P.grid, idx, val);
         return;
     }
@@ -1097,6 +1125,9 @@
 #endif
 #ifndef LT_INV_MODE_MARCH
 #define LT_INV_MODE_MARCH 2
+#endif
+#ifndef LT_SLAB_READS
+#define LT_SLAB_READS 2
 #endif
 #define LT_INV_MODE LT_INV_MODE_SLAB
 #define LT_WALK_NAME walk_kernel
@@ -1162,13 +1193,13 @@
     if constexpr (!TABLE) return pick_tally<R, 2, TABLE, CAPTURE>(v.tally); else return nullptr;
 }
 
-template <typename R, int PHASE>
+template <typename R, int PHASE, bool LOG>
 static WalkFn pick_phase(int tally)
 {
     switch (tally) {
-    case LT_TALLY_F32: return walk_kernel<R, 0, false, LT_TALLY_F32, false, PHASE>;
-    case LT_TALLY_F64: return walk_kernel<R, 0, false, LT_TALLY_F64, false, PHASE>;
-    case LT_TALLY_U64FX: return walk_kernel<R, 0, false, LT_TALLY_U64FX, false, PHASE>;
+    case LT_TALLY_F32: return walk_kernel<R, 0, false, LT_TALLY_F32, false, PHASE, LOG>;
+    case LT_TALLY_F64: return walk_kernel<R, 0, false, LT_TALLY_F64, false, PHASE, LOG>;
+    case LT_TALLY_U64FX: return walk_kernel<R, 0, false, LT_TALLY_U64FX, false, PHASE, LOG>;
     }
     return nullptr;
 }
@@ -1192,8 +1223,12 @@
             if (v.phase == 1) return v.f32 ? pick_phase_q<float, 1>(v.tally) : pick_phase_q<double, 1>(v.tally);
             return v.f32 ? pick_phase_q<float, 2>(v.tally) : pick_phase_q<double, 2>(v.tally);
         }
-        if (v.phase == 1) return v.f32 ? pick_phase<float, 1>(v.tally) : pick_phase<double, 1>(v.tally);
-        return v.f32 ? pick_phase<float, 2>(v.tally) : pick_phase<double, 2>(v.tally);
+        if (v.phase == 1) return !v.log ? nullptr : (v.f32 ? pick_phase<float, 1, true>(v.tally) : pick_phase<double, 1, true>(v.tally));
+        return v.log ? nullptr : (v.f32 ? pick_phase<float, 2, false>(v.tally) : pick_phase<double, 2, false>(v.tally));
+    }
+    if (v.mesh == 0 && v.log) {
+        if (v.table || v.capture) return nullptr;
+        return v.f32 ? pick_phase<float, 0, true>(v.tally) : pick_phase<double, 0, true>(v.tally);
     }
     if (v.capture) return (v.f32 || v.table) ? nullptr : pick_geom<double, false, true>(v);
     if (v.f32) return v.table ? nullptr : pick_geom<float, false, false>(v);
@@ -1204,6 +1239,8 @@
 {
     if (v.mesh) n_layers = 0;
     if (v.mesh != 1) { n_tris = 0; n_nodes = 0; }
+    if (v.mesh == 0)
+        return v.f32 ? LdsLayout<float, true>(n_media, n_layers, 0, 0, n_hist).total : LdsLayout<double, true>(n_media, n_layers, 0, 0, n_hist).total;
     return v.f32 ? LdsLayout<float>(n_media, n_layers, n_tris, n_nodes, n_hist, v.mesh == 3 ? 4 * sizeof(MarchWave<float>) : 0).total
                  : LdsLayout<double>(n_media, n_layers, n_tris, n_nodes, n_hist, v.mesh == 3 ? 4 * sizeof(MarchWave<double>) : 0).total;
 }
@@ -1222,6 +1259,7 @@
 {
     WalkFn fn = pick(v);
     if (!fn) return hipErrorInvalidValue;
+    if (v.mesh == 0 && (v.log != 0) != (Pin.log_idx != nullptr)) return hipErrorInvalidValue;
     WalkParams P = Pin;
     if (v.mesh) P.n_layers = 0; else { P.n_tris = 0; P.n_nodes = 0; }
     if (cfg.lds_bytes > 64 * 1024) {
diff --git a/light_transport_amd/csrc/lt_walk_kernel.inc b/light_transport_amd/csrc/lt_walk_kernel.inc
--- a/light_transport_amd/csrc/lt_walk_kernel.inc
+++ b/light_transport_amd/csrc/lt_walk_kernel.inc
@@ -1,7 +1,14 @@
 #ifndef LT_MED
 #define LT_MED(i) reinterpret_cast<const MedD<R>*>(reinterpret_cast<const unsigned char*>(s_med) + __umul24((unsigned)(i), (unsigned)sizeof(MedD<R>)))
 #endif
-#if LT_WALK_BATCH != 2
+#if LT_WALK_BATCH == 0
+#define LT_END_PHOTON() do { alive = false; acc_steps += step; } while (0)
+#else
+#define LT_END_PHOTON() do { alive = false; } while (0)
+#endif
+#if LT_WALK_BATCH == 0
+template <typename R, int GEOM, bool TABLE, int TALLY, bool CAPTURE, int PHASE = 0, bool LOG = false>
+#elif LT_WALK_BATCH != 2
 template <typename R, int GEOM, bool TABLE, int TALLY, bool CAPTURE, int PHASE = 0>
 #else
 template <typename R, int GEOM, bool TABLE, int TALLY, bool CAPTURE>
@@ -19,24 +26,36 @@
     __builtin_amdgcn_s_setprio(LT_WALK_PRIO);
 #endif
     extern __shared__ __attribute__((aligned(16))) unsigned char lds_raw[];
+#if LT_WALK_BATCH == 0
+    static_assert(GEOM == 0 && !(LOG && PHASE == 2) && !(LOG && (TABLE || CAPTURE)), "walk_kernel: slabs; the tail deposits with atomics");
+    constexpr int ROUTE = LOG ? 1 : 0;
+    constexpr bool log_mode = LOG;
+    typedef LdsLayout<R, true> Lds;
+    const Lds L(P.n_media, P.n_layers, 0, 0, LOG ? P.log_n_hist : 0u, 0);
+    constexpr size_t o_cnt = Lds::kOffCnt, o_frame = Lds::kOffFrame, o_math = Lds::kOffMath, o_hist = Lds::kOffHist;
+#else
+    constexpr int ROUTE = -1;
+    const bool log_mode = P.log_idx != nullptr;
     const LdsLayout<R> L(P.n_media, P.n_layers, GEOM == 1 ? P.n_tris : 0, GEOM == 1 ? P.n_nodes : 0,
                          P.log_idx ? P.log_n_hist : 0u, LT_WALK_BATCH == 2 ? 4 * sizeof(MarchWave<R>) : 0);
-    uint32_t* s_hist = reinterpret_cast<uint32_t*>(lds_raw + L.off_hist);
-    if (P.log_idx) for (unsigned t = threadIdx.x; t < P.log_n_hist; t += blockDim.x) s_hist[t] = 0;
-    double* s_cnt = reinterpret_cast<double*>(lds_raw + L.off_cnt);
+    const size_t o_cnt = L.off_cnt, o_frame = L.off_frame, o_math = L.off_math, o_hist = L.off_hist;
+#endif
+    uint32_t* s_hist = reinterpret_cast<uint32_t*>(lds_raw + o_hist);
+    if (log_mode) for (unsigned t = threadIdx.x; t < P.log_n_hist; t += blockDim.x) s_hist[t] = 0;
+    double* s_cnt = reinterpret_cast<double*>(lds_raw + o_cnt);
     const MedD<R>* s_med = reinterpret_cast<const MedD<R>*>(lds_raw + L.off_media);
     const R* s_zb = reinterpret_cast<const R*>(lds_raw + L.off_zb);
     const int32_t* s_lm = reinterpret_cast<const int32_t*>(lds_raw + L.off_lm);
     const IfD<R>* s_if = reinterpret_cast<const IfD<R>*>(lds_raw + L.off_if);
     const TriD<R>* s_tris = GEOM == 2 ? reinterpret_cast<const TriD<R>*>(P.tris)
                                       : reinterpret_cast<const TriD<R>*>(lds_raw + L.off_tris);
-    const NodeD<R>* s_nodes = GEOM == 2 ? reinterpret_cast<const NodeD<R>*>(P.nodes)
+    [[maybe_unused]] const NodeD<R>* s_nodes = GEOM == 2 ? reinterpret_cast<const NodeD<R>*>(P.nodes)
                                         : reinterpret_cast<const NodeD<R>*>(lds_raw + L.off_nodes);
 
-    const int16_t* s_links = !MESH || !P.links ? nullptr
+    [[maybe_unused]] const int16_t* s_links = !MESH || !P.links ? nullptr
                              : (GEOM == 1 ? reinterpret_cast<const int16_t*>(lds_raw + L.off_links) : P.links);
     if (threadIdx.x < 8) s_cnt[threadIdx.x] = 0.0;
-    R* s_frame = reinterpret_cast<R*>(lds_raw + L.off_frame);
+    R* s_frame = reinterpret_cast<R*>(lds_raw + o_frame);
     if (threadIdx.x == 64 % blockDim.x && P.src_type == LT_SRC_COSINE_QUAD) {
         const R nrm[3] = {(R)P.src_dir[0], (R)P.src_dir[1], (R)P.src_dir[2]};
         R v2[3], v3[3];
@@ -51,8 +70,8 @@
         for (int k = 0; k < 3; k++) { s_frame[6 + k] = LT_PV(origin, k); s_frame[9 + k] = LT_PV(inv_voxel, k); s_frame[12 + k] = LT_PV(fdim, k); }
     }
 #endif
-    const double* s_math = reinterpret_cast<const double*>(lds_raw + L.off_math);
-    if constexpr (sizeof(R) == 8) lds_copy(lds_raw + L.off_math, kWalkMathTab, kWalkMathTabBytes);
+    const double* s_math = reinterpret_cast<const double*>(lds_raw + o_math);
+    if constexpr (sizeof(R) == 8) lds_copy(lds_raw + o_math, kWalkMathTab, kWalkMathTabBytes);
     lds_copy(lds_raw + L.off_media, P.media, (size_t)P.n_media * sizeof(MedD<R>));
     if constexpr (!MESH) {
         lds_copy(lds_raw + L.off_zb, P.zb, (size_t)(P.n_layers + 1) * sizeof(R));
@@ -72,6 +91,10 @@
     bool alive = false;
     R px = 0, py = 0, pz = 0, ux = 0, uy = 0, uz = 1, w = 0, sleft = 0;
     int cur = 0;
+#if LT_WALK_BATCH == 0 && LT_SLAB_READS >= 1
+    unsigned moff = (unsigned)L.off_media;
+#define LT_MOFF(layer) ((unsigned)L.off_media + __umul24((unsigned)s_lm[layer], (unsigned)sizeof(MedD<R>)))
+#endif
     unsigned step = 0, max_steps = P.max_steps, nv = 0;
     unsigned long long pid = 0, grp = 0;
     rocrand_state_xorwow rng;
@@ -137,6 +160,12 @@
             const SurvD<R>& S = reinterpret_cast<const SurvD<R>*>(P.pool)[e];
             px = S.p[0]; py = S.p[1]; pz = S.p[2]; ux = S.u[0]; uy = S.u[1]; uz = S.u[2]; w = S.w; sleft = S.sleft;
             cur = S.cur; step = S.step;
+#if LT_WALK_BATCH == 0 && LT_SLAB_READS >= 1
+            moff = LT_MOFF(cur);
+#endif
+#if LT_WALK_BATCH == 0
+            acc_steps -= step;
+#endif
             __builtin_memcpy(&rng, S.rng, sizeof S.rng);
             alive = true;
 #if LT_WALK_BATCH == 1
@@ -189,7 +218,7 @@
                 pid = P.photon_offset + id;
                 alive = true; w = 1; sleft = 0; step = 0; grp = 0;
                 R e_pdf_dir = 1;
-                max_steps = P.max_steps;
+                if constexpr (TABLE || LT_WALK_BATCH != 0) max_steps = P.max_steps;
                 if constexpr (!TABLE) photon_stream(P.seed, pid, &rng);
                 if (P.src_type == LT_SRC_COSINE_QUAD) {
                     R u4[4];
@@ -222,6 +251,9 @@
                     cur = -1;
                     for (int l = 0; l < P.n_layers; l++)
                         if (pz >= s_zb[l] && pz < s_zb[l + 1]) { cur = l; break; }
+#if LT_WALK_BATCH == 0 && LT_SLAB_READS >= 1
+                    if (cur >= 0) moff = LT_MOFF(cur);
+#endif
                     if (cur < 0) {
                         atomicAdd(&s_cnt[CW_ESC_TOP], (double)w); alive = false;
                     } else if (P.src_type == LT_SRC_PENCIL && pz == s_zb[0] && uz > 0) {
@@ -263,7 +295,7 @@
                 const unsigned long long am = __ballot(alive);
                 const unsigned na = (unsigned)__popcll(am);
                 if (na != 0u && na <= P.dump_max) {
-                    emit_deposit<TALLY>(P, pend_idx != kNoVoxel, pend_idx, pend_val, lg_cur, lg_end, lg_chunk, s_hist);
+                    emit_deposit<TALLY, ROUTE>(P, pend_idx != kNoVoxel, pend_idx, pend_val, lg_cur, lg_end, lg_chunk, s_hist);
                     pend_idx = kNoVoxel;
                     const int leader = __ffsll((long long)am) - 1;
                     unsigned base = 0;
@@ -286,7 +318,7 @@
 #else
                             S.q_pend = 0u;
 #endif
-                            alive = false;
+                            LT_END_PHOTON();
                         }
                     }
                     dumped = true;
@@ -524,21 +556,9 @@
         TV f_val = 0;
         if (alive) {
             if (step >= max_steps) {
-                atomicAdd(&s_cnt[CW_CAPPED], (double)w); alive = false;
+                atomicAdd(&s_cnt[CW_CAPPED], (double)w); LT_END_PHOTON();
             } else {
                 step++;
-                acc_steps++;
-                float clr = -1.0f;
-                if constexpr (GEOM == 2) {
-                    if (P.mg.cell) clr = march_clearance<R>(P.mg, px, py, pz);
-                } else if constexpr (MESH) {
-                    if (P.clear) {
-                        const R cx = (px - LT_PV(corg, 0)) * LT_PV(cinv, 0), cy = (py - LT_PV(corg, 1)) * LT_PV(cinv, 1),
-                                cz = (pz - LT_PV(corg, 2)) * LT_PV(cinv, 2);
-                        if (cx >= 0 && cx < LT_PV(cdim, 0) && cy >= 0 && cy < LT_PV(cdim, 1) && cz >= 0 && cz < LT_PV(cdim, 2))
-                            clr = __uint_as_float(P.clear[((size_t)(int)cz * P.cny + (int)cy) * P.cnx + (int)cx].x);
-                    }
-                }
                 R u1;
                 typename HeldU<R, TABLE>::type x0, x2, x3;
                 if constexpr (TABLE) {
@@ -551,35 +571,47 @@
                     x3 = HeldU<R, TABLE>::draw(&rng);
                 }
                 grp++;
-                const MedD<R>* Mp = LT_MED(MESH ? cur : s_lm[cur]);
-                const R mu_t = Mp->mu_t;
+#if LT_SLAB_READS >= 1
+                const MedD<R>* Mp = reinterpret_cast<const MedD<R>*>(lds_raw + moff);
+#else
+                const MedD<R>* Mp = LT_MED(s_lm[cur]);
+#endif
+                const Pair<R> fp = ld_pair(&Mp->mu_t);
+                const R mu_t = fp.a;
+#if LT_SLAB_READS >= 2
+                constexpr bool kEarlyTab = sizeof(R) == 8 && !TABLE;
+                const R z_ahead = s_zb[uz > 0 ? cur + 1 : cur];
+                double2 ln_cell = {0.0, 0.0}, sc_cell = {0.0, 0.0};
+                if constexpr (kEarlyTab) { ln_cell = *neg_log_raw_cell(x0, s_math); sc_cell = *sincos_turn_raw_cell(x2, s_math); }
+                if (sleft == 0) {
+                    if constexpr (kEarlyTab) sleft = neg_log_raw_at(x0, ln_cell);
+                    else sleft = HeldU<R, TABLE>::neg_log(x0, s_math);
+                }
+#else
                 if (sleft == 0) sleft = HeldU<R, TABLE>::neg_log(x0, s_math);
-                const R s = (mu_t > 0) ? sleft * Mp->inv_mu_t : inf;
-
-                R tb = inf; int hit_tri = -1;
-                if constexpr (!MESH) {
-                    if (uz != 0) {
-                        const R dz = (uz > 0 ? s_zb[cur + 1] : s_zb[cur]) - pz;
-                        const R guard = sizeof(R) == 8 ? (R)(1.0 + 1e-12) : (R)(1.0 + 1e-5);
-                        const bool near = !(Mx<R>::abs(dz) > s * Mx<R>::abs(uz) * guard);
-                        if (__any(near)) {
-                            R den = uz;
-                            asm volatile("" : "+v"(den));
-                            if (near) tb = dz / den;
-                        }
-                    }
-                } else {
-                    const bool query = !(s < (R)clr);
-                    if (query) {
-                        R o[3] = {px, py, pz}, d[3] = {ux, uy, uz}, th;
-                        nearest_bvh_walk(s_tris, s_nodes, P.n_nodes, s_links, o, d, s, hit_tri, th);
-                        if (hit_tri >= 0) tb = th;
+#endif
+                const R s_mu = sleft * fp.b;
+                const R s = (mu_t > 0) ? s_mu : inf;
+
+                R tb = inf; constexpr int hit_tri = -1;
+                if (uz != 0) {
+#if LT_SLAB_READS >= 2
+                    const R dz = z_ahead - pz;
+#else
+                    const R dz = (uz > 0 ? s_zb[cur + 1] : s_zb[cur]) - pz;
+#endif
+                    const R guard = sizeof(R) == 8 ? (R)(1.0 + 1e-12) : (R)(1.0 + 1e-5);
+                    const bool near = !(Mx<R>::abs(dz) > s * Mx<R>::abs(uz) * guard);
+                    if (__any(near)) {
+                        R den = uz;
+                        asm volatile("" : "+v"(den));
+                        if (near) tb = dz / den;
                     }
                 }
 #endif
                 const bool at_boundary = MESH ? (hit_tri >= 0) : (tb <= s);
                 if (!at_boundary && !(s < inf)) {
-                    atomicAdd(&s_cnt[MESH ? CW_ESC_MESH : CW_CAPPED], (double)w); alive = false;
+                    atomicAdd(&s_cnt[MESH ? CW_ESC_MESH : CW_CAPPED], (double)w); LT_END_PHOTON();
                 } else if (at_boundary) {
                     px += ux * tb; py += uy * tb; pz += uz * tb;
                     sleft -= tb * mu_t;
@@ -587,7 +619,11 @@
                     if constexpr (!MESH) {
                         const bool down = uz > 0;
                         const int k = down ? cur + 1 : cur, next = down ? cur + 1 : cur - 1;
+#if LT_WALK_BATCH == 0 && LT_SLAB_READS >= 2
+                        pz = z_ahead;
+#else
                         pz = s_zb[k];
+#endif
                         const IfD<R> F = s_if[k];
                         const R Nr = down ? F.nr_down : F.nr_up;
                         R ct;
@@ -599,8 +635,13 @@
                                              refl ? LT_VERTEX_REFLECTIVE : LT_VERTEX_TRANSMISSIVE, cur, step, (R)0, (R)0, down ? (R)-1 : (R)1, (R)0,
                                              gone ? (R)0 : (refl ? Rf : (R)1 - Rf));
                         if (refl) uz = -uz;
-                        else if (gone) { atomicAdd(&s_cnt[next < 0 ? CW_ESC_TOP : CW_ESC_BOT], (double)w); alive = false; }
-                        else { ux *= Nr; uy *= Nr; uz = down ? ct : -ct; cur = next; }
+                        else if (gone) { atomicAdd(&s_cnt[next < 0 ? CW_ESC_TOP : CW_ESC_BOT], (double)w); LT_END_PHOTON(); }
+                        else {
+                            ux *= Nr; uy *= Nr; uz = down ? ct : -ct; cur = next;
+#if LT_WALK_BATCH == 0 && LT_SLAB_READS >= 1
+                            moff = LT_MOFF(next);
+#endif
+                        }
                     } else {
                     R nf[3], n1 = Mp->n, n2; int next;
                     {
@@ -627,7 +668,7 @@
                         ux = ro[0]; uy = ro[1]; uz = ro[2];
                         px += eps * nf[0]; py += eps * nf[1]; pz += eps * nf[2];
                     } else if (next < 0) {
-                        atomicAdd(&s_cnt[CW_ESC_MESH], (double)w); alive = false;
+                        atomicAdd(&s_cnt[CW_ESC_MESH], (double)w); LT_END_PHOTON();
                     } else {
                         ux = refr[0]; uy = refr[1]; uz = refr[2];
                         px -= eps * nf[0]; py -= eps * nf[1]; pz -= eps * nf[2];
@@ -637,7 +678,8 @@
                 } else {
                     px += ux * s; py += uy * s; pz += uz * s;
                     sleft = 0;
-                    const R dw = w * Mp->absorb;
+                    const Pair<R> ad = ld_pair(&Mp->absorb);
+                    const R dw = w * ad.a;
                     if constexpr (CAPTURE) if (P.vertices) {
                         const R ct_c = hg_sample_walk(u1, Mp);
                         record_vertex<R>(P, pid - P.photon_offset, nv, px, py, pz, ux, uy, uz, w, LT_VERTEX_VOLUME, cur, step, (R)0, (R)0, (R)0,
@@ -649,11 +691,11 @@
                     if constexpr (!MESH) inside = (int)(Mx<R>::sign_word(fx) | Mx<R>::sign_word(fy) | Mx<R>::sign_word(fz)) >= 0 &&
                                                   vx < (unsigned)P.nx && vy < (unsigned)P.ny && vz < (unsigned)P.nz;
                     else inside = fx >= 0 && fx < fnx && fy >= 0 && fy < fny && fz >= 0 && fz < fnz;
-                    const unsigned idx = P.log_idx
+                    const unsigned idx = log_mode
                         ? (((__umul24(__umul24(vz >> kTileBZ, P.log_nty) + (vy >> kTileBY), P.log_ntx) + (vx >> kTileBX)) << kTileShift)
                            | ((vz & 15u) << 10) | ((vy & 31u) << 5) | (vx & 31u))
                         : (vz * (unsigned)P.ny + vy) * (unsigned)P.nx + vx;
-                    const TV q = tally_quantum<TALLY, R>(w * Mp->dep);
+                    const TV q = tally_quantum<TALLY, R>(w * ad.b);
                     const bool same = inside && idx == pend_idx;
                     const bool flush = inside && !same;
                     f_idx = flush ? pend_idx : kNoVoxel; f_val = pend_val;
@@ -662,14 +704,20 @@
                     acc_abs += inside ? (double)dw : 0.0;
                     acc_lost += inside ? 0.0 : (double)dw;
                     w -= dw;
-                    if (!(w > 0)) alive = false;
+                    if (!(w > 0)) LT_END_PHOTON();
                     else {
                         R u[3] = {ux, uy, uz};
+#if LT_WALK_BATCH == 0 && LT_SLAB_READS >= 2
+                        if constexpr (kEarlyTab) {
+                            R sp, cp; sincos_turn_raw_at(x2, sc_cell, &sp, &cp);
+                            spin_with<R>(u, hg_sample_walk(u1, Mp), sp, cp);
+                        } else
+#endif
                         spin<R, TABLE>(u, hg_sample_walk(u1, Mp), x2, s_math);
                         ux = u[0]; uy = u[1]; uz = u[2];
                         if (w < (R)1e-4) {
                             if (HeldU<R, TABLE>::get(x3) <= (R)0.1) { atomicAdd(&s_cnt[CW_ROULETTE], -9.0 * (double)w); w *= (R)10; }
-                            else { atomicAdd(&s_cnt[CW_ROULETTE], (double)w); alive = false; }
+                            else { atomicAdd(&s_cnt[CW_ROULETTE], (double)w); LT_END_PHOTON(); }
                         }
                     }
                 }
@@ -678,10 +726,10 @@
 #if LT_WALK_BATCH && defined(LT_DIAG_MESH)
         dg_clk_bnd += clock64() - dg_t1;
 #endif
-        emit_deposit<TALLY>(P, f_idx != kNoVoxel, f_idx, f_val, lg_cur, lg_end, lg_chunk, s_hist);
+        emit_deposit<TALLY, ROUTE>(P, f_idx != kNoVoxel, f_idx, f_val, lg_cur, lg_end, lg_chunk, s_hist);
     }
-    emit_deposit<TALLY>(P, pend_idx != kNoVoxel, pend_idx, pend_val, lg_cur, lg_end, lg_chunk, s_hist);
-    if (P.log_idx && lg_chunk < kLogExhausted && (threadIdx.x & 63) == 0) P.log_fill[lg_chunk] = lg_cur - lg_chunk * kLogChunk;
+    emit_deposit<TALLY, ROUTE>(P, pend_idx != kNoVoxel, pend_idx, pend_val, lg_cur, lg_end, lg_chunk, s_hist);
+    if (log_mode && lg_chunk < kLogExhausted && (threadIdx.x & 63) == 0) P.log_fill[lg_chunk] = lg_cur - lg_chunk * kLogChunk;
 
 #if LT_WALK_BATCH && defined(LT_DIAG_MESH)
 #if LT_WALK_BATCH == 2
@@ -720,7 +768,7 @@
         __hip_atomic_fetch_add(&P.counters->steps, ws, __ATOMIC_RELAXED, __HIP_MEMORY_SCOPE_AGENT);
     }
     __syncthreads();
-    if (P.log_idx)
+    if (log_mode)
         for (unsigned t = threadIdx.x; t < P.log_n_hist; t += blockDim.x)
             if (s_hist[t]) __hip_atomic_fetch_add(&P.log_hist[t * kLogGroups + (blockIdx.x & (kLogGroups - 1))], s_hist[t],
                                                   __ATOMIC_RELAXED, __HIP_MEMORY_SCOPE_AGENT);
@@ -730,6 +778,10 @@
         __hip_atomic_fetch_add(&P.counters->w[threadIdx.x], s_cnt[threadIdx.x], __ATOMIC_RELAXED,
                                __HIP_MEMORY_SCOPE_AGENT);
 }
+#undef LT_END_PHOTON
+#ifdef LT_MOFF
+#undef LT_MOFF
+#endif
 #if LT_INV_MODE == 2
 #undef gx0
 #undef gy0
```
